# thunlp/OpenMatch

Hardware: AMD Instinct MI355X
Metric: passages/sec encode (bert-base DPR bi-encoder, 128 tok -> 768-d) [+ queries/sec exact top-1000 over 8.8M x 768 in `search`] (higher is better)
Workload: dtype f16; 1 GPU; bert-base DPR bi-encoder encode+search, MS MARCO 8.8M x 128-tok -> 768-d (BASELINE configs[1]); seq_len=128, global_batch=1024, index_rows=8841823, queries=6980, topk=1000, weights=random-init BertConfig() seed 0, parallelism=shard1

## Files before the change

### include/openmatch_hip.h

```cpp
#ifndef OPENMATCH_HIP_H
#define OPENMATCH_HIP_H

#include <stddef.h>
#include <stdint.h>

#ifdef __cplusplus
extern "C" {
#endif

#define OM_ABI_VERSION 6

#define OM_F32 0
#define OM_BF16 1
#define OM_F16 2

#define OM_ACT_NONE 0
#define OM_ACT_GELU_ERF 1
#define OM_ACT_RELU 2
#define OM_ACT_GELU_TANH 3
#define OM_ACT_SILU 5
#define OM_ACT_MUL_RESID 0x100
#define OM_ACT_PRE_GRAD 0x200

#define OM_ARCH_BERT 0
#define OM_ARCH_T5 1
#define OM_ARCH_MODERNBERT 2

#define OM_ARCH_CAUSAL 3

#define OM_ARCH_NOMICBERT 4

#define OM_POOL_NONE 0
#define OM_POOL_FIRST 1
#define OM_POOL_MEAN 2
#define OM_POOL_LAST 3

#define OM_SEARCH_F32 0
#define OM_SEARCH_F16_RESCORE 1
#define OM_SEARCH_F16_ONLY 2

const char* om_last_error(void);
int om_abi_version(void);

int om_device_count(void);

#define OM_TIMING_GEMM_BF16 0
#define OM_TIMING_GEMM_F32 1
#define OM_TIMING_SCAN 2
void om_debug_gemm_trace(unsigned long long* buf);
void om_debug_gemm_gen(int gen);
#define OM_GEMM_FAMILY_V1 1
#define OM_GEMM_FAMILY_V2 2
#define OM_GEMM_FAMILY_V6 6
#define OM_GEMM_FAMILY_G7 7
#define OM_GEMM_FAMILY_G7_ONE_TILE 70
#define OM_GEMM_FAMILY_G7C16 71
#define OM_GEMM_FAMILY_G7R16 72
#define OM_GEMM_FAMILY_SKINNY 9
int om_debug_gemm_last(void);
int om_debug_gemm_plan(int in_dtype, const void* A, int64_t lda, const void* B, int64_t ldb, int out_dtype, void* C, int64_t ldc,
                       int64_t M, int64_t N, int64_t K, const float* bias, const void* resid, int64_t ldr, int act);
typedef struct OmDebugGemmEpilogue {
  const float* bias; const void* resid; int64_t ldr; int act;
  void* pre_act; int64_t ldp; float drop_p; uint64_t seed; const int* drop_rows;
  const float* ln_stats; const float* ln_colsum; const float* rln_stats; const float* rln_g; const float* rln_b; float* stats_out;
  const void* resid_lo; void* out_lo;
  const float* resid32; float* out32;
  const float* a_ln32; const float* a_ln_g; const float* a_ln_b; float* a_ln_stats_out; const float* rln32; const float* rln32_stats;
  int lo8; float ln_inv_h, ln_eps; int ln_rms; int reverse;
  const int* rows_dev;
} OmDebugGemmEpilogue;
int om_debug_gemm_ex(int in_dtype, const void* A, int64_t lda, const void* B, int64_t ldb, int out_dtype, void* C, int64_t ldc,
                     int64_t M, int64_t N, int64_t K, const OmDebugGemmEpilogue* ep, void* stream);
int om_debug_gemm_plan_ex(int in_dtype, const void* A, int64_t lda, const void* B, int64_t ldb, int out_dtype, void* C, int64_t ldc,
                          int64_t M, int64_t N, int64_t K, const OmDebugGemmEpilogue* ep);
int om_debug_gemm_splitk(int in_dtype, const void* A, int64_t lda, const void* B, int64_t ldb, float* C, int64_t ldc, int64_t M,
                         int64_t N, int64_t K, void* stream);
#define OM_OPT_ENCODER_FUSED_LN 0
#define OM_OPT_ENCODER_DEBUG 1
#define OM_OPT_ATTENTION_FAST 2
#define OM_OPT_SCAN_GEN7 3
#define OM_OPT_SCAN_GROWTH 4
#define OM_OPT_WGRAD_DEBUG 5
#define OM_OPT_GEMM_GROUP_M 6
#define OM_OPT_SCAN_QGROUP 7
#define OM_OPT_TRAIN_WGRAD_STREAM 8
#define OM_OPT_ATTENTION_DEBUG 9
#define OM_OPT_ENCODER_PINGPONG 10
#define OM_OPT_ENCODER_TWO_PLANE 11
#define OM_OPT_GEMM_VARIANT 12
#define OM_OPT_SEARCH_DEBUG 13
#define OM_OPT_TRAIN_WGRAD_BATCH 14
#define OM_OPT_GEMM_MAX_GRID 15
#define OM_OPT_GEMM_CONT 16
#define OM_OPT_TRAIN_TAPE_GRAD 17
#define OM_OPT_TRAIN_RES32 18
#define OM_OPT_GEMM_SKINNY_M 19
#define OM_OPT_GEMM_SKINNY_CFG 20
#define OM_OPT_FEW_ROWS_LN_FUSE 21
#define OM_OPT_ENCODER_SKIP_PAD 22
#define OM_OPT_ENCODER_CLS_TAIL 23
#define OM_OPT_ENCODER_LANES 24
#define OM_OPT_COUNT 25
int om_debug_option(int opt, int value);
int om_debug_option_value(int opt);
int om_debug_attention(const void* qkv, void* ctx, const int64_t* mask, int64_t B, int L, int H, int heads, void* stream);
int om_debug_attention_ex(int dtype, const void* qkv, void* ctx, const int64_t* mask, const float* pos_bias, int64_t B, int L, int H,
                          int heads, float scale, float drop_p, uint64_t seed, void* stream, int reverse, const int* kmax,
                          const int* cu, int w);
int om_debug_rope(int dtype, void* qkv, int64_t M, int L, int H, float theta, void* stream);
int om_debug_rope_rows(int dtype, void* qkv, int64_t rows, int L, int H, float theta, const int* row_map, void* stream);
int om_debug_swiglu_rows(int dtype, const void* in, void* out, int64_t M, int F, void* stream);
int om_debug_embed(int dtype, const int64_t* ids, const int64_t* type_ids, const float* word, const float* pos, const float* type,
                   const float* g, const float* b, void* out, int64_t M, int L, int H, int vocab, int type_vocab, float eps, void* stream);
int om_debug_attention_causal(int dtype, const void* qkv, void* ctx, const int64_t* mask, int64_t B, int L, int n_heads, int n_kv_heads,
                              float scale, void* stream);
int om_debug_rope_gqa(int dtype, void* qkv, int64_t M, int L, int n_heads, int n_kv_heads, const float* inv_freq, float scaling, void* stream);
int om_debug_attention_causal_packed(int dtype, const void* qkv, void* ctx, const int64_t* mask, const int* cu, int64_t B, int L, int n_heads,
                                     int n_kv_heads, float scale, void* stream);
int om_debug_rope_gqa_rows(int dtype, void* qkv, int64_t rows, int L, int n_heads, int n_kv_heads, const float* inv_freq, float scaling,
                           const int* row_map, void* stream);
int om_debug_attention_causal_hd(int dtype, const void* qkv, void* ctx, const int64_t* mask, int64_t B, int L, int n_heads, int n_kv_heads,
                                 int head_dim, float scale, void* stream);
int om_debug_attention_causal_hd_packed(int dtype, const void* qkv, void* ctx, const int64_t* mask, const int* cu, int64_t B, int L,
                                        int n_heads, int n_kv_heads, int head_dim, float scale, void* stream);
int om_debug_qknorm_rope(int dtype, void* qkv, int64_t M, int L, int n_heads, int n_kv_heads, int head_dim, const float* q_norm_g,
                         const float* k_norm_g, float eps, const float* inv_freq, float scaling, void* stream);
int om_debug_qknorm_rope_rows(int dtype, void* qkv, int64_t rows, int L, int n_heads, int n_kv_heads, int head_dim, const float* q_norm_g,
                              const float* k_norm_g, float eps, const float* inv_freq, float scaling, const int* row_map, void* stream);
int om_debug_attention_gqa_d256(int dtype, const void* qkv, void* ctx, const int64_t* mask, int64_t B, int L, int n_heads, int n_kv_heads,
                                float scale, int w, void* stream);
int om_debug_qknorm_rope_d256(int dtype, void* qkv, int64_t M, int L, int n_heads, int n_kv_heads, const float* q_norm_g, const float* k_norm_g,
                              float eps, const float* inv_freq, float scaling, void* stream);
int om_debug_attention_gqa_d256_packed(int dtype, const void* qkv, void* ctx, const int64_t* mask, const int* cu, int64_t B, int L, int n_heads,
                                       int n_kv_heads, float scale, int w, void* stream);
int om_debug_qknorm_rope_d256_rows(int dtype, void* qkv, int64_t rows, int L, int n_heads, int n_kv_heads, const float* q_norm_g,
                                   const float* k_norm_g, float eps, const float* inv_freq, float scaling, const int* row_map, void* stream);
int om_debug_rmsnorm_add(int dtype, const void* h, int64_t ldh, float* x, int64_t ldx, const float* g, int64_t M, int H, float eps, void* stream);
int om_debug_mask_extent(const int64_t* mask, int64_t B, int L, int* kmax, void* stream);
int om_debug_pack_rows(const int* kmax, int64_t B, int L, int64_t rows, int* cu, int* cls_rows, int* row_map, void* stream);
#define OM_ATTN_FAMILY_GENERIC 1
#define OM_ATTN_FAMILY_FWD16 2
#define OM_ATTN_FAMILY_FWD16_KMAX4 3
#define OM_ATTN_FAMILY_FWD16C 4
#define OM_ATTN_FAMILY_LONG 5
#define OM_ATTN_FAMILY_D32 6
#define OM_ATTN_FAMILY_BAND16 7
#define OM_ATTN_FAMILY_BAND32 8
int om_debug_attention_last(void);
int om_debug_attention_plan(int dtype, int64_t B, int L, int H, int heads, int has_bias, float drop_p, int has_kmax, int has_cu, int w);
#define OM_ATTN_BWD_FAMILY_BWD16 1
#define OM_ATTN_BWD_FAMILY_GENERIC 2
#define OM_ATTN_BWD_FAMILY_LONG 3
#define OM_ATTN_BWD_FAMILY_D32 4
int om_debug_attention_bwd_last(void);
int om_debug_attention_bwd_plan(int dtype, int64_t B, int L, int H, int heads, int has_bias, int has_drel, int has_cu, int packed);
int om_debug_attention_bwd_ex(int dtype, const void* qkv, const void* ctx, const void* dctx, void* dqkv, const int64_t* mask,
                              const float* pos_bias, float* drel, float* stats, int64_t B, int L, int H, int heads, float scale,
                              float drop_p, uint64_t seed, const int* cu, int packed, void* stream);
size_t om_debug_attention_bwd_stats_bytes(int64_t B, int heads);
#define OM_ENC_PATH_BERT_FUSED 1
#define OM_ENC_PATH_BERT_PENDING_LN 2
#define OM_ENC_PATH_BERT_FEW32 3
#define OM_ENC_PATH_BERT_PLAIN 4
#define OM_ENC_PATH_MODERNBERT 5
#define OM_ENC_PATH_T5_FUSED 6
#define OM_ENC_PATH_T5_PLAIN 7
struct OmEncoderConfig;
int om_debug_encoder_plan(const struct OmEncoderConfig* cfg, int gated_ffn, int has_rel_bias, int64_t B, int64_t L, int64_t packed_rows,
                          int want_hidden);
int om_debug_encoder_skip_pad(const struct OmEncoderConfig* cfg, int gated_ffn, int has_rel_bias, int64_t B, int64_t L, int want_hidden);
int om_debug_encoder_cls_tail(const struct OmEncoderConfig* cfg, int gated_ffn, int has_rel_bias, int64_t B, int64_t L, int64_t packed_rows,
                              int want_hidden);
int om_debug_encoder_lanes(const struct OmEncoderConfig* cfg, int gated_ffn, int has_rel_bias, int64_t B, int64_t L, int64_t packed_rows,
                           int want_hidden, int64_t* B0);
#define OM_ENCODER_LANE_RANGES 15
int om_debug_encoder_lane_ranges(const struct OmEncoderConfig* cfg, int gated_ffn, int has_rel_bias, int64_t B, int64_t L, int lane,
                                 int64_t* out, int cap);
int64_t om_debug_encoder_lane_forks(void);
int om_debug_gather_rows(const void* src0, void* dst0, const void* src1, void* dst1, const void* src2, void* dst2, const float* stats_src,
                         float* stats_dst, const int* rows, int64_t B, int64_t L, int64_t Mc, int H, void* stream);
int om_debug_attn_drop_keep(uint64_t seed, int64_t b, int h, int heads, int Lm, int q, int key, float p);
int om_debug_wave_sum_check(const float* in, float* out_shuffle, float* out_dpp, int64_t groups, void* stream);
#define OM_ROW_FWD_GENERIC 1
#define OM_ROW_FWD_X8 2
#define OM_ROW_LN_BWD 3
int om_debug_row_kernel_last(void);
int om_debug_layernorm(int dtype, const void* x, int64_t ldx, void* y, int64_t ldy, const float* g, const float* b, int64_t M, int H,
                       float eps, int rms, const void* x_lo, int lo8, void* stream);
int om_debug_layernorm_f32out(int dtype, const void* x, int64_t ldx, float* y, int64_t ldy, const float* g, const float* b, int64_t M,
                              int H, float eps, int rms, const void* x_lo, const int* rows, int lo8, void* stream);
int om_debug_layernorm_from_f32(int dtype, const float* x, int64_t ldx, void* y, int64_t ldy, const float* g, const float* b, int64_t M,
                                int H, float eps, int rms, void* stream);
int om_debug_layernorm_dual(int dtype, const float* x, int64_t ldx, void* y, float* y32, int64_t ldy, const float* g, const float* b,
                            int64_t M, int H, float eps, void* stream);
int om_debug_norm_bwd(int dtype, const void* dy, const void* x, const float* g, void* dx, float* dg, float* db, int64_t M, int H,
                      float eps, int rms, const void* add, void* stream);
int om_debug_ln_bwd_drop(int dtype, const void* dy, const void* x, const float* g, void* dx, void* dx_drop, float drop_p,
                         uint64_t drop_seed, float* dg, float* db, int64_t M, int H, float eps, const float* dy32, const float* x32,
                         float* partial, int* partial_blocks , const int* drop_rows, void* stream);
typedef struct OmLnSite { const float* partial; float* dg; float* db; int blocks; } OmLnSite;
int om_debug_ln_param_reduce(const OmLnSite* sites , int n, int H, void* stream);
int om_debug_embed_bwd(int dtype, const void* dy, const int64_t* ids, const int64_t* type_ids, const float* word, const float* pos,
                       const float* type, const float* g, float* dword, float* dpos, float* dtype_, float* dg, float* db, int64_t M,
                       int L, int H, int vocab, int type_vocab, float eps, const int* cu, void* stream);
int om_debug_pool(int dtype, const void* x, const int64_t* mask, float* out, int64_t B, int L, int H, int mode, const int* cu,
                  void* stream);
int om_debug_pool_bwd(int dtype, const float* dp, const int64_t* mask, void* dh, int64_t B, int L, int H, int mode, const int* cu,
                      void* stream);
int om_debug_l2norm(const float* x, float* y, int64_t M, int D, void* stream);
int om_debug_l2norm_bwd(const float* x, const float* dy, float* dx, int64_t M, int D, void* stream);
int om_debug_colsum(int dtype, const void* x, int64_t ld, int64_t M, int N, float* out, void* stream);
int om_debug_dropout(int dtype, const void* x, void* y, int64_t n, float p, uint64_t seed, const int* rows, int H, void* stream);
int om_debug_ln_fold(int dtype, const void* W, const float* gamma, const float* beta, const float* b, void* Wf, float* colsum,
                     float* bf, int N, int K, void* stream);
int om_debug_ln_stats_reduce(const float* slots, int nslots, int64_t M, float* out, void* stream);
int om_debug_transpose(int dtype, const void* in, int64_t ldi, int64_t R, int C, void* out, int64_t ldo, int64_t Rp, int op, void* stream);
int om_debug_transpose_batch(int dtype, const void* const* in, void* const* out, const int* R, const int* C, int n, void* stream);
int om_debug_zero_rows_from(void* p, int64_t row_bytes, const int* first, int64_t M, void* stream);
int om_debug_t5_act_fwd(int dtype, const void* f, const void* f2, void* g, int64_t n, int kind, void* stream);
int om_debug_t5_act_bwd(int dtype, const void* dg, const void* f, const void* f2, void* df, void* df2, int64_t n, int kind, void* stream);
int om_debug_t5_embed_bwd(int dtype, const void* dy, const int64_t* ids, float* dword, int64_t M, int H, int vocab, const int* row_map,
                          void* stream);
int om_debug_t5_bias(const float* table, const int* lut, float* out, int L, int heads, void* stream);
int om_debug_t5_bias_bwd(const float* drel, const int* lut, float* dtable, int L, int heads, void* stream);
int om_kernel_timing_enable(int enable);
int om_kernel_timing_read(int kernel_class, double* total_ms, int64_t* launches, double* flops);

int om_gemm_nt(int in_dtype, const void* A, int64_t lda, const void* B, int64_t ldb,
               int out_dtype, void* C, int64_t ldc, int64_t M, int64_t N, int64_t K,
               const float* bias, const void* resid, int64_t ldr, int act, void* stream);

int om_gemm_tn_acc(int in_dtype, const void* A, int64_t lda, const void* B, int64_t ldb,
                   float* C, int64_t ldc, float* bias, int64_t M, int64_t N, int64_t K, void* stream);

typedef struct OmTnProblem {
  const void* A; const void* B; float* C; float* bias;
  int64_t lda, ldb, ldc, N, K;
} OmTnProblem;
int om_gemm_tn_acc_batch(int in_dtype, const OmTnProblem* problems, int n, int64_t M, void* stream);
int om_debug_gemm_tn_last(int64_t out[8]);
int om_debug_gemm_tn_plan(int dtype, int64_t M, int64_t N, int64_t K, int64_t lda, int64_t ldb, int batch, int64_t out[8]);

typedef struct OmLayerWeights {
  const void* qkv_w;
  const float* qkv_b;
  const void* o_w;
  const float* o_b;
  const float* ln1_g;
  const float* ln1_b;
  const void* ffn1_w;
  const float* ffn1_b;
  const void* ffn1g_w;
  const void* ffn2_w;
  const float* ffn2_b;
  const float* ln2_g;
  const float* ln2_b;
} OmLayerWeights;

typedef struct OmEncoderConfig {
  int arch;
  int dtype;
  int hidden;
  int n_layers;
  int n_heads;
  int head_dim;
  int ffn;
  int vocab;
  int max_pos;
  int type_vocab;
  int act;
  float ln_eps;
  int rel_buckets;
  int rel_max_dist;
  int pooling;
  int head_in;
  int head_out;
  int normalize;
  float rope_theta_global;
  float rope_theta_local;
  int half_window;
  uint64_t sliding_layers;
} OmEncoderConfig;

typedef struct OmEncoderWeights {
  const float* word_emb;
  const float* pos_emb;
  const float* type_emb;
  const float* emb_ln_g;
  const float* emb_ln_b;
  const OmLayerWeights* layers_host;
  const float* final_ln_g;
  const float* rel_bias;
  const float* head_w;
  const void* folded;
  const float* final_ln_b;
} OmEncoderWeights;

size_t om_encoder_fold_bytes(const OmEncoderConfig* cfg);
int om_encoder_fold_weights(const OmEncoderConfig* cfg, const OmEncoderWeights* w, void* folded, size_t bytes, void* stream);

size_t om_encoder_workspace_bytes(const OmEncoderConfig* cfg, int64_t B, int64_t L);

int om_t5_relative_bucket(int relative_position, int num_buckets, int max_distance);

int om_encoder_forward(const OmEncoderConfig* cfg, const OmEncoderWeights* w,
                       const int64_t* input_ids, const int64_t* attention_mask,
                       const int64_t* token_type_ids, int64_t B, int64_t L,
                       void* out_hidden, float* out_reps, void* workspace,
                       size_t workspace_bytes, void* stream);

int om_encoder_packed_supported(const OmEncoderConfig* cfg, int gated_ffn, int64_t B, int64_t L, int64_t packed_rows);
size_t om_encoder_workspace_bytes_packed(const OmEncoderConfig* cfg, int64_t B, int64_t L, int64_t packed_rows);
int om_encoder_forward_packed(const OmEncoderConfig* cfg, const OmEncoderWeights* w,
                              const int64_t* input_ids, const int64_t* attention_mask,
                              const int64_t* token_type_ids, int64_t B, int64_t L, int64_t packed_rows,
                              float* out_reps, void* workspace, size_t workspace_bytes, void* stream);

typedef struct OmCausalConfig {
  OmEncoderConfig base;
  int n_kv_heads;
  float rope_attention_scaling;
  float inv_freq[32];
} OmCausalConfig;
size_t om_causal_encoder_workspace_bytes(const OmCausalConfig* cfg, int64_t B, int64_t L);
int om_causal_encoder_forward(const OmCausalConfig* cfg, const OmEncoderWeights* w, const int64_t* input_ids,
                              const int64_t* attention_mask, int64_t B, int64_t L, void* out_hidden, float* out_reps,
                              void* workspace, size_t workspace_bytes, void* stream);
int om_causal_encoder_packed_supported(const OmCausalConfig* cfg, int64_t B, int64_t L, int64_t packed_rows);
size_t om_causal_encoder_workspace_bytes_packed(const OmCausalConfig* cfg, int64_t B, int64_t L, int64_t packed_rows);
int om_causal_encoder_forward_packed(const OmCausalConfig* cfg, const OmEncoderWeights* w, const int64_t* input_ids,
                                     const int64_t* attention_mask, int64_t B, int64_t L, int64_t packed_rows, float* out_reps,
                                     void* workspace, size_t workspace_bytes, void* stream);

typedef struct OmCausalConfig2 {
  OmCausalConfig base;
  int qk_norm;
  int reserved;
  float inv_freq[64];
} OmCausalConfig2;
typedef struct OmCausalQkNorm {
  const float* q_norm_g;
  const float* k_norm_g;
} OmCausalQkNorm;
size_t om_causal2_encoder_workspace_bytes(const OmCausalConfig2* cfg, int64_t B, int64_t L);
int om_causal2_encoder_forward(const OmCausalConfig2* cfg, const OmEncoderWeights* w, const OmCausalQkNorm* qk_norm_host,
                               const int64_t* input_ids, const int64_t* attention_mask, int64_t B, int64_t L, void* out_hidden,
                               float* out_reps, void* workspace, size_t workspace_bytes, void* stream);
int om_causal2_encoder_packed_supported(const OmCausalConfig2* cfg, int64_t B, int64_t L, int64_t packed_rows);
size_t om_causal2_encoder_workspace_bytes_packed(const OmCausalConfig2* cfg, int64_t B, int64_t L, int64_t packed_rows);
int om_causal2_encoder_forward_packed(const OmCausalConfig2* cfg, const OmEncoderWeights* w, const OmCausalQkNorm* qk_norm_host,
                                      const int64_t* input_ids, const int64_t* attention_mask, int64_t B, int64_t L, int64_t packed_rows,
                                      float* out_reps, void* workspace, size_t workspace_bytes, void* stream);

#define OM_ARCH_GEMMA3 5
typedef struct OmGemma3Config {
  OmCausalConfig base;
  float attn_scale;
  int half_window;
  uint64_t sliding_layers;
  float full_scaling;
  float sliding_scaling;
  float attn_logit_softcapping;
  int bidirectional;
  float full_inv_freq[128];
  float sliding_inv_freq[128];
} OmGemma3Config;
typedef struct OmGemma3Norms {
  const float* q_norm_g;
  const float* k_norm_g;
  const float* post_attention_norm_g;
  const float* post_feedforward_norm_g;
} OmGemma3Norms;
size_t om_gemma3_encoder_workspace_bytes(const OmGemma3Config* cfg, int64_t B, int64_t L);
int om_gemma3_encoder_forward(const OmGemma3Config* cfg, const OmEncoderWeights* w, const OmGemma3Norms* norms_host, const int64_t* input_ids,
                              const int64_t* attention_mask, int64_t B, int64_t L, void* out_hidden, float* out_reps, void* workspace,
                              size_t workspace_bytes, void* stream);
int om_gemma3_encoder_packed_supported(const OmGemma3Config* cfg, int64_t B, int64_t L, int64_t packed_rows);
size_t om_gemma3_encoder_workspace_bytes_packed(const OmGemma3Config* cfg, int64_t B, int64_t L, int64_t packed_rows);
int om_gemma3_encoder_forward_packed(const OmGemma3Config* cfg, const OmEncoderWeights* w, const OmGemma3Norms* norms_host,
                                     const int64_t* input_ids, const int64_t* attention_mask, int64_t B, int64_t L, int64_t packed_rows,
                                     float* out_reps, void* workspace, size_t workspace_bytes, void* stream);

typedef struct OmT5DecoderLayer {
  const void* sa_v_w;
  const void* sa_o_w;
  const float* sa_ln_g;
  const void* ca_q_w;
  const void* ca_kv_w;
  const void* ca_o_w;
  const float* ca_ln_g;
  const void* ffn1_w;
  const void* ffn1g_w;
  const void* ffn2_w;
  const float* ffn_ln_g;
} OmT5DecoderLayer;
typedef struct OmT5DecoderWeights {
  const float* start_emb;
  const float* final_ln_g;
  const OmT5DecoderLayer* layers_host;
  int n_layers;
} OmT5DecoderWeights;
size_t om_t5_decoder_workspace_bytes(const OmEncoderConfig* cfg, int64_t B, int64_t L);
int om_t5_decoder_step(const OmEncoderConfig* cfg, const OmT5DecoderWeights* w, const void* enc_hidden,
                       const int64_t* attention_mask, int64_t B, int64_t L, float* out_hidden,
                       void* workspace, size_t workspace_bytes, void* stream);

typedef struct OmT5DecoderLayerGrads {
  float* sa_v_w;  float* sa_o_w; float* sa_ln_g;
  float* ca_q_w;  float* ca_kv_w; float* ca_o_w; float* ca_ln_g;
  float* ffn1_w;  float* ffn1g_w; float* ffn2_w; float* ffn_ln_g;
} OmT5DecoderLayerGrads;
typedef struct OmT5DecoderGrads {
  float* start_emb;
  float* final_ln_g;
  const OmT5DecoderLayerGrads* layers_host;
} OmT5DecoderGrads;
size_t om_t5_decoder_tape_bytes(const OmEncoderConfig* cfg, int n_layers, int64_t B, int64_t L);
size_t om_t5_decoder_train_workspace_bytes(const OmEncoderConfig* cfg, int n_layers, int64_t B, int64_t L);
int om_t5_decoder_train_forward(const OmEncoderConfig* cfg, const OmT5DecoderWeights* w, const void* enc_hidden,
                                const int64_t* attention_mask, int64_t B, int64_t L, float dropout, uint64_t seed,
                                void* tape, size_t tape_bytes, float* out_hidden, void* workspace,
                                size_t workspace_bytes, void* stream);
int om_t5_decoder_train_backward(const OmEncoderConfig* cfg, const OmT5DecoderWeights* w, const void* enc_hidden,
                                 const int64_t* attention_mask, int64_t B, int64_t L, float dropout, uint64_t seed,
                                 const void* tape, const float* d_out, const OmT5DecoderGrads* grads,
                                 void* d_enc_hidden, void* workspace, size_t workspace_bytes, void* stream);

int om_linear_f32_backward(const float* dy, const float* x, const float* w, float* dw, float* dx, int B, int D, int K,
                           void* stream);

typedef struct OmLayerGrads {
  float* qkv_w;  float* qkv_b;  float* o_w;    float* o_b;   float* ln1_g; float* ln1_b;
  float* ffn1_w; float* ffn1_b; float* ffn2_w; float* ffn2_b; float* ln2_g; float* ln2_b;
  float* ffn1g_w;
} OmLayerGrads;

typedef struct OmEncoderGrads {
  float* word_emb; float* pos_emb; float* type_emb; float* emb_ln_g; float* emb_ln_b;
  const OmLayerGrads* layers_host;
  float* head_w;
  float* final_ln_g;
  float* rel_bias;
} OmEncoderGrads;

size_t om_encoder_tape_bytes(const OmEncoderConfig* cfg, int64_t B, int64_t L);
size_t om_encoder_train_workspace_bytes(const OmEncoderConfig* cfg, int64_t B, int64_t L);

int om_encoder_train_forward(const OmEncoderConfig* cfg, const OmEncoderWeights* w,
                             const int64_t* input_ids, const int64_t* attention_mask,
                             const int64_t* token_type_ids, int64_t B, int64_t L,
                             float hidden_dropout, float attn_dropout, uint64_t seed, void* tape,
                             size_t tape_bytes, float* out_reps, void* workspace,
                             size_t workspace_bytes, void* stream);

int om_encoder_train_backward(const OmEncoderConfig* cfg, const OmEncoderWeights* w,
                              const int64_t* input_ids, const int64_t* attention_mask,
                              const int64_t* token_type_ids, int64_t B, int64_t L,
                              float hidden_dropout, float attn_dropout, uint64_t seed,
                              const void* tape, const float* d_reps, const OmEncoderGrads* grads,
                              void* workspace, size_t workspace_bytes, void* stream);

int om_encoder_train_packed_supported(const OmEncoderConfig* cfg, int64_t B, int64_t L, int64_t packed_rows);
size_t om_encoder_tape_bytes_packed(const OmEncoderConfig* cfg, int64_t B, int64_t L, int64_t packed_rows);
size_t om_encoder_train_workspace_bytes_packed(const OmEncoderConfig* cfg, int64_t B, int64_t L, int64_t packed_rows);
int om_encoder_train_forward_packed(const OmEncoderConfig* cfg, const OmEncoderWeights* w,
                                    const int64_t* input_ids, const int64_t* attention_mask,
                                    const int64_t* token_type_ids, int64_t B, int64_t L, int64_t packed_rows,
                                    float hidden_dropout, float attn_dropout, uint64_t seed,
                                    void* tape, size_t tape_bytes, float* out_reps,
                                    void* workspace, size_t workspace_bytes, void* stream);
int om_encoder_train_backward_packed(const OmEncoderConfig* cfg, const OmEncoderWeights* w,
                                     const int64_t* input_ids, const int64_t* attention_mask,
                                     const int64_t* token_type_ids, int64_t B, int64_t L, int64_t packed_rows,
                                     float hidden_dropout, float attn_dropout, uint64_t seed,
                                     const void* tape, const float* d_reps, const OmEncoderGrads* grads,
// ... 107 lines not shown
```

### openmatch_amd/csrc/abi.cpp

```cpp
#include "common.h"

static thread_local std::string g_last_error;
void om_set_error(const std::string& msg) { g_last_error = msg; }

extern "C" const char* om_last_error(void) { return g_last_error.c_str(); }
extern "C" int om_abi_version(void) { return OM_ABI_VERSION; }
extern "C" int om_device_count(void) {
  int n = 0;
  hipError_t e = hipGetDeviceCount(&n);
  if (e != hipSuccess) {
    om_set_error(std::string("hipGetDeviceCount: ") + hipGetErrorString(e));
    return -1;
  }
  return n;
}

#include <mutex>
#include <vector>
namespace {
struct Span { hipEvent_t a, b; };
struct ClassStat { std::vector<Span> spans; double flops = 0; size_t used = 0; };
bool g_timing = false;
ClassStat g_stat[3];
std::mutex g_mu;
}
bool om_timing_on() { return g_timing; }
void om_timing_begin(int c, hipStream_t s) {
  std::lock_guard<std::mutex> lk(g_mu);
  ClassStat& st = g_stat[c];
  if (st.used == st.spans.size()) {
    Span sp;
    (void)hipEventCreate(&sp.a);
    (void)hipEventCreate(&sp.b);
    st.spans.push_back(sp);
  }
  (void)hipEventRecord(st.spans[st.used].a, s);
}
void om_timing_end(int c, hipStream_t s, double flops) {
  std::lock_guard<std::mutex> lk(g_mu);
  ClassStat& st = g_stat[c];
  (void)hipEventRecord(st.spans[st.used].b, s);
  st.used++;
  st.flops += flops;
}
extern "C" int om_kernel_timing_enable(int enable) { g_timing = enable != 0; return 0; }
extern "C" int om_kernel_timing_read(int c, double* total_ms, int64_t* launches, double* flops) {
  if (c < 0 || c > 2) { om_set_error("om_kernel_timing_read: bad class"); return 1; }
  std::lock_guard<std::mutex> lk(g_mu);
  ClassStat& st = g_stat[c];
  double ms = 0;
  for (size_t i = 0; i < st.used; ++i) {
    hipError_t e = hipEventSynchronize(st.spans[i].b);
    float t = 0;
    if (e == hipSuccess) e = hipEventElapsedTime(&t, st.spans[i].a, st.spans[i].b);
    if (e != hipSuccess) { om_set_error(std::string("om_kernel_timing_read: ") + hipGetErrorString(e)); return 1; }
    ms += t;
  }
  if (total_ms) *total_ms = ms;
  if (launches) *launches = (int64_t)st.used;
  if (flops) *flops = st.flops;
  st.used = 0; st.flops = 0;
  return 0;
}

#include <atomic>
#include <map>
#include <tuple>
namespace {
std::atomic<int> g_opt[OM_OPT_COUNT];
std::atomic<bool> g_opt_init{false};
std::mutex g_opt_mu;
void opt_init() {
  std::lock_guard<std::mutex> lk(g_opt_mu);
  if (g_opt_init.load()) return;
  const char* e = getenv("OM_ENCODER_FUSED_LN");
  g_opt[OM_OPT_ENCODER_FUSED_LN] = e ? atoi(e) : 1;
  g_opt[OM_OPT_ENCODER_DEBUG] = getenv("OM_ENCODER_DEBUG") ? 1 : 0;
  e = getenv("OM_ATTENTION_FAST");
  g_opt[OM_OPT_ATTENTION_FAST] = e ? atoi(e) : 1;
  e = getenv("OM_SCAN_GEN7");
  g_opt[OM_OPT_SCAN_GEN7] = e ? atoi(e) : 1;
  e = getenv("OM_SCAN_GROWTH");
  g_opt[OM_OPT_SCAN_GROWTH] = e ? atoi(e) : 60;
  g_opt[OM_OPT_WGRAD_DEBUG] = 0;
  g_opt[OM_OPT_ATTENTION_DEBUG] = 0;
  e = getenv("OM_ENCODER_PINGPONG");
  g_opt[OM_OPT_ENCODER_PINGPONG] = e ? atoi(e) : 1;
  e = getenv("OM_TRAIN_WGRAD_STREAM");
  g_opt[OM_OPT_TRAIN_WGRAD_STREAM] = e ? atoi(e) : 1;
  e = getenv("OM_SCAN_QGROUP");
  g_opt[OM_OPT_SCAN_QGROUP] = e ? atoi(e) : 8;
  e = getenv("OM_GEMM_GROUP_M");
  g_opt[OM_OPT_GEMM_GROUP_M] = e ? atoi(e) : 8;
  e = getenv("OM_ENCODER_TWO_PLANE");
  g_opt[OM_OPT_ENCODER_TWO_PLANE] = e ? atoi(e) : 3;
  e = getenv("OM_GEMM_VARIANT");
  g_opt[OM_OPT_GEMM_VARIANT] = e ? atoi(e) : 0;
  e = getenv("OM_SEARCH_DEBUG");
  g_opt[OM_OPT_SEARCH_DEBUG] = e ? (atoi(e) ? atoi(e) : 1) : 0;
  e = getenv("OM_TRAIN_WGRAD_BATCH");
  g_opt[OM_OPT_TRAIN_WGRAD_BATCH] = e ? atoi(e) : 4;
  e = getenv("OM_GEMM_MAX_GRID");
  g_opt[OM_OPT_GEMM_MAX_GRID] = e ? atoi(e) : 0;
  e = getenv("OM_TRAIN_TAPE_GRAD");
  g_opt[OM_OPT_TRAIN_TAPE_GRAD] = e ? atoi(e) : 1;
  e = getenv("OM_TRAIN_RES32");
  g_opt[OM_OPT_TRAIN_RES32] = e ? atoi(e) : 1;
  e = getenv("OM_GEMM_CONT");
  g_opt[OM_OPT_GEMM_CONT] = e ? atoi(e) : 495;
  e = getenv("OM_GEMM_SKINNY_M");
  g_opt[OM_OPT_GEMM_SKINNY_M] = e ? atoi(e) : 1024;
  e = getenv("OM_FEW_ROWS_LN_FUSE");
  g_opt[OM_OPT_FEW_ROWS_LN_FUSE] = e ? atoi(e) : 64;
  e = getenv("OM_ENCODER_SKIP_PAD");
  g_opt[OM_OPT_ENCODER_SKIP_PAD] = e ? atoi(e) : 1;
  e = getenv("OM_ENCODER_CLS_TAIL");
  g_opt[OM_OPT_ENCODER_CLS_TAIL] = e ? atoi(e) : 1;
  e = getenv("OM_ENCODER_LANES");
  g_opt[OM_OPT_ENCODER_LANES] = e ? atoi(e) : 65536;
  g_opt_init.store(true);
}
}
bool om_option_is_set(int opt) {
  if (opt == OM_OPT_SCAN_GROWTH) return getenv("OM_SCAN_GROWTH") != nullptr;
  return false;
}
int om_option(int opt) {
  if (!g_opt_init.load(std::memory_order_acquire)) opt_init();
  return g_opt[opt].load(std::memory_order_relaxed);
}
extern "C" int om_debug_option(int opt, int value) {
  if (opt < 0 || opt >= OM_OPT_COUNT) { om_set_error("om_debug_option: unknown option"); return 1; }
  if (!g_opt_init.load(std::memory_order_acquire)) opt_init();
  g_opt[opt].store(value);
  return 0;
}
extern "C" int om_debug_option_value(int opt) {
  if (opt < 0 || opt >= OM_OPT_COUNT) { om_set_error("om_debug_option_value: unknown option"); return -1; }
  return om_option(opt);
}

int om_t5_lut_device(int L, int buckets, int max_dist, const int** out) {
  static std::mutex mu;
  static std::map<std::tuple<int, int, int, int>, int*> cache;
  int dev = 0;
  OM_HIP(hipGetDevice(&dev));
  std::lock_guard<std::mutex> lk(mu);
  auto key = std::make_tuple(dev, L, buckets, max_dist);
  auto it = cache.find(key);
  if (it == cache.end()) {
    std::vector<int> lut(2 * L);
    for (int rel = -(L - 1); rel <= L - 1; ++rel) lut[rel + (L - 1)] = om_t5_relative_bucket(rel, buckets, max_dist);
    int* d = nullptr;
    OM_HIP(hipMalloc(&d, (size_t)(2 * L) * sizeof(int)));
    OM_HIP(hipMemcpy(d, lut.data(), (size_t)(2 * L - 1) * sizeof(int), hipMemcpyHostToDevice));
    it = cache.emplace(key, d).first;
  }
  *out = it->second;
  return 0;
}
```

### openmatch_amd/csrc/attention.hip

```cpp
#include <type_traits>

#include "attn_chunked.h"
#include "attn_plan.h"

static thread_local int g_attn_last = 0;
extern "C" int om_debug_attention_last(void) { return g_attn_last; }

template <typename T, int KT>
__global__ __launch_bounds__(64 * KT) void attention_kernel(
    const T* __restrict__ qkv, T* __restrict__ ctx, const int64_t* __restrict__ mask,
    const float* __restrict__ pos_bias, int L, int H, int heads, float scale, float drop_p,
    uint64_t seed) {
  typedef AttnGeom<T> G;
  typedef typename MmaOps<T>::frag_t frag_t;
  constexpr int LP = KT * 32 + 4;
  extern __shared__ __attribute__((aligned(16))) char smem[];
  char* sK = smem;
  T* sVt = (T*)(smem + KT * 32 * G::ROWB);
  float* sM = (float*)(smem + KT * 32 * G::ROWB + 64 * LP * (int)sizeof(T));

  const int h = blockIdx.x % heads;
  const int64_t b = blockIdx.x / heads;
  const int tid = threadIdx.x, nthr = blockDim.x;
  const int64_t ld = 3 * (int64_t)H;
  const T* base = qkv + b * L * ld + h * 64;

  for (int idx = tid; idx < KT * 32 * G::CPR; idx += nthr) {
    const int row = idx / G::CPR, c = idx % G::CPR;
    uint4 kv = make_uint4(0, 0, 0, 0), vv = make_uint4(0, 0, 0, 0);
    if (row < L) {
      kv = *(const uint4*)(base + (int64_t)row * ld + H + c * G::EPC);
      vv = *(const uint4*)(base + (int64_t)row * ld + 2 * H + c * G::EPC);
    }
    *(uint4*)(sK + row * G::ROWB + ((c ^ G::key(row)) << 4)) = kv;
    const T* ve = (const T*)&vv;
#pragma unroll
    for (int e = 0; e < G::EPC; ++e) sVt[(c * G::EPC + e) * LP + row] = ve[e];
  }
  for (int k = tid; k < KT * 32; k += nthr)
    sM[k] = k < L ? (mask[b * L + k] != 0 ? 0.f : kFinfoMin) : -INFINITY;
  __syncthreads();

  const int wave = tid >> 6, lane = tid & 63, half = lane >> 5, l31 = lane & 31;
  const int q0 = wave * 32;
  if (q0 >= L) return;
  const int qrow = (q0 + l31) < L ? (q0 + l31) : (L - 1);

  frag_t qf[G::NKK];
#pragma unroll
  for (int kk = 0; kk < G::NKK; ++kk)
    qf[kk] = *(const frag_t*)(base + (int64_t)qrow * ld + (kk * 2 + half) * G::EPC);

  f32x16_t s[KT];
#pragma unroll
  for (int t = 0; t < KT; ++t) {
#pragma unroll
    for (int r = 0; r < 16; ++r) s[t][r] = 0.f;
    const int row = t * 32 + l31;
    const char* krow = sK + row * G::ROWB;
    const int key = G::key(row);
#pragma unroll
    for (int kk = 0; kk < G::NKK; ++kk) {
      const frag_t a = *(const frag_t*)(krow + (((kk * 2 + half) ^ key) << 4));
      MmaOps<T>::mma(a, qf[kk], s[t]);
    }
  }

  float mx = -INFINITY;
#pragma unroll
  for (int t = 0; t < KT; ++t)
#pragma unroll
    for (int g = 0; g < 4; ++g) {
      const int k0 = t * 32 + 8 * g + 4 * half;
      const f32x4_t mb = *(const f32x4_t*)(sM + k0);
#pragma unroll
      for (int e = 0; e < 4; ++e) {
        float v = s[t][4 * g + e] * scale;
        if (pos_bias) {
          const int kc = (k0 + e) < L ? (k0 + e) : (L - 1);
          v += pos_bias[((int64_t)h * L + qrow) * L + kc];
        }
        v += mb[e];
        s[t][4 * g + e] = v;
        mx = fmaxf(mx, v);
      }
    }
  mx = fmaxf(mx, __shfl_xor(mx, 32, 64));
  float sum = 0.f;
#pragma unroll
  for (int t = 0; t < KT; ++t)
#pragma unroll
    for (int r = 0; r < 16; ++r) {
      const float e = G::exp_(s[t][r] - mx);
      s[t][r] = e;
      sum += e;
    }
  sum += __shfl_xor(sum, 32, 64);
  const float inv = 1.0f / sum;
#pragma unroll
  for (int t = 0; t < KT; ++t)
#pragma unroll
    for (int r = 0; r < 16; ++r) s[t][r] *= inv;
  if (drop_p > 0.f) {
    const AttnDrop dr(drop_p);
#pragma unroll
    for (int t = 0; t < KT; ++t)
#pragma unroll
      for (int g = 0; g < 4; ++g) {
        const uint64_t bits = attn_drop_bits(seed, b, h, heads, L, q0 + l31, (t * 32 + 8 * g + 4 * half) >> 2);
#pragma unroll
        for (int e = 0; e < 4; ++e) s[t][4 * g + e] = attn_drop_keep(bits, e, dr.thresh) ? s[t][4 * g + e] * dr.keep_scale : 0.f;
      }
  }

  f32x16_t o[2];
#pragma unroll
  for (int dt = 0; dt < 2; ++dt)
#pragma unroll
    for (int r = 0; r < 16; ++r) o[dt][r] = 0.f;
#pragma unroll
  for (int t = 0; t < KT; ++t) SlabMma<T>::run(s[t], sVt + l31 * LP + t * 32 + 4 * half, LP, o);

  __syncthreads();
  T* so = (T*)(sK + (size_t)q0 * G::ROWB);
#pragma unroll
  for (int dt = 0; dt < 2; ++dt)
#pragma unroll
    for (int r = 0; r < 16; ++r) {
      const int q = (r & 3) + 8 * (r >> 2) + 4 * half;
      ElemOps<T>::store(so + q * 64 + dt * 32 + l31, o[dt][r]);
    }
  T* out = ctx + (b * L + q0) * H + h * 64;
  constexpr int VPR = G::ROWB / 16;
#pragma unroll
  for (int it = 0; it < 32 * VPR / 64; ++it) {
    const int idx = it * 64 + lane, row = idx / VPR, c = idx % VPR;
    const uint4 v = *(const uint4*)((const char*)so + row * G::ROWB + c * 16);
    if (q0 + row < L) *(uint4*)((char*)(out + (int64_t)row * H) + c * 16) = v;
  }
}

template <typename T, int KT, bool BIAS, bool DROP, int DBG, int KTV>
__device__ __forceinline__ void attention_fwd16_body(
    const T* __restrict__ qkv, T* __restrict__ ctx, const int64_t* __restrict__ mask,
    const float* __restrict__ pos_bias, int L, int H, int heads, float scale, float drop_p, uint64_t seed, int rev,
    int64_t row0, int Lm) {
  typedef typename MmaOps<T>::frag_t frag_t;
  extern __shared__ __attribute__((aligned(16))) char smem[];
  char* const sK = smem;
  char* const sV = smem + KT * 32 * 128;
  float* const sM = (float*)(smem + 2 * KT * 32 * 128);
  const int h = blockIdx.x % heads;
  const int64_t b = rev ? (int64_t)(gridDim.x / heads) - 1 - blockIdx.x / heads : blockIdx.x / heads;
  const int tid = threadIdx.x, lane = tid & 63, half = lane >> 5, l31 = lane & 31;
  const int wave = __builtin_amdgcn_readfirstlane(tid >> 6);
  const int64_t ld2 = 6 * (int64_t)H;
  const char* const base = (const char*)(qkv + row0 * 3 * (int64_t)H + h * 64);
  if (!(DBG & 1))
#pragma unroll
  for (int i = 0; i < 4; ++i) {
    if (KTV < KT && i * KT + wave >= KTV * 4) continue;
    const int r = (i * KT + wave) * 8 + (lane >> 3);
    const int rr = r < L ? r : L - 1;
    const uint32_t off = (uint32_t)(rr * ld2) + (((lane & 7) ^ ((r >> 1) & 7)) << 4);
    const uint32_t offv = (uint32_t)(rr * ld2) + (((lane & 7) ^ (((r >> 1) & 1) << 2)) << 4);
    const uint32_t dst = (uint32_t)((i * KT + wave) * 1024);
    g7_dma(base + 2 * H, off, g7_lds_addr(sK) + dst);
    g7_dma(base + 4 * H, offv, g7_lds_addr(sV) + dst);
  }
  const float LOG2E = 1.4426950408889634f;
  for (int k = tid; k < KT * 32; k += 64 * KT)
    sM[k] = k < L ? (mask[b * Lm + k] != 0 ? 0.f : -1e30f) : -INFINITY;

  const int q0 = wave * 32;
  const int qrow = (q0 + l31) < L ? (q0 + l31) : (L - 1);
  frag_t qf[4];
#pragma unroll
  for (int kk = 0; kk < 4; ++kk) qf[kk] = *(const frag_t*)(base + (int64_t)qrow * ld2 + (kk * 2 + half) * 16);
  asm volatile("s_waitcnt vmcnt(0)" ::: "memory");
  __syncthreads();
  if (q0 >= L) return;

  constexpr int KTC = (DBG & 2) ? 0 : KTV;
  const int key = (l31 >> 1) & 7;
  f32x16_t s[KTV];
#pragma unroll
  for (int t = 0; t < KTC; ++t) {
#pragma unroll
    for (int r = 0; r < 16; ++r) s[t][r] = 0.f;
    const char* krow = sK + (t * 32 + l31) * 128;
#pragma unroll
    for (int kk = 0; kk < 4; ++kk) {
      const frag_t a = *(const frag_t*)(krow + (((kk * 2 + half) ^ key) << 4));
      MmaOps<T>::mma(a, qf[kk], s[t]);
    }
    __builtin_amdgcn_sched_barrier(0);
  }
  const float c2 = scale * LOG2E;
  float mx = -INFINITY;
#pragma unroll
  for (int t = 0; t < KTC; ++t)
#pragma unroll
    for (int g = 0; g < 4; ++g) {
      const int k0 = t * 32 + 8 * g + 4 * half;
      const f32x4_t mb = *(const f32x4_t*)(sM + k0);
      f32x4_t pb = {0.f, 0.f, 0.f, 0.f};
      if (BIAS) {
        const float* pr = pos_bias + ((int64_t)h * Lm + qrow) * Lm;
#pragma unroll
        for (int e = 0; e < 4; ++e) pb[e] = pr[(k0 + e) < Lm ? (k0 + e) : (Lm - 1)] * LOG2E;
      }
#pragma unroll
      for (int e = 0; e < 4; ++e) {
        const float v = fmaf(s[t][4 * g + e], c2, mb[e]) + pb[e];
        s[t][4 * g + e] = v;
        mx = fmaxf(mx, v);
      }
      __builtin_amdgcn_sched_barrier(0);
    }
  mx = fmaxf(mx, __shfl_xor(mx, 32, 64));
  float sum = 0.f;
#pragma unroll
  for (int t = 0; t < KTC; ++t)
#pragma unroll
    for (int r = 0; r < 16; ++r) {
      const float e = __builtin_amdgcn_exp2f(s[t][r] - mx);
      s[t][r] = e;
      sum += e;
    }
  sum += __shfl_xor(sum, 32, 64);
  float inv = 1.0f / sum;
  if (DROP) {
    const AttnDrop dr(drop_p);
#pragma unroll
    for (int t = 0; t < KTC; ++t)
  #pragma unroll
      for (int g = 0; g < 4; ++g) {
        const uint64_t bits = attn_drop_bits(seed, b, h, heads, Lm, q0 + l31, (t * 32 + 8 * g + 4 * half) >> 2);
#pragma unroll
        for (int e = 0; e < 4; ++e) s[t][4 * g + e] = attn_drop_keep(bits, e, dr.thresh) ? s[t][4 * g + e] : 0.f;
        __builtin_amdgcn_sched_barrier(0);
      }
    inv *= dr.keep_scale;
  }

  const int i16 = lane & 15;
  const char* const vt0 = sV + (4 * half + (i16 >> 2)) * 128 + 32 * ((lane >> 4) & 1) + 8 * (i16 & 3);
  const int vsw = (i16 >> 3) & 1;
  f32x16_t o[2];
#pragma unroll
  for (int dt = 0; dt < 2; ++dt)
#pragma unroll
    for (int r = 0; r < 16; ++r) o[dt][r] = 0.f;
#pragma unroll
  for (int t = 0; t < KTC; ++t) {
    uint4 pa[2];
#pragma unroll
    for (int u = 0; u < 2; ++u)
      pa[u] = make_uint4(Half16<T>::pack2(s[t][8 * u + 0], s[t][8 * u + 1]), Half16<T>::pack2(s[t][8 * u + 2], s[t][8 * u + 3]),
                         Half16<T>::pack2(s[t][8 * u + 4], s[t][8 * u + 5]), Half16<T>::pack2(s[t][8 * u + 6], s[t][8 * u + 7]));
#pragma unroll
    for (int u = 0; u < 2; ++u) {
#pragma unroll
      for (int dt = 0; dt < 2; ++dt) {
        const char* p = vt0 + (t * 32 + 16 * u) * 128 + ((dt ^ vsw) << 6);
        const frag_t vf = vfrag_of<frag_t>(vtrd(p), vtrd(p + 8 * 128));
        MmaOps<T>::mma(vf, __builtin_bit_cast(frag_t, pa[u]), o[dt]);
      }
    }
    __builtin_amdgcn_sched_barrier(0);
  }
  if (DBG & 2) {
#pragma unroll
    for (int kk = 0; kk < 4; ++kk) o[0][kk] = (float)qf[kk][0];
  }
  __syncthreads();
  char* const so = sK + q0 * 128;
#pragma unroll
  for (int dt = 0; dt < 2; ++dt)
#pragma unroll
    for (int gp = 0; gp < 2; ++gp) {
      uint32_t a0 = Half16<T>::pack2(o[dt][8 * gp + 0] * inv, o[dt][8 * gp + 1] * inv), a1 = Half16<T>::pack2(o[dt][8 * gp + 2] * inv, o[dt][8 * gp + 3] * inv);
      uint32_t b0 = Half16<T>::pack2(o[dt][8 * gp + 4] * inv, o[dt][8 * gp + 5] * inv), b1 = Half16<T>::pack2(o[dt][8 * gp + 6] * inv, o[dt][8 * gp + 7] * inv);
      auto r0 = __builtin_amdgcn_permlane32_swap(a0, b0, false, false);
      auto r1 = __builtin_amdgcn_permlane32_swap(a1, b1, false, false);
      *(uint4*)(so + l31 * 128 + (((4 * dt + 2 * gp + half) ^ (l31 & 7)) << 4)) = make_uint4(r0[0], r1[0], r0[1], r1[1]);
    }
  char* const out = (char*)(ctx + (row0 + q0) * (int64_t)H + h * 64);
#pragma unroll
  for (int it = 0; it < 4; ++it) {
    const int row = it * 8 + (lane >> 3), c = lane & 7;
    const uint4 v = *(const uint4*)(so + row * 128 + ((c ^ (row & 7)) << 4));
    if (!(DBG & 4) || v.x == 0x12345u) { if (q0 + row < L) *(uint4*)(out + (int64_t)row * H * 2 + c * 16) = v; }
  }
}

template <typename T, int KT, bool BIAS, bool DROP, int DBG = 0>
__global__ __launch_bounds__(64 * KT, KT <= 4 ? ((BIAS || DROP) ? 3 : 4) : 2) void attention_fwd16_kernel(
    const T* __restrict__ qkv, T* __restrict__ ctx, const int64_t* __restrict__ mask,
    const float* __restrict__ pos_bias, int L, int H, int heads, float scale, float drop_p, uint64_t seed, int rev,
    const int* __restrict__ kmax, const int* __restrict__ cu) {
#define OM_ATTN_BODY(V) attention_fwd16_body<T, KT, BIAS, DROP, DBG, V>(qkv, ctx, mask, pos_bias, Lb, H, heads, scale, drop_p, seed, rev, row0, L)
  const int64_t b = rev ? (int64_t)(gridDim.x / heads) - 1 - blockIdx.x / heads : blockIdx.x / heads;
  int64_t row0 = b * L;
  int Lb = L;
  if (cu) {
    const int c0 = __builtin_amdgcn_readfirstlane(cu[b]), c1 = __builtin_amdgcn_readfirstlane(cu[b + 1]);
    row0 = c0; Lb = c1 - c0;
    if (Lb <= 0) return;
  }
  if (KT == 4 && !BIAS && !DROP && (kmax || cu)) {
    const int kt = ((cu ? Lb : __builtin_amdgcn_readfirstlane(kmax[b])) + 31) >> 5;
    if (kt <= 1) { OM_ATTN_BODY(1); return; }
    if (kt == 2) { OM_ATTN_BODY(2); return; }
    if (kt == 3) { OM_ATTN_BODY(3); return; }
  }
  OM_ATTN_BODY(KT);
#undef OM_ATTN_BODY
}

template <typename T, int KT, bool BIAS, bool DROP>
static int launch_attn16(const void* qkv, void* ctx, const int64_t* mask, const float* pos_bias, int64_t B, int L, int H,
                         int heads, float scale, float drop_p, uint64_t seed, hipStream_t s, int rev, const int* kmax, const int* cu) {
  const int lds = 2 * KT * 32 * 128 + KT * 32 * 4;
  if (attn_lds_once<attention_fwd16_kernel<T, KT, BIAS, DROP>>(lds)) return 1;
#ifdef OM_PROBE_KERNELS
  const int dbg = (sizeof(T) == 2 && std::is_same<T, bf16_t>::value && KT == 4 && !BIAS && !DROP) ? om_option(OM_OPT_ATTENTION_DEBUG) : 0;
#else
  const int dbg = 0;
#endif
  if (dbg) {
#ifdef OM_PROBE_KERNELS
#define OM_ATTN_DBG(D)                                                                                                        \
  case D:                                                                                                                     \
    hipLaunchKernelGGL((attention_fwd16_kernel<bf16_t, 4, false, false, D>), dim3((unsigned)(heads * B)), dim3(256), lds, s,          \
                       (const bf16_t*)qkv, (bf16_t*)ctx, mask, pos_bias, L, H, heads, scale, drop_p, seed, rev, kmax, cu);    \
    break;
    switch (dbg) { OM_ATTN_DBG(1) OM_ATTN_DBG(2) OM_ATTN_DBG(3) OM_ATTN_DBG(4) OM_ATTN_DBG(5) OM_ATTN_DBG(6) OM_ATTN_DBG(7) default: break; }
#undef OM_ATTN_DBG
#endif
    OM_LAUNCH_CHECK();
    return 0;
  }
  hipLaunchKernelGGL((attention_fwd16_kernel<T, KT, BIAS, DROP>), dim3((unsigned)(heads * B)), dim3(64 * KT), lds, s, (const T*)qkv,
                     (T*)ctx, mask, pos_bias, L, H, heads, scale, drop_p, seed, rev, kmax, cu);
  OM_LAUNCH_CHECK();
  return 0;
}
template <typename T, bool BIAS, bool DROP>
__global__ __launch_bounds__(256, 2) void attention_fwd16c_kernel(
    const T* __restrict__ qkv, T* __restrict__ ctx, const int64_t* __restrict__ mask,
    const float* __restrict__ pos_bias, int Lm, int H, int heads, float scale, float drop_p, uint64_t seed, const int* __restrict__ cu) {
  const int h = blockIdx.x % heads;
  const int64_t b = blockIdx.x / heads;
  int64_t row0 = b * Lm;
  int L = Lm;
  if (cu) {
    const int c0 = __builtin_amdgcn_readfirstlane(cu[b]), c1 = __builtin_amdgcn_readfirstlane(cu[b + 1]);
    row0 = c0; L = c1 - c0;
  }
  const int qb = blockIdx.y * 128;
  if (qb >= L) return;
  attn_chunked16<T, AttnFull, BIAS, DROP>(attn_rows_fused(qkv, ctx, row0, H, h), AttnFull{}, mask + b * Lm, L, L, qb, scale, AttnFullArgs{pos_bias, drop_p, seed, b, h, heads, Lm});
}

template <typename T, bool BIAS, bool DROP>
static int launch_attn16c(const void* qkv, void* ctx, const int64_t* mask, const float* pos_bias, int64_t B, int L, int H,
                           int heads, float scale, float drop_p, uint64_t seed, hipStream_t s, const int* cu) {
  const int lds = 2 * 128 * 128 + 128 * 4;
  hipLaunchKernelGGL((attention_fwd16c_kernel<T, BIAS, DROP>), dim3((unsigned)(heads * B), (unsigned)((L + 127) / 128)), dim3(256), lds, s,
                     (const T*)qkv, (T*)ctx, mask, pos_bias, L, H, heads, scale, drop_p, seed, cu);
  OM_LAUNCH_CHECK();
  return 0;
}
template <typename T>
__global__ __launch_bounds__(256) void attention_long_kernel(
    const T* __restrict__ qkv, T* __restrict__ ctx, const int64_t* __restrict__ mask,
    const float* __restrict__ pos_bias, int Lm, int H, int heads, float scale, float drop_p, uint64_t seed, const int* __restrict__ cu) {
  const int h = blockIdx.x % heads;
  const int64_t b = blockIdx.x / heads;
  const int qb = blockIdx.y * 128;
  int64_t row0 = b * Lm;
  int L = Lm;
  if (cu) { row0 = cu[b]; L = cu[b + 1] - cu[b]; }
  if (qb >= L) return;
  attn_chunked_qreg<T, AttnFull>(attn_rows_fused(qkv, ctx, row0, H, h), AttnFull{}, mask + b * Lm, L, L, qb, scale, AttnFullArgs{pos_bias, drop_p, seed, b, h, heads, Lm});
}

template <typename T>
static int launch_attn_long(const void* qkv, void* ctx, const int64_t* mask, const float* pos_bias, int64_t B, int L, int H,
                            int heads, float scale, float drop_p, uint64_t seed, hipStream_t s, const int* cu) {
  const int lds = 128 * AttnGeom<T>::ROWB + 64 * 132 * (int)sizeof(T) + 128 * 4 + 128 * 4;
  if (attn_lds_once<attention_long_kernel<T>>(lds)) return 1;
  hipLaunchKernelGGL((attention_long_kernel<T>), dim3((unsigned)(heads * B), (unsigned)((L + 127) / 128)), dim3(256), lds, s,
                     (const T*)qkv, (T*)ctx, mask, pos_bias, L, H, heads, scale, drop_p, seed, cu);
  OM_LAUNCH_CHECK();
  return 0;
}

template <typename T, int KT>
static int launch_attn(const void* qkv, void* ctx, const int64_t* mask, const float* pos_bias,
                       int64_t B, int L, int H, int heads, float scale, float drop_p, uint64_t seed,
                       hipStream_t s) {
  constexpr int LP = KT * 32 + 4;
  const int lds = KT * 32 * AttnGeom<T>::ROWB + 64 * LP * (int)sizeof(T) + KT * 32 * 4;
  if (attn_lds_once<attention_kernel<T, KT>>(lds)) return 1;
  const int waves = (L + 31) / 32;
  hipLaunchKernelGGL((attention_kernel<T, KT>), dim3((unsigned)(heads * B)),
                     dim3(64 * waves), lds, s, (const T*)qkv, (T*)ctx, mask, pos_bias, L, H, heads,
                     scale, drop_p, seed);
  OM_LAUNCH_CHECK();
  return 0;
}

__global__ void mask_extent_kernel(const int64_t* __restrict__ mask, int64_t B, int L, int* __restrict__ kmax) {
  const int64_t b = (int64_t)blockIdx.x * (blockDim.x >> 6) + (threadIdx.x >> 6);
  if (b >= B) return;
  const int lane = threadIdx.x & 63;
  int last = 0;
  for (int k = lane; k < L; k += 64) if (mask[b * L + k] != 0) last = k + 1;
#pragma unroll
  for (int o = 32; o > 0; o >>= 1) last = max(last, __shfl_xor(last, o, 64));
  if (lane == 0) kmax[b] = last ? last : L;
}
__global__ __launch_bounds__(1024) void pack_rows_kernel(const int* __restrict__ kmax, int64_t B, int L, int64_t rows, int* __restrict__ cu,
                                                          int* __restrict__ cls_rows, int* __restrict__ row_map) {
  __shared__ int part[1024];
  const int tid = threadIdx.x;
  const int64_t per = (B + 1023) / 1024, lo = tid * per, hi = lo + per < B ? lo + per : B;
  int sum = 0;
  for (int64_t i = lo; i < hi; ++i) sum += kmax[i];
  part[tid] = sum;
  __syncthreads();
  for (int off = 1; off < 1024; off <<= 1) {
    const int v = tid >= off ? part[tid - off] : 0;
    __syncthreads();
    part[tid] += v;
    __syncthreads();
  }
  const int total = part[1023];
  const int cap = (int)rows;
  if (blockIdx.x == 0) {
    int run = part[tid] - sum;
    for (int64_t i = lo; i < hi; ++i) {
      cu[i] = run < cap ? run : cap;
      cls_rows[i] = run < cap ? run : cap - 1;
      run += kmax[i];
    }
    if (tid == 1023) { cu[B] = total < cap ? total : cap; cu[B + 1] = total; }
  }
  for (int64_t t = (int64_t)blockIdx.x * 1024 + tid; t < rows; t += (int64_t)gridDim.x * 1024) {
    int v = -1;
    if (t < total) {
      int a = 0, b = 1023;
      while (a < b) { const int m = (a + b) >> 1; if (part[m] > (int)t) b = m; else a = m + 1; }
      int64_t i = a * per;
      int run = a ? part[a - 1] : 0;
      for (int n = kmax[i]; run + n <= (int)t; n = kmax[++i]) run += n;
      v = (int)(i * L + ((int)t - run));
    }
    row_map[t] = v;
  }
}
int omk_pack_rows(const int* kmax, int64_t B, int L, int64_t rows, int* cu, int* cls_rows, int* row_map, hipStream_t s) {
  if (B <= 0) return 0;
  if (rows > 0x7fffffff || B * (int64_t)L > 0x7fffffff) OM_FAIL("packed rows: token counts below 2^31");
  const int64_t slices = (rows + 1023) / 1024;
  hipLaunchKernelGGL(pack_rows_kernel, dim3((unsigned)(slices < 1 ? 1 : slices > 1024 ? 1024 : slices)), dim3(1024), 0, s, kmax, B, L, rows, cu, cls_rows,
                     row_map);
  OM_LAUNCH_CHECK();
  return 0;
}

int omk_mask_extent(const int64_t* mask, int64_t B, int L, int* kmax, hipStream_t s) {
  if (B <= 0) return 0;
  hipLaunchKernelGGL(mask_extent_kernel, dim3((unsigned)((B + 3) / 4)), dim3(256), 0, s, mask, B, L, kmax);
  OM_LAUNCH_CHECK();
  return 0;
}

int omk_attention(int dtype, const void* qkv, void* ctx, const int64_t* mask, const float* pos_bias, int64_t B, int L, int H, int heads,
                  float scale, float drop_p, uint64_t seed, hipStream_t s, int reverse, const int* kmax, const int* cu, int w) {
  g_attn_last = 0;
  const AttnPlan p = attn_plan_fwd(dtype, B, L, H, heads, pos_bias != nullptr, drop_p, kmax != nullptr, cu != nullptr, w, attn_switches());
  if (p.error) OM_FAIL(p.error);
  g_attn_last = p.family | (p.kt << 8);
  switch (p.family) {
    case 0: return 0;
    case OM_ATTN_FAMILY_D32: return omk_attention_d32(p, dtype, qkv, ctx, mask, pos_bias, B, L, H, heads, scale, drop_p, seed, s, reverse, kmax, cu);
    case OM_ATTN_FAMILY_BAND16: case OM_ATTN_FAMILY_BAND32: return omk_attention_band(dtype, qkv, ctx, mask, B, L, H, heads, scale, w, kmax, s);
    case OM_ATTN_FAMILY_FWD16: case OM_ATTN_FAMILY_FWD16_KMAX4:
      return attn_with_type16(dtype, [&](auto t) {
        return attn_with_kt<1, 2, 4, 6, 8>(p.kt, [&](auto kt) {
          return attn_with_flags(p.bias, p.drop, [&](auto bias, auto drop) {
            return launch_attn16<decltype(t), kt(), bias(), drop()>(qkv, ctx, mask, pos_bias, B, L, H, heads, scale, drop_p, seed, s, reverse, kmax, cu);
          });
        });
      });
    case OM_ATTN_FAMILY_FWD16C:
      return attn_with_type16(dtype, [&](auto t) {
        return attn_with_flags(p.bias, p.drop, [&](auto bias, auto drop) {
          return launch_attn16c<decltype(t), bias(), drop()>(qkv, ctx, mask, pos_bias, B, L, H, heads, scale, drop_p, seed, s, cu);
        });
      });
    case OM_ATTN_FAMILY_LONG:
      return attn_with_type(dtype, [&](auto t) { return launch_attn_long<decltype(t)>(qkv, ctx, mask, pos_bias, B, L, H, heads, scale, drop_p, seed, s, cu); });
    default:
      if (dtype == OM_BF16)
        return attn_with_kt<1, 2, 4, 6, 8>(p.kt, [&](auto kt) { return launch_attn<bf16_t, kt()>(qkv, ctx, mask, pos_bias, B, L, H, heads, scale, drop_p, seed, s); });
      return attn_with_kt<1, 2, 4, 6, 8>(p.kt, [&](auto kt) { return launch_attn<float, kt()>(qkv, ctx, mask, pos_bias, B, L, H, heads, scale, drop_p, seed, s); });
  }
}

extern "C" int om_debug_attention_plan(int dtype, int64_t B, int L, int H, int heads, int has_bias, float drop_p, int has_kmax, int has_cu, int w) {
  const AttnPlan p = attn_plan_fwd(dtype, B, L, H, heads, has_bias != 0, drop_p, has_kmax != 0, has_cu != 0, w, attn_switches());
  if (p.error) { om_set_error(std::string(__func__) + ": " + p.error); return -1; }
  return p.family | (p.kt << 8);
}

extern "C" int om_debug_attention_ex(int dtype, const void* qkv, void* ctx, const int64_t* mask, const float* pos_bias, int64_t B, int L, int H,
                                     int heads, float scale, float drop_p, uint64_t seed, void* stream, int reverse, const int* kmax,
                                     const int* cu, int w) {
  g_attn_last = 0;
  if (!qkv || !ctx || !mask) OM_FAIL("null argument");
  if (dtype != OM_F32 && dtype != OM_BF16 && dtype != OM_F16) OM_FAIL("attention: dtype must be OM_F32, OM_BF16 or OM_F16");
  if (w > 0 && (pos_bias || drop_p > 0.f || cu || reverse)) OM_FAIL("banded attention: no position bias, dropout, packed rows or reverse walk");
  return omk_attention(dtype, qkv, ctx, mask, pos_bias, B, L, H, heads, scale, drop_p, seed, (hipStream_t)stream, reverse, kmax, cu, w);
}
extern "C" int om_debug_attention(const void* qkv, void* ctx, const int64_t* mask, int64_t B, int L, int H, int heads, void* stream) {
  return om_debug_attention_ex(OM_BF16, qkv, ctx, mask, nullptr, B, L, H, heads, 0.125f, 0.f, 0, stream, 0, nullptr, nullptr, 0);
}
extern "C" int om_debug_rope(int dtype, void* qkv, int64_t M, int L, int H, float theta, void* stream) {
  if (!qkv) OM_FAIL("null argument");
  if (dtype != OM_F32 && dtype != OM_BF16 && dtype != OM_F16) OM_FAIL("rotary positions: dtype must be OM_F32, OM_BF16 or OM_F16");
  return omk_rope(dtype, qkv, M, L, H, theta, (hipStream_t)stream);
}
extern "C" int om_debug_rope_rows(int dtype, void* qkv, int64_t rows, int L, int H, float theta, const int* row_map, void* stream) {
  if (!qkv || !row_map) OM_FAIL("null argument");
  if (dtype != OM_F32 && dtype != OM_BF16 && dtype != OM_F16) OM_FAIL("rotary positions: dtype must be OM_F32, OM_BF16 or OM_F16");
  return omk_rope(dtype, qkv, rows, L, H, theta, (hipStream_t)stream, row_map);
}
extern "C" int om_debug_mask_extent(const int64_t* mask, int64_t B, int L, int* kmax, void* stream) {
  if (!mask || !kmax) OM_FAIL("null argument");
  if (L < 1) OM_FAIL("mask extent: L must be at least 1");
  return omk_mask_extent(mask, B, L, kmax, (hipStream_t)stream);
}
extern "C" int om_debug_pack_rows(const int* kmax, int64_t B, int L, int64_t rows, int* cu, int* cls_rows, int* row_map, void* stream) {
  if (!kmax || !cu || !cls_rows || !row_map) OM_FAIL("null argument");
  if (rows < 1) OM_FAIL("packed rows: rows must be at least 1");
  return omk_pack_rows(kmax, B, L, rows, cu, cls_rows, row_map, (hipStream_t)stream);
}
extern "C" int om_debug_attn_drop_keep(uint64_t seed, int64_t b, int h, int heads, int Lm, int q, int key, float p) {
  return attn_drop_keep1(seed, b, h, heads, Lm, q, key, AttnDrop(p).thresh) ? 1 : 0;
}
```

### openmatch_amd/csrc/attn_plan.h

```cpp
#pragma once
#include "kernels.h"

struct AttnSwitches {
  int fast;
};

static AttnSwitches attn_switches() { return AttnSwitches{om_option(OM_OPT_ATTENTION_FAST)}; }

static int attn_kt(int L) { return L <= 32 ? 1 : L <= 64 ? 2 : L <= 128 ? 4 : L <= 192 ? 6 : 8; }

static bool attn_is16(int dtype) { return dtype == OM_BF16 || dtype == OM_F16; }

struct AttnPlan { int family; int kt; bool bias, drop; const char* error; };

static AttnPlan attn_plan_fwd(int dtype, int64_t B, int L, int H, int heads, bool has_bias, float drop_p, bool has_kmax, bool has_cu, int w,
                              const AttnSwitches sw) {
  AttnPlan p = {0, 0, has_bias, drop_p > 0.f, nullptr};
  auto run = [&](int family, int kt) { p.family = family; p.kt = kt; return p; };
  auto refuse = [&](const char* why) { p.error = why; return p; };
  const bool d32 = H == heads * 32;
  if (dtype != OM_F32 && !attn_is16(dtype)) return refuse("attention: dtype must be OM_F32, OM_BF16 or OM_F16");
  if (B <= 0) return p;
  const bool band = w > 0 && w < L - 1;
  if (band && H != heads * 64) return refuse("banded attention: head_dim must be 64");
  if (band && (has_bias || p.drop || has_cu)) return refuse("banded attention: no position bias, dropout, packed rows or reverse walk");
  if (!band && !d32 && H != heads * 64) return refuse("head_dim must be 32 or 64");
  if (has_cu && !(dtype == OM_F16 || (dtype == OM_BF16 && (d32 || sw.fast)))) return refuse("packed rows: the 16-bit attention kernels");
  if (L < 1 || L > 1024) return refuse("sequence length must be in [1,1024]");
  if (L > 256 && p.drop && (L > 512 || dtype == OM_F32)) return refuse("attention with dropout: up to 512 tokens in the 16-bit formats (float32: 256)");
  if (B * heads > 0x7fffffffLL) return refuse("batch too large for one launch");
  if (d32) return run(OM_ATTN_FAMILY_D32, attn_kt(L));
  if (band) return run(dtype == OM_F32 ? OM_ATTN_FAMILY_BAND32 : OM_ATTN_FAMILY_BAND16, 4);
  const bool fast16 = dtype == OM_F16 || (dtype == OM_BF16 && sw.fast);
  if (L > 256 || ((sw.fast & 2) && dtype != OM_F32)) return run(fast16 && !(sw.fast & 4) ? OM_ATTN_FAMILY_FWD16C : OM_ATTN_FAMILY_LONG, 4);
  if (fast16) return run(attn_kt(L) == 4 && !has_bias && !p.drop && (has_kmax || has_cu) ? OM_ATTN_FAMILY_FWD16_KMAX4 : OM_ATTN_FAMILY_FWD16, attn_kt(L));
  return run(OM_ATTN_FAMILY_GENERIC, attn_kt(L));
}

static AttnPlan attn_plan_bwd(int dtype, int64_t B, int L, int H, int heads, bool has_bias, bool has_drel, bool has_cu, bool packed,
                              const AttnSwitches sw) {
  AttnPlan p = {0, 0, has_bias, false, nullptr};
  auto run = [&](int family, int kt) { p.family = family; p.kt = kt; return p; };
  auto refuse = [&](const char* why) { p.error = why; return p; };
  const bool b16 = attn_is16(dtype);
  if (B <= 0) return p;
  if (H != heads * 32 && H != heads * 64) return refuse("head_dim must be 32 or 64");
  if (H == heads * 32) {
    if (L < 1 || L > 256) return refuse("training with head_dim 32 supports sequence lengths up to 256");
    if (has_cu && !b16) return refuse("packed rows: attention backward for 16-bit formats");
    if (B * heads > 0x7fffffffLL) return refuse("batch too large for one launch");
    if (has_bias != has_drel) return refuse("attention backward: a position bias needs its gradient buffer (and the reverse)");
    if (!b16 && dtype != OM_F32) return refuse("attention backward: dtype must be OM_F32, OM_BF16 or OM_F16");
    return run(OM_ATTN_BWD_FAMILY_D32, attn_kt(L));
  }
  if (L > 256 || (!packed && dtype != OM_F32 && ((sw.fast & 2) || ((sw.fast & 1) && L > 192)))) {
    if (L < 1 || L > 512) return refuse("attention backward (tile-at-a-time form): up to 512 tokens");
    if (!b16) return refuse("attention backward beyond 256 tokens: 16-bit formats");
    if (has_cu) return refuse("attention backward (tile-at-a-time form): no packed rows");
    return run(OM_ATTN_BWD_FAMILY_LONG, 4);
  }
  if (has_cu && !b16) return refuse("packed rows: attention backward for 16-bit formats");
  if (b16 && L >= 1 && L <= 128 && sw.fast && has_bias == has_drel) return run(OM_ATTN_BWD_FAMILY_BWD16, attn_kt(L));
  if (L < 1 || L > 256)
    return refuse(has_cu && !has_bias && !has_drel ? "packed rows: attention backward up to 256 tokens, head_dim 64" : "training supports sequence lengths up to 256");
  if (dtype == OM_F32 && L > 192) return refuse("float32 training supports sequence lengths up to 192 (16-bit formats: 256)");
  return run(OM_ATTN_BWD_FAMILY_GENERIC, attn_kt(L));
}
```

### openmatch_amd/csrc/encoder.hip

```cpp
#include <math.h>

#include <stdlib.h>

#include <algorithm>
#include <atomic>
#include <map>
#include <mutex>
#include <utility>
#include <vector>

#include "encoder_plan.h"

namespace {
struct FoldSlot { size_t w, cs, bf; };
struct FoldLayout { size_t per_layer, total; FoldSlot qkv, ffn1; };
FoldLayout fold_layout(const OmEncoderConfig* c) {
  const size_t H = c->hidden, F = enc_ffn1_cols(c);
  size_t off = 0;
  auto take = [&](size_t bytes) { size_t o = off; off = align_up(off + bytes, 256); return o; };
  FoldLayout L;
  L.qkv.w = take(3 * H * H * 2); L.qkv.cs = take(3 * H * 4); L.qkv.bf = take(3 * H * 4);
  L.ffn1.w = take(F * H * 2); L.ffn1.cs = take(F * 4); L.ffn1.bf = take(F * 4);
  L.per_layer = off;
  L.total = off * (size_t)c->n_layers;
  return L;
}
bool fold_applies(const OmEncoderConfig* c) {
  return c->arch != OM_ARCH_MODERNBERT && (c->dtype == OM_BF16 || c->dtype == OM_F16) && c->n_layers > 0 && c->hidden % 256 == 0 && c->ffn % 256 == 0;
}
}

extern "C" size_t om_encoder_fold_bytes(const OmEncoderConfig* cfg) {
  if (!cfg || !fold_applies(cfg)) return 0;
  return fold_layout(cfg).total;
}

extern "C" int om_encoder_fold_weights(const OmEncoderConfig* c, const OmEncoderWeights* w, void* blob, size_t bytes, void* stream) {
  if (!c || !w || !blob) OM_FAIL("null argument");
  if (!fold_applies(c)) OM_FAIL("nothing to fold for this configuration (om_encoder_fold_bytes is 0)");
  const FoldLayout L = fold_layout(c);
  if (bytes < L.total || ((uintptr_t)blob & 255)) OM_FAIL("fold buffer too small or not 256-byte aligned");
  const OmLayerWeights* Ls = w->layers_host;
  if (!Ls) OM_FAIL("layers_host is null");
  hipStream_t s = (hipStream_t)stream;
  const int H = c->hidden, F = enc_ffn1_cols(c);
  const bool bert = enc_bert_family(c);
  for (int l = 0; l < c->n_layers; ++l) {
    char* base = (char*)blob + (size_t)l * L.per_layer;
    const OmLayerWeights& lw = Ls[l];
    if (l > 0) {
      const float* g = bert ? Ls[l - 1].ln2_g : lw.ln1_g;
      const float* beta = bert ? Ls[l - 1].ln2_b : nullptr;
      if (omk_ln_fold(c->dtype, lw.qkv_w, g, beta, bert ? lw.qkv_b : nullptr, base + L.qkv.w, (float*)(base + L.qkv.cs),
                      (float*)(base + L.qkv.bf), 3 * H, H, s)) return 1;
    }
    if (!lw.ffn1g_w) {
      const float* g = bert ? lw.ln1_g : lw.ln2_g;
      const float* beta = bert ? lw.ln1_b : nullptr;
      if (omk_ln_fold(c->dtype, lw.ffn1_w, g, beta, bert ? lw.ffn1_b : nullptr, base + L.ffn1.w, (float*)(base + L.ffn1.cs),
                      (float*)(base + L.ffn1.bf), F, H, s)) return 1;
    }
  }
  return 0;
}

static int folded_weights(const OmEncoderConfig* c, const OmEncoderWeights* w, int layer, bool ffn1, const void* W, const float* g,
                          const float* beta, const float* b, int N, int K, void* scratch_w, float* scratch_cs, float* scratch_bf,
                          hipStream_t s, const void** Wf, const float** cs, const float** bf) {
  if (w->folded) {
    const FoldLayout L = fold_layout(c);
    const char* base = (const char*)w->folded + (size_t)layer * L.per_layer;
    const FoldSlot& sl = ffn1 ? L.ffn1 : L.qkv;
    *Wf = base + sl.w; *cs = (const float*)(base + sl.cs); *bf = (const float*)(base + sl.bf);
    return 0;
  }
  if (omk_ln_fold(c->dtype, W, g, beta, b, scratch_w, scratch_cs, scratch_bf, N, K, s)) return 1;
  *Wf = scratch_w; *cs = scratch_cs; *bf = scratch_bf;
  return 0;
}

struct EncWs {
  char *x, *y, *x1, *qkv, *ctx, *ff, *ff2;
  float *pooled, *headout, *posbias;
  float* final32;
  int* lut;
  int* kmax;
  int *cu, *cls_rows, *row_map;
  char* wfold;
  float *colsum, *bfold, *stats1, *stats2, *slots;
  char *y_lo, *x1_lo;
  float *r32a, *r32b, *y32;
  size_t total;
};

static EncWs carve(const OmEncoderConfig* c, const EncPlan& p, int64_t B, int64_t L, int64_t packed_rows, char* base) {
  const bool half = c->dtype == OM_BF16 || c->dtype == OM_F16;
  const size_t es = half ? 2 : 4;
  const size_t Mreal = (size_t)p.M, M = (size_t)p.Mp, H = c->hidden, F = c->ffn, F1 = enc_ffn1_cols(c);
  const bool bertf = enc_bert_family(c);
  size_t off = 0;
  auto take = [&](size_t bytes) { size_t o = off; off = align_up(off + bytes, 256); return base + o; };
  EncWs w;
  w.x = take(M * H * es);
  w.y = take(M * H * es);
  w.x1 = take(M * H * es);
  w.qkv = take(M * 3 * H * es);
  w.ctx = take(M * H * es);
  w.ff = take(M * F1 * es);
  w.ff2 = take(c->arch == OM_ARCH_T5 || c->arch == OM_ARCH_MODERNBERT || c->arch == OM_ARCH_NOMICBERT ? M * F * es : 0);
  w.pooled = (float*)take((size_t)B * H * 4);
  w.headout = (float*)take((size_t)B * (c->head_out > 0 ? c->head_out : 1) * 4);
  const bool rel = c->arch == OM_ARCH_T5 || (c->arch == OM_ARCH_BERT && c->rel_buckets > 0);
  w.posbias = (float*)take(rel ? (size_t)c->n_heads * L * L * 4 : 0);
  w.lut = (int*)take(rel ? (size_t)(2 * L) * 4 : 0);
  w.kmax = (int*)take((size_t)B * 4);
  w.cu = (int*)take(packed_rows > 0 ? (size_t)(B + 2) * 4 : 0);
  w.cls_rows = (int*)take(packed_rows > 0 ? (size_t)B * 4 : 0);
  w.row_map = (int*)take(packed_rows > 0 ? (size_t)packed_rows * 4 : 0);
  w.final32 = (float*)take(half && c->pooling != OM_POOL_NONE ? (c->pooling == OM_POOL_FIRST ? (size_t)B : Mreal) * H * 4 : 0);
  const bool fuse = half && c->arch != OM_ARCH_MODERNBERT;
  const size_t wide = std::max((size_t)3 * H, F1);
  w.wfold = take(fuse ? wide * H * es : 0);
  w.colsum = (float*)take(fuse ? wide * 4 : 0);
  w.bfold = (float*)take(fuse ? wide * 4 : 0);
  w.stats1 = (float*)take(fuse ? (size_t)2 * c->n_layers * M * 8 : 0);
  w.stats2 = w.stats1 ? w.stats1 + (size_t)c->n_layers * M * 2 : nullptr;
  w.slots = (float*)take(fuse ? (size_t)2 * ((H + 255) / 256) * M * 8 : 0);
  const bool two = fuse && bertf;
  w.y_lo = take(two ? M * H * es : 0);
  w.x1_lo = take(two ? M * H * es : 0);
  w.r32a = (float*)take(p.alloc_few32 ? Mreal * H * 4 : 0);
  w.r32b = (float*)take(p.alloc_few32 ? Mreal * H * 4 : 0);
  w.y32 = (float*)take(p.alloc_few32 ? Mreal * H * 4 : 0);
  w.total = off;
  return w;
}

static size_t workspace_bytes(const OmEncoderConfig* c, int64_t B, int64_t L, int64_t packed_rows) {
  const EncPlan p = encoder_plan_checked(EncPlanIn{c, B, L, packed_rows, false, false, false, false}, encoder_switches());
  return carve(c, p, B, L, packed_rows, nullptr).total;
}

extern "C" size_t om_encoder_workspace_bytes(const OmEncoderConfig* cfg, int64_t B, int64_t L) {
  if (!cfg || B <= 0 || L <= 0) return 0;
  return workspace_bytes(cfg, B, L, 0);
}

extern "C" size_t om_encoder_workspace_bytes_packed(const OmEncoderConfig* cfg, int64_t B, int64_t L, int64_t packed_rows) {
  if (!cfg || B <= 0 || L <= 0 || packed_rows <= 0) return 0;
  return workspace_bytes(cfg, B, L, packed_rows);
}

extern "C" int om_encoder_packed_supported(const OmEncoderConfig* c, int gated_ffn, int64_t B, int64_t L, int64_t packed_rows) {
  return encoder_packed_ok(c, gated_ffn != 0, B, L, packed_rows, encoder_switches()) ? 1 : 0;
}

extern "C" int om_debug_encoder_plan(const OmEncoderConfig* c, int gated_ffn, int has_rel_bias, int64_t B, int64_t L, int64_t packed_rows,
                                     int want_hidden) {
  if (!c) {
    om_set_error("om_debug_encoder_plan: null argument");
    return -1;
  }
  const EncPlan p = encoder_plan(EncPlanIn{c, B, L, packed_rows, want_hidden != 0, gated_ffn != 0, has_rel_bias != 0, c->type_vocab > 0},
                                 encoder_switches());
  if (p.error) {
    om_set_error(std::string("om_debug_encoder_plan: ") + p.error);
    return -1;
  }
  return p.path | (int)p.few_rows << 8 | (int)p.two << 9 | p.lo8 << 10;
}

extern "C" int om_debug_encoder_skip_pad(const OmEncoderConfig* c, int gated_ffn, int has_rel_bias, int64_t B, int64_t L, int want_hidden) {
  if (!c) {
    om_set_error("om_debug_encoder_skip_pad: null argument");
    return -1;
  }
  const EncPlanIn in = {c, B, L, 0, want_hidden != 0, gated_ffn != 0, has_rel_bias != 0, c->type_vocab > 0};
  const EncSwitches sw = encoder_switches();
  return encoder_skip_pad(in, encoder_plan(in, sw), sw) ? 1 : 0;
}

extern "C" int om_debug_encoder_cls_tail(const OmEncoderConfig* c, int gated_ffn, int has_rel_bias, int64_t B, int64_t L, int64_t packed_rows,
                                         int want_hidden) {
  if (!c) {
    om_set_error("om_debug_encoder_cls_tail: null argument");
    return -1;
  }
  const EncPlanIn in = {c, B, L, packed_rows, want_hidden != 0, gated_ffn != 0, has_rel_bias != 0, c->type_vocab > 0};
  const EncSwitches sw = encoder_switches();
  return encoder_cls_tail(in, encoder_plan(in, sw), sw) ? 1 : 0;
}

extern "C" int om_t5_relative_bucket(int relative_position, int num_buckets, int max_distance) {
  int nb = num_buckets / 2;
  int bucket = relative_position > 0 ? nb : 0;
  const int n = relative_position < 0 ? -relative_position : relative_position;
  const int max_exact = nb / 2;
  if (n < max_exact) return bucket + n;
  const double v = log((double)n / max_exact) / log((double)max_distance / max_exact) * (nb - max_exact);
  int large = max_exact + (int)v;
  if (large > nb - 1) large = nb - 1;
  return bucket + large;
}

static int check_cfg(const OmEncoderConfig* c) {
  if (const char* why = encoder_cfg_error(c)) OM_FAIL(why);
  return 0;
}

struct EncCall {
  const OmEncoderConfig* c;
  const OmEncoderWeights* w;
  const int64_t* mask;
  int64_t B, L;
  const EncPlan& p;
  const EncWs& ws;
  const float* posbias;
  const int* cu;
  const int* row_map;
  void* out_hidden;
  hipStream_t s;
  const int* rows_dev;
  int64_t cls_mc;
  std::vector<int>* families;
  int64_t whole_mg, whole_mc;
};

struct EncStream {
  const void* x;
  const void* x_lo;
  int lo8;
  const float *g, *b;
  int rms;
  void* spare;
  char* hidden;
  const float* rows32;
  bool cls_compact;
};

#define GEMM(A_, lda_, W_, ldw_, C_, ldc_, N_, K_, bias_, res_, ldr_, act_)                        \
  do {                                                                                             \
    if (om_gemm_nt(dt, A_, lda_, W_, ldw_, dt, C_, ldc_, Mg, N_, K_, bias_, res_, ldr_, act_, s)) \
      return 1;                                                                                    \
  } while (0)
#define RUN(expr) do { if (expr) return 1; } while (0)
#define ENC_LOCALS                                                                                                   \
  const OmEncoderConfig* c = k.c; const EncWs& ws = k.ws; const OmLayerWeights* Ls = k.w->layers_host; hipStream_t s = k.s;     \
  const int dt = c->dtype, H = c->hidden, F = c->ffn, nh = c->n_heads;                                              \
  const int64_t B = k.B, L = k.L, M = k.p.M, Mg = k.p.Mg
#define NOMIC_LOCALS                                                                                                 \
  const bool nomic = c->arch == OM_ARCH_NOMICBERT;                                                                   \
  const int F1 = enc_ffn1_cols(c), act1 = nomic ? OM_ACT_NONE : c->act;                                             \
  const void* const ffa = nomic ? ws.ff2 : ws.ff
#define NOMIC_ROPE() do { if (nomic) RUN(omk_rope(dt, ws.qkv, M, (int)L, H, c->rope_theta_global, s, k.row_map)); } while (0)
#define NOMIC_SWIGLU(rows_) do { if (nomic) RUN(omk_swiglu_rows(dt, ws.ff, ws.ff2, rows_, F, s)); } while (0)

static int bert_fused(const EncCall& k, EncStream* out) {
  ENC_LOCALS;
  NOMIC_LOCALS;
  const float scale = 1.0f / sqrtf((float)c->head_dim);
  const float inv_h = 1.0f / (float)H;
  const bool two = k.p.two;
  const int lo8 = k.p.lo8;
  const int nslots = 2 * (H / 256);
  const bool pingpong = k.p.pingpong;
  int walk = 1;
  const bool probe = k.families != nullptr;
  auto gemm = [&](const void* A, int64_t lda, const void* W, int64_t ldw, void* C, int64_t ldc, int64_t rows, int64_t N, int64_t K,
                  const GemmEpilogue& ep) {
    const int64_t as = rows == Mg ? k.whole_mg : k.whole_mc;
    if (!probe) return omk_gemm(dt, A, lda, W, ldw, dt, C, ldc, rows, N, K, ep, s, as);
    k.families->push_back(omk_gemm_family(dt, A, lda, W, ldw, dt, C, ldc, rows, N, K, ep, as));
    return 0;
  };
#define LAUNCH(expr) do { if (!probe) RUN(expr); } while (0)
  const int64_t Mc = k.cls_mc;
  const size_t cplane = (size_t)Mc * H * 2;
  char* const cbase = ws.qkv;
  float* const cst2p = (float*)(cbase + 7 * cplane);
  float* const cst1 = cst2p + 2 * Mc;
  if (Mc > 0 && ((char*)(cst1 + 2 * Mc) > ws.qkv + (size_t)Mg * 3 * H * 2 || Mc > Mg || c->n_layers < 2 || lo8))
    OM_FAIL("[CLS] tail: the compact buffers do not fit the qkv area");
#define OM_WALK() (pingpong ? (walk ^= 1, walk ^ 1) : 0)
  for (int l = 0; l < c->n_layers; ++l) {
    const OmLayerWeights& lw = Ls[l];
    const bool last = l == c->n_layers - 1, tail = last && Mc > 0;
    float* st1 = tail ? cst1 : ws.stats1 + (size_t)l * Mg * 2;
    float* st2 = ws.stats2 + (size_t)l * Mg * 2;
    const float* st2p = l ? ws.stats2 + (size_t)(l - 1) * Mg * 2 : nullptr;
    const int64_t Mr = tail ? Mc : Mg;
    const int* const rdev = tail ? nullptr : k.rows_dev;
    const char *ctx = ws.ctx, *xin = ws.x1, *xin_lo = ws.x1_lo;
    char *y = ws.y, *y_lo = ws.y_lo, *xout = ws.x1, *xout_lo = ws.x1_lo;
    GemmEpilogue e = {};
    if (l == 0) {
      e.bias = lw.qkv_b; e.reverse = OM_WALK(); e.rows_dev = k.rows_dev;
      RUN(gemm(ws.x, H, lw.qkv_w, H, ws.qkv, 3 * H, Mg, 3 * H, H, e));
    } else {
      const OmLayerWeights& pw = Ls[l - 1];
      const void* wf; const float *cs, *bfp;
      RUN(folded_weights(c, k.w, l, false, lw.qkv_w, pw.ln2_g, pw.ln2_b, lw.qkv_b, 3 * H, H, ws.wfold, ws.colsum, ws.bfold, s, &wf, &cs, &bfp));
      e.bias = bfp; e.ln_stats = st2p; e.ln_colsum = cs; e.ln_inv_h = inv_h; e.ln_eps = c->ln_eps; e.reverse = OM_WALK(); e.rows_dev = k.rows_dev;
      RUN(gemm(ws.x1, H, wf, H, ws.qkv, 3 * H, Mg, 3 * H, H, e));
    }
    if (!probe) NOMIC_ROPE();
    const int attn_walk = OM_WALK();
    LAUNCH(omk_attention(dt, ws.qkv, ws.ctx, k.mask, k.posbias, B, (int)L, H, nh, scale, 0.f, 0, s, attn_walk, ws.kmax, k.cu));
    if (tail) {
      const GatherPlane planes[3] = {{ws.ctx, cbase}, {ws.x1, cbase + cplane}, {two ? ws.x1_lo : nullptr, cbase + 2 * cplane}};
      LAUNCH(omk_gather_rows(planes, st2p, cst2p, k.cu ? ws.cls_rows : nullptr, B, L, Mc, H, s));
      ctx = cbase; xin = cbase + cplane; xin_lo = cbase + 2 * cplane; st2p = cst2p;
      y = cbase + 3 * cplane; y_lo = cbase + 4 * cplane; xout = cbase + 5 * cplane; xout_lo = cbase + 6 * cplane;
    }
    e = GemmEpilogue{};
    e.bias = lw.o_b; e.ldr = H; e.stats_out = ws.slots; e.ln_inv_h = inv_h; e.ln_eps = c->ln_eps;
    if (two) { e.out_lo = y_lo; e.lo8 = lo8; }
    if (l == 0) {
      e.resid = ws.x;
    } else {
      const OmLayerWeights& pw = Ls[l - 1];
      e.resid = xin; e.rln_stats = st2p; e.rln_g = pw.ln2_g; e.rln_b = pw.ln2_b;
      if (two) e.resid_lo = xin_lo;
    }
    e.reverse = OM_WALK(); e.rows_dev = rdev;
    RUN(gemm(ctx, H, lw.o_w, H, y, H, Mr, H, H, e));
    LAUNCH(omk_ln_stats_reduce(ws.slots, nslots, Mr, st1, s));
    const void* wf1; const float *cs1, *bf1;
    RUN(folded_weights(c, k.w, l, true, lw.ffn1_w, lw.ln1_g, lw.ln1_b, lw.ffn1_b, F1, H, ws.wfold, ws.colsum, ws.bfold, s, &wf1, &cs1, &bf1));
    e = GemmEpilogue{};
    e.bias = bf1; e.act = act1; e.ln_stats = st1; e.ln_colsum = cs1; e.ln_inv_h = inv_h; e.ln_eps = c->ln_eps;
    e.reverse = OM_WALK(); e.rows_dev = rdev;
    RUN(gemm(y, H, wf1, H, ws.ff, F1, Mr, F1, H, e));
    if (!probe) NOMIC_SWIGLU(Mr);
    e = GemmEpilogue{};
    e.bias = lw.ffn2_b; e.resid = y; e.ldr = H; e.rln_stats = st1; e.rln_g = lw.ln1_g; e.rln_b = lw.ln1_b;
    e.stats_out = ws.slots; e.ln_inv_h = inv_h; e.ln_eps = c->ln_eps;
    if (two) { e.resid_lo = y_lo; e.out_lo = xout_lo; e.lo8 = lo8; }
    e.reverse = OM_WALK(); e.rows_dev = rdev;
    RUN(gemm(ffa, F, lw.ffn2_w, F, xout, H, Mr, H, F, e));
    if (!last) LAUNCH(omk_ln_stats_reduce(ws.slots, nslots, Mg, st2, s));
  }
#undef LAUNCH
#undef OM_WALK
  const OmLayerWeights& lastw = Ls[c->n_layers - 1];
  *out = EncStream{ws.x1, two ? ws.x1_lo : nullptr, lo8, lastw.ln2_g, lastw.ln2_b, 0, ws.x};
  if (Mc > 0) { out->x = cbase + 5 * cplane; out->x_lo = two ? cbase + 6 * cplane : nullptr; out->cls_compact = true; }
  return 0;
}

static int bert_pending_ln(const EncCall& k, EncStream* out) {
  ENC_LOCALS;
  NOMIC_LOCALS;
  const float scale = 1.0f / sqrtf((float)c->head_dim);
  float* const y_a = ws.y32;
  float* const y_b = ws.r32b;
  for (int l = 0; l < c->n_layers; ++l) {
    const OmLayerWeights& lw = Ls[l];
    float* const st1 = ws.stats1 + (size_t)l * M * 2;
    float* const st2p = l ? ws.stats2 + (size_t)(l - 1) * M * 2 : nullptr;
    GemmEpilogue e = {};
    e.bias = lw.qkv_b; e.ln_eps = c->ln_eps;
    if (l) { e.a_ln32 = y_b; e.a_ln_g = Ls[l - 1].ln2_g; e.a_ln_b = Ls[l - 1].ln2_b; e.a_ln_stats_out = st2p; }
    RUN(omk_gemm(dt, ws.x, H, lw.qkv_w, H, dt, ws.qkv, 3 * H, Mg, 3 * H, H, e, s));
    NOMIC_ROPE();
    RUN(omk_attention(dt, ws.qkv, ws.ctx, k.mask, k.posbias, B, (int)L, H, nh, scale, 0.f, 0, s, 0, ws.kmax));
    e = GemmEpilogue{};
    e.bias = lw.o_b; e.ldr = H; e.out32 = y_a; e.ln_eps = c->ln_eps;
    if (l) { e.rln32 = y_b; e.rln32_stats = st2p; e.rln_g = Ls[l - 1].ln2_g; e.rln_b = Ls[l - 1].ln2_b; }
    else e.resid32 = ws.r32a;
    RUN(omk_gemm(dt, ws.ctx, H, lw.o_w, H, dt, ws.y, H, Mg, H, H, e, s));
    e = GemmEpilogue{};
    e.bias = lw.ffn1_b; e.act = act1; e.ln_eps = c->ln_eps;
    e.a_ln32 = y_a; e.a_ln_g = lw.ln1_g; e.a_ln_b = lw.ln1_b; e.a_ln_stats_out = st1;
    RUN(omk_gemm(dt, ws.x1, H, lw.ffn1_w, H, dt, ws.ff, F1, Mg, F1, H, e, s));
    NOMIC_SWIGLU(Mg);
    e = GemmEpilogue{};
    e.bias = lw.ffn2_b; e.ldr = H; e.out32 = y_b; e.ln_eps = c->ln_eps;
    e.rln32 = y_a; e.rln32_stats = st1; e.rln_g = lw.ln1_g; e.rln_b = lw.ln1_b;
    RUN(omk_gemm(dt, ffa, F, lw.ffn2_w, F, dt, ws.y, H, Mg, H, F, e, s));
  }
  const OmLayerWeights& last = Ls[c->n_layers - 1];
  void* dst = k.out_hidden ? k.out_hidden : (void*)ws.x;
  RUN(omk_layernorm_dual(dt, y_b, H, dst, ws.r32a, H, last.ln2_g, last.ln2_b, M, H, c->ln_eps, s));
  *out = EncStream{};
  out->hidden = (char*)dst; out->rows32 = ws.r32a;
  return 0;
}

static int bert_few32(const EncCall& k, EncStream* out) {
  ENC_LOCALS;
  NOMIC_LOCALS;
  const float scale = 1.0f / sqrtf((float)c->head_dim);
  void* dst = ws.x;
  for (int l = 0; l < c->n_layers; ++l) {
    const OmLayerWeights& lw = Ls[l];
    GEMM(ws.x, H, lw.qkv_w, H, ws.qkv, 3 * H, 3 * H, H, lw.qkv_b, nullptr, 0, OM_ACT_NONE);
    NOMIC_ROPE();
    RUN(omk_attention(dt, ws.qkv, ws.ctx, k.mask, k.posbias, B, (int)L, H, nh, scale, 0.f, 0, s, 0, ws.kmax));
    GemmEpilogue e = {};
    e.bias = lw.o_b; e.resid32 = ws.r32a; e.ldr = H; e.out32 = ws.y32;
    RUN(omk_gemm(dt, ws.ctx, H, lw.o_w, H, dt, ws.y, H, Mg, H, H, e, s));
    RUN(omk_layernorm_dual(dt, ws.y32, H, ws.x1, ws.r32b, H, lw.ln1_g, lw.ln1_b, M, H, c->ln_eps, s));
    GEMM(ws.x1, H, lw.ffn1_w, H, ws.ff, F1, F1, H, lw.ffn1_b, nullptr, 0, act1);
    NOMIC_SWIGLU(Mg);
    e = GemmEpilogue{};
    e.bias = lw.ffn2_b; e.resid32 = ws.r32b; e.ldr = H; e.out32 = ws.y32;
    RUN(omk_gemm(dt, ffa, F, lw.ffn2_w, F, dt, ws.y, H, Mg, H, F, e, s));
    if (l == c->n_layers - 1 && k.out_hidden) dst = k.out_hidden;
    RUN(omk_layernorm_dual(dt, ws.y32, H, dst, ws.r32a, H, lw.ln2_g, lw.ln2_b, M, H, c->ln_eps, s));
  }
  *out = EncStream{};
  out->hidden = (char*)dst; out->rows32 = ws.r32a;
  return 0;
}

static int bert_plain(const EncCall& k, EncStream* out) {
  ENC_LOCALS;
  NOMIC_LOCALS;
  const float scale = 1.0f / sqrtf((float)c->head_dim);
  for (int l = 0; l < c->n_layers; ++l) {
    const OmLayerWeights& lw = Ls[l];
    if (l) RUN(omk_layernorm(dt, ws.y, H, ws.x, H, Ls[l - 1].ln2_g, Ls[l - 1].ln2_b, M, H, c->ln_eps, 0, s));
    GEMM(ws.x, H, lw.qkv_w, H, ws.qkv, 3 * H, 3 * H, H, lw.qkv_b, nullptr, 0, OM_ACT_NONE);
    NOMIC_ROPE();
    RUN(omk_attention(dt, ws.qkv, ws.ctx, k.mask, k.posbias, B, (int)L, H, nh, scale, 0.f, 0, s, 0, ws.kmax));
    GEMM(ws.ctx, H, lw.o_w, H, ws.y, H, H, H, lw.o_b, ws.x, H, OM_ACT_NONE);
    RUN(omk_layernorm(dt, ws.y, H, ws.x1, H, lw.ln1_g, lw.ln1_b, M, H, c->ln_eps, 0, s));
    GEMM(ws.x1, H, lw.ffn1_w, H, ws.ff, F1, F1, H, lw.ffn1_b, nullptr, 0, act1);
    NOMIC_SWIGLU(Mg);
    GEMM(ffa, F, lw.ffn2_w, F, ws.y, H, H, F, lw.ffn2_b, ws.x1, H, OM_ACT_NONE);
  }
  *out = EncStream{};
  if (c->n_layers > 0) *out = EncStream{ws.y, nullptr, 0, Ls[c->n_layers - 1].ln2_g, Ls[c->n_layers - 1].ln2_b, 0, ws.x};
  else out->hidden = ws.x;
  return 0;
}

static int modernbert(const EncCall& k, EncStream* out) {
  ENC_LOCALS;
  const float scale = 1.0f / sqrtf((float)c->head_dim);
  for (int l = 0; l < c->n_layers; ++l) {
    const OmLayerWeights& lw = Ls[l];
    if (!lw.ffn1g_w) OM_FAIL("ModernBERT layers need the gate half of Wi (ffn1g_w)");
    const void* a_in = ws.x;
    if (lw.ln1_g) {
      RUN(omk_layernorm(dt, ws.x, H, ws.y, H, lw.ln1_g, lw.ln1_b, M, H, c->ln_eps, 0, s));
      a_in = ws.y;
    }
    GEMM(a_in, H, lw.qkv_w, H, ws.qkv, 3 * H, 3 * H, H, lw.qkv_b, nullptr, 0, OM_ACT_NONE);
    const bool sliding = ((c->sliding_layers >> l) & 1) != 0;
    RUN(omk_rope(dt, ws.qkv, M, (int)L, H, sliding ? c->rope_theta_local : c->rope_theta_global, s));
    RUN(omk_attention(dt, ws.qkv, ws.ctx, k.mask, nullptr, B, (int)L, H, nh, scale, 0.f, 0, s, 0, ws.kmax, nullptr, sliding ? c->half_window : 0));
    GEMM(ws.ctx, H, lw.o_w, H, ws.x, H, H, H, lw.o_b, ws.x, H, OM_ACT_NONE);
    RUN(omk_layernorm(dt, ws.x, H, ws.y, H, lw.ln2_g, lw.ln2_b, M, H, c->ln_eps, 0, s));
    GEMM(ws.y, H, lw.ffn1g_w, H, ws.ff2, F, F, H, nullptr, nullptr, 0, OM_ACT_NONE);
    GEMM(ws.y, H, lw.ffn1_w, H, ws.ff, F, F, H, lw.ffn1_b, ws.ff2, F, c->act | OM_ACT_MUL_RESID);
    GEMM(ws.ff, F, lw.ffn2_w, F, ws.x, H, H, F, lw.ffn2_b, ws.x, H, OM_ACT_NONE);
  }
  *out = EncStream{ws.x, nullptr, 0, k.w->final_ln_g, k.w->final_ln_b, 0, ws.y};
  return 0;
}

static int t5_fused(const EncCall& k, EncStream* out) {
  ENC_LOCALS;
  const float inv_h = 1.0f / (float)H;
  const int nslots = 2 * (H / 256);
  auto folded = [&](int layer_, bool ffn1_, const void* A_, const void* W_, const float* g_, const float* stats_, void* C_, int N_, int act_,
                    const void* res_, int64_t ldr_) -> int {
    const void* wf; const float *cs, *bfp;
    if (folded_weights(c, k.w, layer_, ffn1_, W_, g_, nullptr, nullptr, N_, H, ws.wfold, ws.colsum, ws.bfold, s, &wf, &cs, &bfp)) return 1;
    (void)cs; (void)bfp;
    GemmEpilogue e = {};
    e.act = act_; e.resid = res_; e.ldr = ldr_;
    e.ln_stats = stats_; e.ln_rms = 1; e.ln_inv_h = inv_h; e.ln_eps = c->ln_eps; e.rows_dev = k.rows_dev;
    return omk_gemm(dt, A_, H, wf, H, dt, C_, N_, Mg, N_, H, e, s);
  };
  for (int l = 0; l < c->n_layers; ++l) {
    const OmLayerWeights& lw = Ls[l];
    float* st1 = ws.stats1 + (size_t)l * Mg * 2;
    float* st2 = ws.stats2 + (size_t)l * Mg * 2;
    if (l == 0) {
      RUN(omk_layernorm(dt, ws.x, H, ws.y, H, lw.ln1_g, nullptr, M, H, c->ln_eps, 1, s));
      GemmEpilogue e0 = {};
      e0.rows_dev = k.rows_dev;
      RUN(omk_gemm(dt, ws.y, H, lw.qkv_w, H, dt, ws.qkv, 3 * H, Mg, 3 * H, H, e0, s));
    } else {
      RUN(folded(l, false, ws.x, lw.qkv_w, lw.ln1_g, ws.stats2 + (size_t)(l - 1) * Mg * 2, ws.qkv, 3 * H, OM_ACT_NONE, nullptr, 0));
    }
    RUN(omk_attention(dt, ws.qkv, ws.ctx, k.mask, k.posbias, B, (int)L, H, nh, 1.0f, 0.f, 0, s, 0, ws.kmax, k.cu));
    GemmEpilogue e = {};
    e.resid = ws.x; e.ldr = H; e.stats_out = ws.slots; e.ln_inv_h = inv_h; e.ln_eps = c->ln_eps; e.rows_dev = k.rows_dev;
    RUN(omk_gemm(dt, ws.ctx, H, lw.o_w, H, dt, ws.x, H, Mg, H, H, e, s));
    RUN(omk_ln_stats_reduce(ws.slots, nslots, Mg, st1, s));
    RUN(folded(l, true, ws.x, lw.ffn1_w, lw.ln2_g, st1, ws.ff, F, c->act, nullptr, 0));
    e = GemmEpilogue{};
    e.resid = ws.x; e.ldr = H; e.stats_out = ws.slots; e.ln_inv_h = inv_h; e.ln_eps = c->ln_eps; e.rows_dev = k.rows_dev;
    RUN(omk_gemm(dt, ws.ff, F, lw.ffn2_w, F, dt, ws.x, H, Mg, H, F, e, s));
    RUN(omk_ln_stats_reduce(ws.slots, nslots, Mg, st2, s));
  }
  *out = EncStream{ws.x, nullptr, 0, k.w->final_ln_g, nullptr, 1, ws.y};
  return 0;
}

static int t5_plain(const EncCall& k, EncStream* out) {
  ENC_LOCALS;
  for (int l = 0; l < c->n_layers; ++l) {
    const OmLayerWeights& lw = Ls[l];
    RUN(omk_layernorm(dt, ws.x, H, ws.y, H, lw.ln1_g, nullptr, M, H, c->ln_eps, 1, s));
    GEMM(ws.y, H, lw.qkv_w, H, ws.qkv, 3 * H, 3 * H, H, nullptr, nullptr, 0, OM_ACT_NONE);
    RUN(omk_attention(dt, ws.qkv, ws.ctx, k.mask, k.posbias, B, (int)L, H, nh, 1.0f, 0.f, 0, s, 0, ws.kmax));
    GEMM(ws.ctx, H, lw.o_w, H, ws.x, H, H, H, nullptr, ws.x, H, OM_ACT_NONE);
    RUN(omk_layernorm(dt, ws.x, H, ws.y, H, lw.ln2_g, nullptr, M, H, c->ln_eps, 1, s));
    if (lw.ffn1g_w) {
      GEMM(ws.y, H, lw.ffn1g_w, H, ws.ff2, F, F, H, nullptr, nullptr, 0, OM_ACT_NONE);
      GEMM(ws.y, H, lw.ffn1_w, H, ws.ff, F, F, H, nullptr, ws.ff2, F, c->act | OM_ACT_MUL_RESID);
    } else {
      GEMM(ws.y, H, lw.ffn1_w, H, ws.ff, F, F, H, nullptr, nullptr, 0, c->act);
    }
    GEMM(ws.ff, F, lw.ffn2_w, F, ws.x, H, H, F, nullptr, ws.x, H, OM_ACT_NONE);
  }
  *out = EncStream{ws.x, nullptr, 0, k.w->final_ln_g, nullptr, 1, ws.y};
  return 0;
}

static int final_norm(const EncCall& k, const EncStream& n, char** hidden, const float** rows32, int64_t* n32) {
  const OmEncoderConfig* c = k.c; const EncWs& ws = k.ws; hipStream_t s = k.s;
  const int dt = c->dtype, H = c->hidden;
  const int64_t B = k.B, L = k.L, M = k.p.M;
  const bool pooled32 = dt != OM_F32 && c->pooling != OM_POOL_NONE;
  *hidden = n.hidden; *rows32 = ws.final32; *n32 = 0;
  if (!n.x) {
    if (n.rows32 && c->pooling != OM_POOL_NONE) { *rows32 = n.rows32; *n32 = M; }
    return 0;
  }
  if (k.out_hidden || !pooled32) {
    void* dst = k.out_hidden ? k.out_hidden : n.spare;
    RUN(omk_layernorm(dt, n.x, H, dst, H, n.g, n.b, M, H, c->ln_eps, n.rms, s, n.x_lo, n.lo8));
    *hidden = (char*)dst;
  }
  if (pooled32 && c->pooling == OM_POOL_FIRST) {
    const int* rows = k.cu && !n.cls_compact ? ws.cls_rows : nullptr;
    RUN(omk_layernorm_f32out(dt, n.x, rows || n.cls_compact ? H : L * H, ws.final32, H, n.g, n.b, B, H, c->ln_eps, n.rms, s, n.x_lo, rows, n.lo8));
    *n32 = B;
  } else if (pooled32) {
    RUN(omk_layernorm_f32out(dt, n.x, H, ws.final32, H, n.g, n.b, M, H, c->ln_eps, n.rms, s, n.x_lo, nullptr, n.lo8));
    *n32 = M;
  }
  return 0;
}

int omk_pooled_tail(const OmEncoderConfig* c, const OmEncoderWeights* w, const float* pooled, float* out_reps, int64_t B, const int* cu,
                    int64_t packed_rows, hipStream_t s) {
  int D = c->hidden;
  if (c->head_in > 0 && w->head_w) {
    D = c->head_out;
    RUN(om_gemm_nt(OM_F32, pooled, c->hidden, w->head_w, c->head_in, OM_F32, out_reps, D, B, D, c->head_in, nullptr, nullptr, 0, OM_ACT_NONE, s));
  }
  if (c->normalize) RUN(omk_l2norm(out_reps, out_reps, B, D, s));
  if (cu) RUN(omk_pack_overflow_poison(cu, B, packed_rows, out_reps, B * (int64_t)D, s));
  return 0;
}

static int skip_pad_buffer(hipStream_t s, size_t ints, int** out) {
  struct Buf { int* p = nullptr; size_t n = 0; bool captured = false; };
  static std::mutex mu;
  static std::map<std::pair<int, hipStream_t>, Buf> bufs;
  *out = nullptr;
  int dev = 0;
  OM_HIP(hipGetDevice(&dev));
  hipStreamCaptureStatus st = hipStreamCaptureStatusNone;
  if (hipStreamIsCapturing(s, &st) != hipSuccess) {
    (void)hipGetLastError();
    return 0;
  }
  const bool capturing = st != hipStreamCaptureStatusNone;
  std::lock_guard<std::mutex> lk(mu);
  Buf& b = bufs[std::make_pair(dev, s)];
  if (b.n < ints) {
    if (capturing) return 0;
    if (b.p && !b.captured) { OM_HIP(hipDeviceSynchronize()); OM_HIP(hipFree(b.p)); }
    b = Buf{};
    OM_HIP(hipMalloc(&b.p, ints * sizeof(int)));
    b.n = ints;
  }
  b.captured |= capturing;
  *out = b.p;
  return 0;
}

struct EncChain {
  const OmEncoderConfig* c;
  const OmEncoderWeights* w;
  const int64_t *input_ids, *attention_mask, *token_type_ids;
  void* out_hidden;
  float* out_reps;
  EncPlanIn in;
  EncPlan plan;
  EncSwitches sw;
  EncWs ws;
  hipStream_t s;
  int* side;
  int64_t whole_mg, whole_mc;
};

static EncWs lane_view(const OmEncoderConfig* c, const EncWs& w, const EncPlan& lane, int h, int64_t B0, int64_t L) {
  const size_t H = c->hidden, F = c->ffn, F1 = enc_ffn1_cols(c), es = 2;
  const size_t row0 = h ? (size_t)(B0 * L) : 0, seq0 = h ? (size_t)B0 : 0;
  EncWs v = {};
  v.x = w.x + row0 * H * es; v.y = w.y + row0 * H * es; v.x1 = w.x1 + row0 * H * es;
  v.qkv = w.qkv + row0 * 3 * H * es;
  v.ctx = w.ctx + row0 * H * es;
  v.ff = w.ff + row0 * F1 * es;
  v.ff2 = c->arch == OM_ARCH_NOMICBERT ? w.ff2 + row0 * F * es : w.ff2;
  v.y_lo = w.y_lo + row0 * H * es; v.x1_lo = w.x1_lo + row0 * H * es;
  v.pooled = w.pooled + seq0 * H;
  v.headout = w.headout + seq0 * (size_t)(c->head_out > 0 ? c->head_out : 1);
  v.kmax = w.kmax + seq0;
  v.final32 = w.final32 + (c->pooling == OM_POOL_FIRST ? seq0 : row0) * H;
  v.stats1 = w.stats1 + 4 * (size_t)c->n_layers * row0;
  v.stats2 = v.stats1 + (size_t)c->n_layers * (size_t)lane.Mg * 2;
  v.slots = w.slots + 4 * ((H + 255) / 256) * row0;
  v.total = w.total;
  return v;
}

static void lane_ranges(const OmEncoderConfig* c, const EncWs& v, const EncPlan& lane, int64_t Bh, const char* base, int64_t* out) {
  const size_t H = c->hidden, F = c->ffn, F1 = enc_ffn1_cols(c), es = 2, M = (size_t)lane.Mp, B = (size_t)Bh;
  const bool nomic = c->arch == OM_ARCH_NOMICBERT;
  const std::pair<const void*, size_t> f[OM_ENCODER_LANE_RANGES] = {
      {v.x, M * H * es}, {v.y, M * H * es}, {v.x1, M * H * es}, {v.qkv, M * 3 * H * es}, {v.ctx, M * H * es}, {v.ff, M * F1 * es},
      {v.ff2, nomic ? M * F * es : 0}, {v.pooled, B * H * 4}, {v.headout, B * (size_t)(c->head_out > 0 ? c->head_out : 1) * 4}, {v.kmax, B * 4},
      {v.final32, (c->pooling == OM_POOL_FIRST ? B : (size_t)lane.M) * H * 4}, {v.stats1, (size_t)2 * c->n_layers * M * 8},
      {v.slots, (size_t)2 * ((H + 255) / 256) * M * 8}, {v.y_lo, M * H * es}, {v.x1_lo, M * H * es}};
  for (int i = 0; i < OM_ENCODER_LANE_RANGES; ++i) {
    out[2 * i] = (int64_t)((const char*)f[i].first - base);
    out[2 * i + 1] = (int64_t)f[i].second;
  }
}

extern "C" int om_debug_encoder_lanes(const OmEncoderConfig* c, int gated_ffn, int has_rel_bias, int64_t B, int64_t L, int64_t packed_rows,
                                      int want_hidden, int64_t* B0) {
  if (!c) {
    om_set_error("om_debug_encoder_lanes: null argument");
    return -1;
  }
  const EncPlanIn in = {c, B, L, packed_rows, want_hidden != 0, gated_ffn != 0, has_rel_bias != 0, c->type_vocab > 0};
  const EncSwitches sw = encoder_switches();
  return encoder_lanes(in, encoder_plan(in, sw), sw, B0) ? 1 : 0;
}

extern "C" int om_debug_encoder_lane_ranges(const OmEncoderConfig* c, int gated_ffn, int has_rel_bias, int64_t B, int64_t L, int lane,
                                            int64_t* out, int cap) {
  if (!c || !out || cap < 2 * OM_ENCODER_LANE_RANGES || (lane != 0 && lane != 1)) {
    om_set_error("om_debug_encoder_lane_ranges: null argument, a lane other than 0 | 1, or room for fewer than 15 pairs");
    return -1;
  }
  EncPlanIn in = {c, B, L, 0, false, gated_ffn != 0, has_rel_bias != 0, c->type_vocab > 0};
  const EncSwitches sw = encoder_switches();
  const EncPlan whole = encoder_plan(in, sw);
  int64_t B0 = 0;
  if (!encoder_lanes(in, whole, sw, &B0)) {
    om_set_error("om_debug_encoder_lane_ranges: this call does not fork (om_debug_encoder_lanes)");
    return -1;
  }
  static char origin[1];
  const EncWs ws = carve(c, whole, B, L, 0, origin);
  in.B = lane ? B - B0 : B0;
  const EncPlan lp = encoder_plan_checked(in, sw);
  lane_ranges(c, lane_view(c, ws, lp, lane, B0, L), lp, in.B, origin, out);
  return OM_ENCODER_LANE_RANGES;
}

static std::atomic<int64_t> g_lane_forks{0};
extern "C" int64_t om_debug_encoder_lane_forks(void) { return g_lane_forks.load(); }

struct LaneStream { hipStream_t side = nullptr; hipEvent_t fork = nullptr, join = nullptr; };
static int lane_stream(hipStream_t s, LaneStream* out) {
  static std::mutex mu;
  static std::map<std::pair<int, hipStream_t>, LaneStream> lanes;
  int dev = 0;
  OM_HIP(hipGetDevice(&dev));
  std::lock_guard<std::mutex> lk(mu);
  LaneStream& l = lanes[std::make_pair(dev, s)];
  if (!l.side) {
    LaneStream n;
    OM_HIP(hipStreamCreateWithFlags(&n.side, hipStreamNonBlocking));
    OM_HIP(hipEventCreateWithFlags(&n.fork, hipEventDisableTiming));
    OM_HIP(hipEventCreateWithFlags(&n.join, hipEventDisableTiming));
    l = n;
  }
  *out = l;
  return 0;
}

static int encoder_chain(const EncChain& q, std::vector<int>* families);

static int encoder_fork(const EncChain& whole, int* forked) {
  *forked = 0;
  const OmEncoderConfig* c = whole.c;
  const int64_t B = whole.in.B, L = whole.in.L;
  int64_t B0 = 0;
  if (!whole.w->folded || om_timing_on() || !encoder_lanes(whole.in, whole.plan, whole.sw, &B0)) return 0;
  hipStreamCaptureStatus st = hipStreamCaptureStatusNone;
  if (hipStreamIsCapturing(whole.s, &st) != hipSuccess) {
    (void)hipGetLastError();
    return 0;
  }
  if (st != hipStreamCaptureStatusNone) return 0;
  LaneStream ls;
  RUN(lane_stream(whole.s, &ls));
  const bool skip = encoder_skip_pad(whole.in, whole.plan, whole.sw);
  int64_t whole_mc = 0;
  if (!encoder_cls_tail(whole.in, whole.plan, whole.sw, &whole_mc)) whole_mc = 0;
  const int64_t D =c->head_in > 0 && whole.w->head_w ? c->head_out : c->hidden;
  EncChain lane[2] = {whole, whole};
  for (int h = 0; h < 2; ++h) {
    EncChain& q = lane[h];
    const int64_t seq0 = h ? B0 : 0;
    q.in.B = h ? B - B0 : B0;
    q.plan = encoder_plan_checked(q.in, q.sw);
    q.ws = lane_view(c, whole.ws, q.plan, h, B0, L);
    q.input_ids += seq0 * L; q.attention_mask += seq0 * L;
    if (q.token_type_ids) q.token_type_ids += seq0 * L;
    q.out_reps += seq0 * D;
    if (h) q.s = ls.side;
    q.whole_mg = whole.plan.Mg; q.whole_mc = whole_mc;
    q.side = nullptr;
    if (skip) {
      RUN(skip_pad_buffer(q.s, (size_t)(q.plan.Mp + 2 * q.in.B + 2), &q.side));
      if (!q.side) return 0;
    }
  }
  if (lane[0].plan.Mp != B0 * L || lane[0].plan.Mp + lane[1].plan.Mp != whole.plan.Mp) return 0;
  EncChain ask = whole;
  ask.side = lane[0].side;
  std::vector<int> fam_whole, fam_lane[2];
  if (encoder_chain(ask, &fam_whole) || encoder_chain(lane[0], &fam_lane[0]) || encoder_chain(lane[1], &fam_lane[1])) return 0;
  if (fam_lane[0] != fam_whole || fam_lane[1] != fam_whole || std::find_if(fam_whole.begin(), fam_whole.end(), [](int f) { return f <= 0; }) != fam_whole.end())
    return 0;

  OM_HIP(hipEventRecord(ls.fork, whole.s));
  OM_HIP(hipStreamWaitEvent(ls.side, ls.fork, 0));
  *forked = 1;
  g_lane_forks.fetch_add(1);
  int rc = encoder_chain(lane[0], nullptr);
  if (!rc) rc = encoder_chain(lane[1], nullptr);
  hipError_t e = hipEventRecord(ls.join, ls.side);
  if (e == hipSuccess) e = hipStreamWaitEvent(whole.s, ls.join, 0);
  if (e != hipSuccess) {
    (void)hipStreamSynchronize(ls.side);
    if (!rc) OM_FAIL(std::string("encoder lanes: join failed: ") + hipGetErrorString(e));
  }
  return rc;
}

static int encoder_forward_impl(const OmEncoderConfig* c, const OmEncoderWeights* w,
                                const int64_t* input_ids, const int64_t* attention_mask,
                                const int64_t* token_type_ids, int64_t B, int64_t L,
                                void* out_hidden, float* out_reps, void* workspace,
                                size_t workspace_bytes, void* stream, int64_t packed_rows) {
  if (!c || !w || !input_ids || !attention_mask) OM_FAIL("null argument");
  if (check_cfg(c)) return 1;
  if (B <= 0) return 0;
  const OmLayerWeights* Ls = w->layers_host;
  if (!Ls) OM_FAIL("layers_host is null");
  const EncPlanIn plan_in = {c, B, L, packed_rows, out_hidden != nullptr, c->n_layers > 0 && Ls[0].ffn1g_w != nullptr, w->rel_bias != nullptr,
                             w->type_emb != nullptr};
  const EncSwitches sw = encoder_switches();
  const EncPlan plan = encoder_plan_checked(plan_in, sw);
  if (om_option(OM_OPT_ENCODER_DEBUG) && plan.path && enc_bert_family(c))
    fprintf(stderr, "om_encoder_forward: M=%ld fused_ln=%d packed=%d few_rows=%d pending_ln=%d L=%ld head_dim=%d rel_bias=%d\n", (long)plan.M,
            (int)(plan.path == OM_ENC_PATH_BERT_FUSED), (int)(packed_rows > 0), (int)plan.few_rows, (int)(plan.path == OM_ENC_PATH_BERT_PENDING_LN), (long)L,
            c->head_dim, (int)plan.rel_bias);
  if (om_option(OM_OPT_ENCODER_DEBUG) && plan.path && c->arch == OM_ARCH_T5)
    fprintf(stderr, "om_encoder_forward (t5): M=%ld fused_norm=%d packed=%d\n", (long)plan.M, (int)(plan.path == OM_ENC_PATH_T5_FUSED), (int)(packed_rows > 0));
  if (plan.error) OM_FAIL(plan.error);
  if (c->arch == OM_ARCH_T5 && !w->final_ln_g) OM_FAIL("T5 needs rel_bias and final_ln_g");
  if (c->arch == OM_ARCH_MODERNBERT && (!w->emb_ln_g || !w->final_ln_g)) OM_FAIL("ModernBERT needs emb_ln_g and final_ln_g");
  if (c->arch == OM_ARCH_NOMICBERT && (!w->type_emb || w->pos_emb || w->rel_bias)) OM_FAIL("NomicBERT needs type_emb and takes no pos_emb or rel_bias");
  if (!workspace || ((uintptr_t)workspace & 255)) OM_FAIL("workspace must be 256-byte aligned");
  EncChain whole = {c, w, input_ids, attention_mask, token_type_ids, out_hidden, out_reps, plan_in, plan, sw,
                    carve(c, plan, B, L, packed_rows, (char*)workspace), (hipStream_t)stream, nullptr, 0, 0};
  if (whole.ws.total > workspace_bytes) OM_FAIL("workspace too small");
  if (c->pooling != OM_POOL_NONE && !out_reps) OM_FAIL("out_reps required when pooling is set");
  int forked = 0;
  RUN(encoder_fork(whole, &forked));
  if (forked) return 0;
  if (encoder_skip_pad(plan_in, plan, sw)) RUN(skip_pad_buffer(whole.s, (size_t)(plan.Mp + 2 * B + 2), &whole.side));
  return encoder_chain(whole, nullptr);
}

static int encoder_chain(const EncChain& q, std::vector<int>* families) {
  const OmEncoderConfig* c = q.c; const OmEncoderWeights* w = q.w;
  const int64_t *input_ids = q.input_ids, *attention_mask = q.attention_mask, *token_type_ids = q.token_type_ids;
  void* const out_hidden = q.out_hidden; float* const out_reps = q.out_reps;
  const EncPlanIn& plan_in = q.in; const EncPlan& plan = q.plan; const EncSwitches sw = q.sw;
  const int64_t B = q.in.B, L = q.in.L, packed_rows = q.in.packed_rows;
  const bool bert = enc_bert_family(c);
  EncWs ws = q.ws;
  hipStream_t s = q.s;
  const int dt = c->dtype, H = c->hidden;
  const int64_t M = plan.M;
  int64_t pack_bound = packed_rows;
  const bool skip = q.side != nullptr;
  if (skip) {
    pack_bound = plan.Mp;
    ws.cu = q.side; ws.cls_rows = q.side + (B + 2); ws.row_map = ws.cls_rows + B;
  }
  const bool packed = pack_bound > 0;
  int64_t cls_mc = 0;
  if (!encoder_cls_tail(plan_in, plan, sw, &cls_mc)) cls_mc = 0;
  const int* const row_map = packed ? ws.row_map : nullptr;
  if (families) {
    if (plan.path != OM_ENC_PATH_BERT_FUSED) OM_FAIL("encoder lanes: the fused BERT path only");
    const EncCall k = {c, w, attention_mask, B, L, plan, ws, nullptr, packed ? ws.cu : nullptr, row_map, out_hidden, s, skip ? ws.cu + B : nullptr,
                       cls_mc, families, q.whole_mg, q.whole_mc};
    EncStream unused = {};
    RUN(bert_fused(k, &unused));
    if (c->head_in > 0 && w->head_w)
      families->push_back(omk_gemm_family(OM_F32, ws.pooled, c->hidden, w->head_w, c->head_in, OM_F32, out_reps, c->head_out, B, c->head_out,
                                          c->head_in, GemmEpilogue{}));
    return 0;
  }

  RUN(omk_mask_extent(attention_mask, B, (int)L, ws.kmax, s));
  if (packed) RUN(omk_pack_rows(ws.kmax, B, (int)L, pack_bound, ws.cu, ws.cls_rows, ws.row_map, s));
  if (plan.rel_bias) {
    const int* lut = nullptr;
    RUN(om_t5_lut_device((int)L, c->rel_buckets, c->rel_max_dist, &lut));
    RUN(omk_t5_bias(w->rel_bias, lut, ws.posbias, (int)L, c->n_heads, s));
  }
  const bool few32 = plan.path == OM_ENC_PATH_BERT_FEW32 || plan.path == OM_ENC_PATH_BERT_PENDING_LN;
  if (bert)
    RUN(omk_embed(dt, input_ids, token_type_ids, w->word_emb, w->pos_emb, w->type_emb, w->emb_ln_g, w->emb_ln_b, ws.x, M, (int)L, H,
                  c->vocab, c->type_vocab, c->ln_eps, 1, s, row_map, few32 ? ws.r32a : nullptr));
  else if (c->arch == OM_ARCH_MODERNBERT)
    RUN(omk_embed(dt, input_ids, nullptr, w->word_emb, nullptr, nullptr, w->emb_ln_g, w->emb_ln_b, ws.x, M, (int)L, H, c->vocab, 1, c->ln_eps, 1, s));
  else
    RUN(omk_embed(dt, input_ids, nullptr, w->word_emb, nullptr, nullptr, nullptr, nullptr, ws.x, M, (int)L, H, c->vocab, 1, c->ln_eps, 0, s, row_map));

  const EncCall k = {c, w, attention_mask, B, L, plan, ws, plan.rel_bias ? ws.posbias : nullptr, packed ? ws.cu : nullptr, row_map, out_hidden, s,
                     skip ? ws.cu + B : nullptr, cls_mc, nullptr, q.whole_mg, q.whole_mc};
  EncStream stream_out = {};
  switch (plan.path) {
    case OM_ENC_PATH_BERT_FUSED: RUN(bert_fused(k, &stream_out)); break;
    case OM_ENC_PATH_BERT_PENDING_LN: RUN(bert_pending_ln(k, &stream_out)); break;
    case OM_ENC_PATH_BERT_FEW32: RUN(bert_few32(k, &stream_out)); break;
    case OM_ENC_PATH_BERT_PLAIN: RUN(bert_plain(k, &stream_out)); break;
    case OM_ENC_PATH_MODERNBERT: RUN(modernbert(k, &stream_out)); break;
    case OM_ENC_PATH_T5_FUSED: RUN(t5_fused(k, &stream_out)); break;
    case OM_ENC_PATH_T5_PLAIN: RUN(t5_plain(k, &stream_out)); break;
    default: OM_FAIL("no path planned");
  }
  char* final_hidden;
  const float* f32_rows;
  int64_t final32_rows;
  RUN(final_norm(k, stream_out, &final_hidden, &f32_rows, &final32_rows));

  if (c->pooling != OM_POOL_NONE) {
    float* pooled = c->head_in > 0 && w->head_w ? ws.pooled : out_reps;
    if (final32_rows == B && c->pooling == OM_POOL_FIRST && (f32_rows == ws.final32 || L == 1))
      OM_HIP(hipMemcpyAsync(pooled, f32_rows, (size_t)B * H * 4, hipMemcpyDeviceToDevice, s));
    else if (final32_rows == M)
      RUN(omk_pool(OM_F32, f32_rows, attention_mask, pooled, B, (int)L, H, c->pooling, s, k.cu));
    else
      RUN(omk_pool(dt, final_hidden, attention_mask, pooled, B, (int)L, H, c->pooling, s));
    RUN(omk_pooled_tail(c, w, pooled, out_reps, B, k.cu, pack_bound, s));
  }
  return 0;
}
#undef NOMIC_SWIGLU
#undef NOMIC_ROPE
#undef NOMIC_LOCALS
#undef ENC_LOCALS
#undef GEMM
#undef RUN

extern "C" int om_encoder_forward(const OmEncoderConfig* c, const OmEncoderWeights* w,
                                  const int64_t* input_ids, const int64_t* attention_mask,
                                  const int64_t* token_type_ids, int64_t B, int64_t L,
                                  void* out_hidden, float* out_reps, void* workspace,
                                  size_t workspace_bytes, void* stream) {
  return encoder_forward_impl(c, w, input_ids, attention_mask, token_type_ids, B, L, out_hidden, out_reps, workspace, workspace_bytes, stream, 0);
}

extern "C" int om_encoder_forward_packed(const OmEncoderConfig* c, const OmEncoderWeights* w,
                                         const int64_t* input_ids, const int64_t* attention_mask,
                                         const int64_t* token_type_ids, int64_t B, int64_t L, int64_t packed_rows,
                                         float* out_reps, void* workspace, size_t workspace_bytes, void* stream) {
  if (packed_rows <= 0) OM_FAIL("packed_rows must be positive");
  return encoder_forward_impl(c, w, input_ids, attention_mask, token_type_ids, B, L, nullptr, out_reps, workspace, workspace_bytes, stream, packed_rows);
}
```

### openmatch_amd/csrc/encoder_plan.h

```cpp
#pragma once
#include <algorithm>

#include "kernels.h"

bool omk_gemm_skinny_ok(int in_dtype, int out_dtype, int64_t M, int64_t N, int64_t K, const GemmEpilogue& ep, int max_m);

struct EncSwitches {
  int fused_ln;
  int two_plane;
  int pingpong;
  int skinny_m;
  int few_ln_fuse;
  int attention_fast;
  int skip_pad;
  int cls_tail;
  int lanes;
};

static EncSwitches encoder_switches() {
  return EncSwitches{om_option(OM_OPT_ENCODER_FUSED_LN), om_option(OM_OPT_ENCODER_TWO_PLANE), om_option(OM_OPT_ENCODER_PINGPONG),
                     om_option(OM_OPT_GEMM_SKINNY_M), om_option(OM_OPT_FEW_ROWS_LN_FUSE), om_option(OM_OPT_ATTENTION_FAST),
                     om_option(OM_OPT_ENCODER_SKIP_PAD), om_option(OM_OPT_ENCODER_CLS_TAIL), om_option(OM_OPT_ENCODER_LANES)};
}

struct EncPlanIn {
  const OmEncoderConfig* c;
  int64_t B, L, packed_rows;
  bool want_hidden;
  bool gated_ffn, has_rel_bias, has_type_emb;
};

struct EncPlan {
  int path;
  const char* error;
  int64_t M;
  int64_t Mp;
  int64_t Mg;
  bool few_rows;
  bool two;
  int lo8;
  bool pingpong;
  bool rel_bias;
  bool alloc_few32;
};

static const char* encoder_cfg_error(const OmEncoderConfig* c) {
  if (c->dtype != OM_F32 && c->dtype != OM_BF16 && c->dtype != OM_F16) return "dtype must be OM_F32, OM_BF16 or OM_F16";
  if (c->dtype == OM_F16 && c->arch == OM_ARCH_BERT && c->act != OM_ACT_GELU_ERF) return "float16 mode: erf-GELU BERT-family encoders only";
  if (c->dtype == OM_F16 && c->arch == OM_ARCH_T5 && c->act != OM_ACT_RELU && c->act != OM_ACT_GELU_TANH)
    return "float16 mode: T5 feed-forwards with ReLU or tanh-GELU only";
  if (c->arch != OM_ARCH_BERT && c->arch != OM_ARCH_T5 && c->arch != OM_ARCH_MODERNBERT && c->arch != OM_ARCH_NOMICBERT) return "unknown arch";
  if (c->arch == OM_ARCH_NOMICBERT) {
    if (c->head_dim != 64 || c->n_heads * 64 != c->hidden) return "NomicBERT: only head_dim 64 with n_heads*64 == hidden is supported";
    if (c->act != OM_ACT_SILU) return "NomicBERT: hidden_act must be \"silu\"";
    if (!(c->rope_theta_global > 0.f)) return "NomicBERT: a positive rope theta";
    if (c->rel_buckets != 0) return "NomicBERT: no relative position bias (rel_buckets must be 0)";
    if (c->hidden % 64 || c->ffn % 64 || c->ffn < 64) return "NomicBERT: hidden and ffn must be multiples of 64";
  }
  if (c->arch == OM_ARCH_MODERNBERT) {
    if (c->head_dim != 64 || c->n_heads * 64 != c->hidden) return "ModernBERT: only head_dim 64 with n_heads*64 == hidden is supported";
    if (c->act != OM_ACT_GELU_ERF) return "ModernBERT: hidden_activation must be \"gelu\" (erf)";
    if (c->n_layers > 64) return "ModernBERT: at most 64 layers";
    if (!(c->rope_theta_global > 0.f) || !(c->rope_theta_local > 0.f) || c->half_window < 0)
      return "ModernBERT: positive rope thetas and a non-negative half window";
  }
  if (c->arch == OM_ARCH_T5 && (c->head_dim != 64 || c->n_heads * 64 != c->hidden))
    return "T5 encoders: only d_kv 64 with n_heads*64 == d_model is supported";
  if ((c->head_dim != 32 && c->head_dim != 64) || c->n_heads * c->head_dim != c->hidden)
    return "head_dim must be 32 or 64 with n_heads*head_dim == hidden";
  if (c->arch == OM_ARCH_BERT && c->rel_buckets != 0 && (c->rel_buckets < 4 || c->rel_buckets % 2 || c->rel_max_dist <= c->rel_buckets / 4))
    return "relative position bias: an even number of buckets >= 4 and a maximum distance beyond the exact buckets";
  const int es = c->dtype == OM_F32 ? 4 : 2;
  if ((c->hidden * es) % 128 || (c->ffn * es) % 128) return "hidden/ffn rows must be multiples of 128 bytes";
  if (c->head_in > 0 && ((c->head_in * 4) % 128 || c->head_in != c->hidden)) return "head_in must equal hidden";
  return nullptr;
}

static inline bool enc_bert_family(const OmEncoderConfig* c) { return c->arch == OM_ARCH_BERT || c->arch == OM_ARCH_NOMICBERT; }
static inline int enc_ffn1_cols(const OmEncoderConfig* c) { return c->arch == OM_ARCH_NOMICBERT ? 2 * c->ffn : c->ffn; }

static bool enc_ln_fusable(int dt, int64_t rows, int H, int F, int F1) {
  return omk_gemm_ln_fusable(dt, rows, H, H) && omk_gemm_ln_fusable(dt, rows, F1, H) && omk_gemm_ln_fusable(dt, rows, 3 * H, H) &&
         omk_gemm_ln_fusable(dt, rows, H, F);
}

static bool enc_pending_ln_ok(int dt, int64_t M, int H, int F, int F1, int act, int max_m) {
  static const float one = 1.f;
  GemmEpilogue a = {}, r = {};
  a.a_ln32 = &one; a.a_ln_g = &one; a.a_ln_b = &one;
  r.rln32 = &one; r.rln32_stats = &one; r.rln_g = &one; r.rln_b = &one; r.out32 = const_cast<float*>(&one);
  GemmEpilogue f = a;
  f.act = act;
  return omk_gemm_skinny_ok(dt, dt, M, 3 * (int64_t)H, H, a, max_m) && omk_gemm_skinny_ok(dt, dt, M, F1, H, f, max_m) &&
         omk_gemm_skinny_ok(dt, dt, M, H, H, r, max_m) && omk_gemm_skinny_ok(dt, dt, M, H, F, r, max_m);
}

static EncPlan encoder_plan_checked(const EncPlanIn& in, const EncSwitches sw) {
  const OmEncoderConfig* c = in.c;
  EncPlan p = {};
  auto run = [&](int path) { p.path = path; return p; };
  auto refuse = [&](const char* why) { p.error = why; return p; };
  const int dt = c->dtype, H = c->hidden, F = c->ffn, F1 = enc_ffn1_cols(c);
  const bool half = dt == OM_BF16 || dt == OM_F16, packed = in.packed_rows > 0, bert = enc_bert_family(c), nomic = c->arch == OM_ARCH_NOMICBERT;
  p.M = packed ? in.packed_rows : in.B * in.L;
  p.Mp = half && p.M >= 512 ? (p.M + 255) / 256 * 256 : p.M;
  p.alloc_few32 = half && bert && !packed && p.M <= (int64_t)std::max(0, sw.skinny_m);
  if (in.B <= 0) return p;
  if (in.L < 1 || in.L > 1024) return refuse("sequence length must be in [1,1024]");
  if (packed) {
    if (dt == OM_F32 || in.want_hidden || c->pooling == OM_POOL_NONE || c->n_layers < 1)
      return refuse("packed rows: 16-bit inference that returns representations only");
    if (in.packed_rows % 256 || in.packed_rows < 512 || in.packed_rows > in.B * in.L + 255)
      return refuse("packed_rows: a multiple of 256 in [512, B * L + 255]");
  }
  p.few_rows = !packed && half && p.M <= (int64_t)sw.skinny_m && !(dt == OM_BF16 && bert && p.M >= 512 && (sw.two_plane & 1) != 0);
  p.Mg = p.few_rows ? p.M : p.Mp;
  const bool fusable = sw.fused_ln != 0 && !p.few_rows && c->n_layers > 0 && H % 8 == 0 && enc_ln_fusable(dt, p.Mg, H, F, F1);
  if (c->arch == OM_ARCH_MODERNBERT) {
    if (packed) return refuse("packed rows: not for ModernBERT (om_encoder_packed_supported is 0)");
    return run(OM_ENC_PATH_MODERNBERT);
  }
  if (!bert) {
    if (!in.has_rel_bias) return refuse("T5 needs rel_bias and final_ln_g");
    p.rel_bias = true;
    p.path = fusable && !in.gated_ffn ? OM_ENC_PATH_T5_FUSED : OM_ENC_PATH_T5_PLAIN;
    if (packed && p.path != OM_ENC_PATH_T5_FUSED) return refuse("packed rows need the fused 16-bit path (T5: widths of 256, no gated feed-forward)");
    return p;
  }
  if (in.L > c->max_pos) return refuse(nomic ? "NomicBERT: sequence longer than max_pos (max_position_embeddings)" : "sequence longer than the position table");
  if (in.has_rel_bias != (c->rel_buckets > 0)) return refuse("relative position bias: rel_bias and rel_buckets must be set together");
  if (in.has_type_emb && c->type_vocab <= 0) return refuse("token types: a type_emb table needs type_vocab > 0");
  p.rel_bias = in.has_rel_bias;
  const bool plane = (sw.two_plane & (dt == OM_BF16 ? 1 : 2)) != 0;
  if (fusable && (c->act == OM_ACT_GELU_ERF || nomic)) {
    p.two = plane;
    p.lo8 = plane && dt == OM_F16 && (sw.two_plane & 4) ? 1 : 0;
    p.pingpong = sw.pingpong != 0;
    return run(OM_ENC_PATH_BERT_FUSED);
  }
  const bool few32 = p.few_rows && c->n_layers > 0 && plane;
  p.path = !few32 ? OM_ENC_PATH_BERT_PLAIN
           : p.M <= (int64_t)sw.few_ln_fuse && enc_pending_ln_ok(dt, p.Mg, H, F, F1, nomic ? OM_ACT_NONE : c->act, sw.skinny_m) ? OM_ENC_PATH_BERT_PENDING_LN
                                                                                                       : OM_ENC_PATH_BERT_FEW32;
  if (packed) return refuse("packed rows need the fused 16-bit path (hidden, ffn multiples of 256; erf-GELU)");
  return p;
}

static EncPlan encoder_plan(const EncPlanIn& in, const EncSwitches sw) {
  if (const char* why = encoder_cfg_error(in.c)) {
    EncPlan p = {};
    p.error = why;
    return p;
  }
  return encoder_plan_checked(in, sw);
}

static bool encoder_packed_ok(const OmEncoderConfig* c, bool gated_ffn, int64_t B, int64_t L, int64_t packed_rows, const EncSwitches sw) {
  if (!c || B <= 0 || packed_rows <= 0) return false;
  if ((c->dtype != OM_BF16 && c->dtype != OM_F16) || (!enc_bert_family(c) && c->arch != OM_ARCH_T5)) return false;
  if (B * L <= (int64_t)sw.skinny_m) return false;
  if (c->dtype == OM_BF16 && !sw.attention_fast) return false;
  if (c->arch == OM_ARCH_T5 && c->dtype == OM_F16 && c->act != OM_ACT_RELU) return false;
  OmEncoderConfig q = *c;
  q.pooling = OM_POOL_FIRST;
  q.max_pos = 1024;
  const bool rel = c->arch == OM_ARCH_T5 || c->rel_buckets > 0;
  const EncPlan p = encoder_plan_checked(EncPlanIn{&q, B, L, packed_rows, false, gated_ffn, rel, false}, sw);
  return p.path && !p.error;
}

static bool encoder_skip_pad(const EncPlanIn& in, const EncPlan& p, const EncSwitches sw) {
  if (!sw.skip_pad || in.packed_rows != 0 || in.want_hidden || in.c->pooling == OM_POOL_NONE) return false;
  if (p.error || (p.path != OM_ENC_PATH_BERT_FUSED && p.path != OM_ENC_PATH_T5_FUSED)) return false;
  return encoder_packed_ok(in.c, in.gated_ffn, in.B, in.L, p.Mp, sw);
}

static bool encoder_cls_tail(const EncPlanIn& in, const EncPlan& p, const EncSwitches sw, int64_t* Mc = nullptr) {
  if (!sw.cls_tail || p.error || p.path != OM_ENC_PATH_BERT_FUSED || p.lo8) return false;
  if (in.c->pooling != OM_POOL_FIRST || in.want_hidden || in.c->n_layers < 2 || in.B < 512) return false;
  const int64_t mc = (in.B + 255) / 256 * 256;
  if (4 * mc > p.Mp) return false;
  if (Mc) *Mc = mc;
  return true;
}

static const int64_t ENC_LANE_ROWS_END = 131072;
static bool encoder_lanes(const EncPlanIn& in, const EncPlan& p, const EncSwitches sw, int64_t* B0 = nullptr) {
  if (sw.lanes <= 0 || in.packed_rows != 0 || in.want_hidden || in.has_rel_bias || in.c->pooling == OM_POOL_NONE) return false;
  if (p.error || p.path != OM_ENC_PATH_BERT_FUSED || p.rel_bias || in.B < 2 || in.L < 1) return false;
  int64_t step = 256;
  for (int64_t l = in.L; step > 1 && l % 2 == 0; l /= 2) step /= 2;
  const int64_t b0 = in.B / 2 / step * step;
  if (b0 <= 0 || b0 * in.L < (int64_t)sw.lanes || (in.B - b0) * in.L < (int64_t)sw.lanes) return false;
  if ((in.B - b0) * in.L >= ENC_LANE_ROWS_END) return false;
  const bool skip = encoder_skip_pad(in, p, sw), tail = encoder_cls_tail(in, p, sw);
  for (const int64_t bh : {b0, in.B - b0}) {
    EncPlanIn li = in;
    li.B = bh;
    const EncPlan lp = encoder_plan_checked(li, sw);
    if (lp.error || lp.path != p.path || lp.two != p.two || lp.lo8 != p.lo8 || lp.pingpong != p.pingpong) return false;
    if (encoder_skip_pad(li, lp, sw) != skip || encoder_cls_tail(li, lp, sw) != tail) return false;
  }
  if (B0) *B0 = b0;
  return true;
}
```

### openmatch_amd/csrc/kernels.h

```cpp
#pragma once
#include "common.h"

int omk_ln_fold(int dtype , const void* W, const float* gamma, const float* beta, const float* b, void* Wf,
                float* colsum, float* bf, int N, int K, hipStream_t s);
int omk_layernorm(int dtype, const void* x, int64_t ldx, void* y, int64_t ldy, const float* g,
                  const float* b, int64_t M, int H, float eps, int rms, hipStream_t s,
                  const void* x_lo = nullptr ,
                  int lo8 = 0 );
int omk_layernorm_dual(int dtype, const float* x, int64_t ldx, void* y, float* y32, int64_t ldy, const float* g, const float* b,
                       int64_t M, int H, float eps, hipStream_t s);
int omk_layernorm_f32out(int dtype, const void* x, int64_t ldx, float* y, int64_t ldy, const float* g, const float* b,
                         int64_t M, int H, float eps, int rms, hipStream_t s, const void* x_lo = nullptr,
                         const int* rows = nullptr ,
                         int lo8 = 0 );
int omk_layernorm_from_f32(int dtype, const float* x, int64_t ldx, void* y, int64_t ldy, const float* g, const float* b, int64_t M, int H,
                           float eps, int rms, hipStream_t s);
int omk_embed(int dtype, const int64_t* ids, const int64_t* type_ids, const float* word,
              const float* pos, const float* type, const float* g, const float* b, void* out,
              int64_t M, int L, int H, int vocab, int type_vocab, float eps, int bert,
              hipStream_t s, const int* row_map = nullptr ,
              float* out32 = nullptr );
int omk_pool(int dtype, const void* x, const int64_t* mask, float* out, int64_t B, int L, int H,
             int mode, hipStream_t s, const int* cu = nullptr );
int omk_l2norm(const float* x, float* y, int64_t M, int D, hipStream_t s);
int omk_swiglu_rows(int dtype, const void* in, void* out, int64_t M, int F, hipStream_t s);
void omk_row_note(int word);
int omk_t5_bias(const float* table, const int* lut, float* out, int L, int heads, hipStream_t s);

int omk_attention(int dtype, const void* qkv, void* ctx, const int64_t* mask,
                  const float* pos_bias, int64_t B, int L, int H, int heads, float scale,
                  float drop_p, uint64_t seed, hipStream_t s, int reverse = 0 ,
                  const int* kmax = nullptr ,
                  const int* cu = nullptr ,
                  int w = 0 );
struct AttnPlan;
int omk_attention_d32(const AttnPlan& p, int dtype, const void* qkv, void* ctx, const int64_t* mask, const float* pos_bias, int64_t B, int L,
                      int H, int heads, float scale, float drop_p, uint64_t seed, hipStream_t s, int reverse, const int* kmax, const int* cu);
int omk_rope(int dtype, void* qkv, int64_t M, int L, int H, float theta, hipStream_t s,
             const int* row_map = nullptr );
int omk_attention_band(int dtype, const void* qkv, void* ctx, const int64_t* mask, int64_t B, int L, int H, int heads, float scale,
                       int w, const int* kmax, hipStream_t s);
int omk_rope_gqa(int dtype, void* qkv, int64_t M, int L, int heads, int kv_heads, const float* inv_freq_host, float scaling, hipStream_t s,
                 const int* row_map = nullptr );
int omk_attention_causal(int dtype, const void* qkv, void* ctx, const int64_t* mask, int64_t B, int L, int heads, int kv_heads, float scale,
                         const int* kmax, hipStream_t s);
int omk_attention_causal_packed(int dtype, const void* qkv, void* ctx, const int64_t* mask, int64_t B, int L, int heads, int kv_heads, float scale,
                                const int* cu, hipStream_t s);
int omk_attention_causal_d128(int dtype, const void* qkv, void* ctx, const int64_t* mask, int64_t B, int L, int heads, int kv_heads, float scale,
                              const int* kmax, hipStream_t s);
int omk_attention_causal_d128_packed(int dtype, const void* qkv, void* ctx, const int64_t* mask, int64_t B, int L, int heads, int kv_heads,
                                     float scale, const int* cu, hipStream_t s);
int omk_qknorm_rope(int dtype, void* qkv, int64_t M, int L, int heads, int kv_heads, int head_dim, const float* q_norm_g, const float* k_norm_g,
                    float eps, const float* inv_freq_host, float scaling, hipStream_t s, const int* row_map = nullptr,
                    int gemma = 0 );
int omk_attention_gqa_d256(int dtype, const void* qkv, void* ctx, const int64_t* mask, int64_t B, int L, int heads, int kv_heads, float scale, int w,
                           const int* kmax, hipStream_t s);
int omk_attention_gqa_d256_packed(int dtype, const void* qkv, void* ctx, const int64_t* mask, int64_t B, int L, int heads, int kv_heads, float scale,
                                  int w, const int* cu, hipStream_t s);
int omk_rmsnorm_add(int dtype, const void* h, int64_t ldh, float* x, int64_t ldx, const float* g, int64_t M, int H, float eps, hipStream_t s);
int omk_rope_table(const float* inv_freq, int n, float scaling, const float2** out);
int omk_causal_debug_kmax(int64_t B, int** out);
int omk_pack_rows(const int* kmax, int64_t B, int L, int64_t rows, int* cu, int* cls_rows, int* row_map, hipStream_t s);
int omk_pack_overflow_poison(const int* cu, int64_t B, int64_t rows, float* out, int64_t n, hipStream_t s);
int omk_mask_extent(const int64_t* mask, int64_t B, int L, int* kmax, hipStream_t s);
int omk_pooled_tail(const OmEncoderConfig* c, const OmEncoderWeights* w, const float* pooled, float* out_reps, int64_t B, const int* cu,
                    int64_t packed_rows, hipStream_t s);

#define OM_ACT_GELU_ERF_GRAD 4
struct GemmEpilogue {
  const float* bias;
  const void* resid;
  int64_t ldr;
  int act;
  void* pre_act;
  int64_t ldp;
  float drop_p;
  uint64_t seed;
  const int* drop_rows;
  unsigned long long* trace;
  const float* ln_stats;
  const float* ln_colsum;
  const float* rln_stats;
  const float* rln_g;
  const float* rln_b;
  float* stats_out;
  const void* resid_lo;
  void* out_lo;
  const float* resid32;
  float* out32;
  const float* a_ln32;
  const float* a_ln_g;
  const float* a_ln_b;
  float* a_ln_stats_out;
  const float* rln32;
  const float* rln32_stats;
  int lo8;
  float ln_inv_h, ln_eps;
  int ln_rms;
  int reverse;
  const int* rows_dev;
};
__host__ __device__ inline size_t omk_lo8_offset(int64_t m, int64_t n, int64_t N) {
  const int64_t tile = (m >> 8) * (N >> 8) + (n >> 8);
  const int wave = (int)(((m >> 7) & 1) * 2 + ((n >> 7) & 1));
  const int r = (int)(m & 127), c = (int)(n & 127);
  const int P = 2 * (r >> 5) + (c >> 6);
  const int G = 2 * ((r >> 4) & 1) + ((c >> 5) & 1);
  const int lane = ((c >> 2) & 3) * 16 + (r & 15);
  return ((size_t)((tile * 4 + wave) * 8 + P)) * 2048 + (size_t)((G >> 1) * 1024 + lane * 16 + (G & 1) * 8 + ((c >> 4) & 1) * 4 + (c & 3));
}
int omk_ln_stats_reduce(const float* slots, int nslots, int64_t M, float* out, hipStream_t s);
struct GatherPlane { const void* src; void* dst; };
int omk_gather_rows(const GatherPlane (&planes)[3], const float* stats_src, float* stats_dst, const int* rows, int64_t B, int64_t L, int64_t Mc,
                    int H, hipStream_t s);
struct GemmPlan { int family; const char* error; int act ; bool resid, train ; int lnf ; };
inline int gemm_lnf(const GemmEpilogue& ep, bool f16) {
  return ep.ln_stats ? 1 : ((ep.rln_stats || ep.stats_out) ? (ep.out_lo ? (ep.lo8 && f16 ? 4 : 3) : 2) : 0);
}
inline bool gemm_whole_tiles(int64_t M, int64_t N, int64_t K) { return M % 256 == 0 && N % 256 == 0 && (K * 2) % 128 == 0; }
bool omk_gemm_ln_fusable(int dtype, int64_t M, int64_t N, int64_t K);
unsigned long long* omk_debug_trace();
bool omk_gemm_tn_ok(int dtype, int64_t M, int64_t N, int64_t K, int64_t lda, int64_t ldb);
int omk_gemm_tn(int dtype, const void* A, int64_t lda, const void* B, int64_t ldb, float* C, int64_t ldc, float* bias,
                int64_t M, int64_t N, int64_t K, hipStream_t s);
bool omk_gemm_tn_batch_ok(int dtype, int64_t M, int64_t N, int64_t K, int64_t lda, int64_t ldb);
int omk_gemm_tn_batch(int dtype, const OmTnProblem* probs, int n, int64_t M, hipStream_t s);
bool omk_gemm_wide6_b16_has(int in_dtype, int out_dtype, int act, bool train, bool resid);
int omk_gemm_wide6_b16(int in_dtype, const void* A, int64_t lda, const void* B, int64_t ldb, int out_dtype,
                       void* C, int64_t ldc, int64_t M, int64_t N, int64_t K, const GemmEpilogue& ep, hipStream_t s);
bool omk_gemm_wide6_f32_has(int in_dtype, int out_dtype, int act, bool train, bool resid);
int omk_gemm_wide6_f32(int in_dtype, const void* A, int64_t lda, const void* B, int64_t ldb, int out_dtype,
                       void* C, int64_t ldc, int64_t M, int64_t N, int64_t K, const GemmEpilogue& ep, hipStream_t s);
int omk_gemm(int in_dtype, const void* A, int64_t lda, const void* B, int64_t ldb, int out_dtype,
             void* C, int64_t ldc, int64_t M, int64_t N, int64_t K, const GemmEpilogue& ep,
             hipStream_t s, int64_t plan_m = 0);
int omk_gemm_family(int in_dtype, const void* A, int64_t lda, const void* B, int64_t ldb, int out_dtype, const void* C, int64_t ldc, int64_t M,
                    int64_t N, int64_t K, const GemmEpilogue& ep, int64_t plan_m = 0);
void omk_gemm_note(int family);

int omk_gemm_splitk(int in_dtype, const void* A, int64_t lda, const void* B, int64_t ldb, float* C,
                    int64_t ldc, int64_t M, int64_t N, int64_t K, hipStream_t s);

__host__ __device__ inline uint64_t om_hash64(uint64_t seed, uint64_t idx) {
  uint64_t x = idx * 0x9E3779B97F4A7C15ull + seed;
  x ^= x >> 32; x *= 0xD6E8FEB86659FD93ull;
  x ^= x >> 32; x *= 0xD6E8FEB86659FD93ull;
  x ^= x >> 32;
  return x;
}
struct DropCfg {
  uint32_t thresh;
  float keep_scale;
  __host__ __device__ explicit DropCfg(float p) {
    thresh = p > 0.f ? (uint32_t)(p * 65536.0f + 0.5f) : 0u;
    if (thresh > 65535u) thresh = 65535u;
    keep_scale = 65536.0f / (float)(65536u - thresh);
  }
};
__host__ __device__ inline uint64_t dropout_bits(uint64_t seed, uint64_t group) { return om_hash64(seed, group); }
__host__ __device__ inline bool dropout_field(uint64_t bits, int e, uint32_t thresh) {
  return ((uint32_t)(bits >> (16 * e)) & 0xffffu) >= thresh;
}
__host__ __device__ inline bool dropout_keep(uint64_t seed, uint64_t idx, uint32_t thresh) {
  return dropout_field(dropout_bits(seed, idx >> 2), (int)(idx & 3), thresh);
}
```

### openmatch_amd/native.py

```python
import ctypes as C
import os

import torch

_HERE = os.path.dirname(os.path.abspath(__file__))
LIB_PATH = os.path.join(_HERE, "csrc", "libopenmatch_hip.so")

OM_F32, OM_BF16, OM_F16 = 0, 1, 2
ACT_NONE, ACT_GELU_ERF, ACT_RELU, ACT_GELU_TANH = 0, 1, 2, 3
ACT_SILU = 5
ACT_MUL_RESID = 0x100
ACT_GELU_ERF_GRAD, ACT_PRE_GRAD = 4, 0x200
ARCH_BERT, ARCH_T5, ARCH_MODERNBERT, ARCH_CAUSAL, ARCH_NOMICBERT, ARCH_GEMMA3 = 0, 1, 2, 3, 4, 5
POOL_NONE, POOL_FIRST, POOL_MEAN, POOL_LAST = 0, 1, 2, 3
OPT_TRAIN_WGRAD_BATCH, OPT_GEMM_MAX_GRID, OPT_GEMM_CONT = 14, 15, 16
OPT_WGRAD_DEBUG = 5
OPT_GEMM_GROUP_M, OPT_GEMM_VARIANT, OPT_GEMM_SKINNY_M = 6, 12, 19
GEMM_FAMILY = {"v1": 1, "v2": 2, "v6": 6, "g7": 7, "g7_one_tile": 70, "7c16": 71, "7r16": 72, "skinny": 9}
ATTN_FAMILY = {"generic": 1, "fwd16": 2, "fwd16_kmax4": 3, "fwd16c": 4, "long": 5, "d32": 6, "band16": 7, "band32": 8}
ATTN_BWD_FAMILY = {"bwd16": 1, "generic": 2, "long": 3, "d32": 4}
ENC_PATH = {"bert_fused": 1, "bert_pending_ln": 2, "bert_few32": 3, "bert_plain": 4, "modernbert": 5, "t5_fused": 6, "t5_plain": 7}
SCAN_FAMILY = {"dense": 0, "generic": 1, "wide": 2, "stream32": 3, "stream16": 4}
SCAN_FAMILY_NAME = {v: k for k, v in SCAN_FAMILY.items()}
SCAN_KERNEL = {"dense": 0, "tile2": 1, "tile6": 2, "wide7": 3, "wide7c": 4, "stream": 5}
SCAN_KERNEL_NAME = {v: k for k, v in SCAN_KERNEL.items()}
OPT_SCAN_GEN7 = 3
OPT_ATTENTION_FAST = 2
SEARCH_F32, SEARCH_F16_RESCORE, SEARCH_F16_ONLY = 0, 1, 2
ABI_VERSION = 6

c_void_p, c_int, c_int64, c_float, c_size_t = C.c_void_p, C.c_int, C.c_int64, C.c_float, C.c_size_t


class OmLayerWeights(C.Structure):
    _fields_ = [(n, c_void_p) for n in (
        "qkv_w", "qkv_b", "o_w", "o_b", "ln1_g", "ln1_b", "ffn1_w", "ffn1_b", "ffn1g_w",
        "ffn2_w", "ffn2_b", "ln2_g", "ln2_b")]


class OmEncoderConfig(C.Structure):
    _fields_ = [("arch", c_int), ("dtype", c_int), ("hidden", c_int), ("n_layers", c_int),
                ("n_heads", c_int), ("head_dim", c_int), ("ffn", c_int), ("vocab", c_int),
                ("max_pos", c_int), ("type_vocab", c_int), ("act", c_int), ("ln_eps", c_float),
                ("rel_buckets", c_int), ("rel_max_dist", c_int), ("pooling", c_int),
                ("head_in", c_int), ("head_out", c_int), ("normalize", c_int),
                ("rope_theta_global", c_float), ("rope_theta_local", c_float), ("half_window", c_int),
                ("sliding_layers", C.c_uint64)]


class OmCausalConfig(C.Structure):
    _fields_ = [("base", OmEncoderConfig), ("n_kv_heads", c_int), ("rope_attention_scaling", c_float), ("inv_freq", c_float * 32)]


class OmCausalConfig2(C.Structure):
    _fields_ = [("base", OmCausalConfig), ("qk_norm", c_int), ("reserved", c_int), ("inv_freq", c_float * 64)]


class OmCausalQkNorm(C.Structure):
    _fields_ = [("q_norm_g", c_void_p), ("k_norm_g", c_void_p)]


class OmGemma3Config(C.Structure):
    _fields_ = [("base", OmCausalConfig), ("attn_scale", c_float), ("half_window", c_int), ("sliding_layers", C.c_uint64),
                ("full_scaling", c_float), ("sliding_scaling", c_float), ("attn_logit_softcapping", c_float), ("bidirectional", c_int),
                ("full_inv_freq", c_float * 128), ("sliding_inv_freq", c_float * 128)]


class OmGemma3Norms(C.Structure):
    _fields_ = [(n, c_void_p) for n in ("q_norm_g", "k_norm_g", "post_attention_norm_g", "post_feedforward_norm_g")]


class OmEncoderWeights(C.Structure):
    _fields_ = [("word_emb", c_void_p), ("pos_emb", c_void_p), ("type_emb", c_void_p),
                ("emb_ln_g", c_void_p), ("emb_ln_b", c_void_p),
                ("layers_host", C.POINTER(OmLayerWeights)), ("final_ln_g", c_void_p),
                ("rel_bias", c_void_p), ("head_w", c_void_p), ("folded", c_void_p), ("final_ln_b", c_void_p)]


class OmTnProblem(C.Structure):
    _fields_ = [("A", c_void_p), ("B", c_void_p), ("C", c_void_p), ("bias", c_void_p),
                ("lda", c_int64), ("ldb", c_int64), ("ldc", c_int64), ("N", c_int64), ("K", c_int64)]


class OmT5DecoderLayer(C.Structure):
    _fields_ = [(n, c_void_p) for n in (
        "sa_v_w", "sa_o_w", "sa_ln_g", "ca_q_w", "ca_kv_w", "ca_o_w", "ca_ln_g", "ffn1_w", "ffn1g_w", "ffn2_w", "ffn_ln_g")]


class OmT5DecoderWeights(C.Structure):
    _fields_ = [("start_emb", c_void_p), ("final_ln_g", c_void_p),
                ("layers_host", C.POINTER(OmT5DecoderLayer)), ("n_layers", c_int)]


class OmT5DecoderLayerGrads(C.Structure):
    _fields_ = [(n, c_void_p) for n in (
        "sa_v_w", "sa_o_w", "sa_ln_g", "ca_q_w", "ca_kv_w", "ca_o_w", "ca_ln_g", "ffn1_w", "ffn1g_w", "ffn2_w", "ffn_ln_g")]


class OmT5DecoderGrads(C.Structure):
    _fields_ = [("start_emb", c_void_p), ("final_ln_g", c_void_p), ("layers_host", C.POINTER(OmT5DecoderLayerGrads))]


class OmAdamTensor(C.Structure):
    _fields_ = [("p", c_void_p), ("g", c_void_p), ("m", c_void_p), ("v", c_void_p), ("shadow0", c_void_p), ("shadow1", c_void_p),
                ("n", c_int64), ("weight_decay", c_float), ("shadow0_dtype", c_int), ("shadow1_dtype", c_int), ("reserved", c_int)]


class OmDebugGemmEpilogue(C.Structure):
    _fields_ = [("bias", c_void_p), ("resid", c_void_p), ("ldr", c_int64), ("act", c_int),
                ("pre_act", c_void_p), ("ldp", c_int64), ("drop_p", c_float), ("seed", C.c_uint64), ("drop_rows", c_void_p),
                ("ln_stats", c_void_p), ("ln_colsum", c_void_p), ("rln_stats", c_void_p), ("rln_g", c_void_p), ("rln_b", c_void_p),
                ("stats_out", c_void_p), ("resid_lo", c_void_p), ("out_lo", c_void_p), ("resid32", c_void_p), ("out32", c_void_p),
                ("a_ln32", c_void_p), ("a_ln_g", c_void_p), ("a_ln_b", c_void_p), ("a_ln_stats_out", c_void_p), ("rln32", c_void_p),
                ("rln32_stats", c_void_p), ("lo8", c_int), ("ln_inv_h", c_float), ("ln_eps", c_float), ("ln_rms", c_int),
                ("reverse", c_int), ("rows_dev", c_void_p)]


class OmLnSite(C.Structure):
    _fields_ = [("partial", c_void_p), ("dg", c_void_p), ("db", c_void_p), ("blocks", c_int)]


ROW_KERNEL = {"fwd_generic": 1, "fwd_x8": 2, "ln_bwd": 3}
OPT_TRAIN_WGRAD_STREAM = 8
ADAM_CHUNK = 16384


class OmLayerGrads(C.Structure):
    _fields_ = [(n, c_void_p) for n in (
        "qkv_w", "qkv_b", "o_w", "o_b", "ln1_g", "ln1_b", "ffn1_w", "ffn1_b", "ffn2_w", "ffn2_b",
        "ln2_g", "ln2_b", "ffn1g_w")]


class OmEncoderGrads(C.Structure):
    _fields_ = [("word_emb", c_void_p), ("pos_emb", c_void_p), ("type_emb", c_void_p),
                ("emb_ln_g", c_void_p), ("emb_ln_b", c_void_p),
                ("layers_host", C.POINTER(OmLayerGrads)), ("head_w", c_void_p),
                ("final_ln_g", c_void_p), ("rel_bias", c_void_p)]


_SIGNATURES = {
    "om_last_error": (C.c_char_p, []),
    "om_abi_version": (c_int, []),
    "om_device_count": (c_int, []),
    "om_debug_gemm_trace": (None, [c_void_p]),
    "om_debug_gemm_gen": (None, [c_int]),
    "om_debug_option": (c_int, [c_int, c_int]),
    "om_debug_option_value": (c_int, [c_int]),
    "om_debug_gemm_last": (c_int, []),
    "om_debug_gemm_plan": (c_int, [c_int, c_void_p, c_int64, c_void_p, c_int64, c_int, c_void_p, c_int64,
                                   c_int64, c_int64, c_int64, c_void_p, c_void_p, c_int64, c_int]),
    "om_debug_gemm_ex": (c_int, [c_int, c_void_p, c_int64, c_void_p, c_int64, c_int, c_void_p, c_int64,
                                 c_int64, c_int64, c_int64, C.POINTER(OmDebugGemmEpilogue), c_void_p]),
    "om_debug_gemm_plan_ex": (c_int, [c_int, c_void_p, c_int64, c_void_p, c_int64, c_int, c_void_p, c_int64,
                                      c_int64, c_int64, c_int64, C.POINTER(OmDebugGemmEpilogue)]),
    "om_debug_gemm_splitk": (c_int, [c_int, c_void_p, c_int64, c_void_p, c_int64, c_void_p, c_int64, c_int64, c_int64, c_int64, c_void_p]),
    "om_debug_attention": (c_int, [c_void_p, c_void_p, c_void_p, c_int64, c_int, c_int, c_int, c_void_p]),
    "om_debug_attention_ex": (c_int, [c_int, c_void_p, c_void_p, c_void_p, c_void_p, c_int64, c_int, c_int, c_int, c_float, c_float,
                                      C.c_uint64, c_void_p, c_int, c_void_p, c_void_p, c_int]),
    "om_debug_rope": (c_int, [c_int, c_void_p, c_int64, c_int, c_int, c_float, c_void_p]),
    "om_debug_rope_rows": (c_int, [c_int, c_void_p, c_int64, c_int, c_int, c_float, c_void_p, c_void_p]),
    "om_debug_swiglu_rows": (c_int, [c_int, c_void_p, c_void_p, c_int64, c_int, c_void_p]),
    "om_debug_embed": (c_int, [c_int, c_void_p, c_void_p, c_void_p, c_void_p, c_void_p, c_void_p, c_void_p, c_void_p, c_int64, c_int, c_int,
                               c_int, c_int, c_float, c_void_p]),
    "om_debug_attention_causal": (c_int, [c_int, c_void_p, c_void_p, c_void_p, c_int64, c_int, c_int, c_int, c_float, c_void_p]),
    "om_debug_rope_gqa": (c_int, [c_int, c_void_p, c_int64, c_int, c_int, c_int, C.POINTER(c_float), c_float, c_void_p]),
    "om_debug_attention_causal_packed": (c_int, [c_int, c_void_p, c_void_p, c_void_p, c_void_p, c_int64, c_int, c_int, c_int, c_float, c_void_p]),
    "om_debug_rope_gqa_rows": (c_int, [c_int, c_void_p, c_int64, c_int, c_int, c_int, C.POINTER(c_float), c_float, c_void_p, c_void_p]),
    "om_debug_attention_causal_hd": (c_int, [c_int, c_void_p, c_void_p, c_void_p, c_int64, c_int, c_int, c_int, c_int, c_float, c_void_p]),
    "om_debug_attention_causal_hd_packed": (c_int, [c_int, c_void_p, c_void_p, c_void_p, c_void_p, c_int64, c_int, c_int, c_int, c_int, c_float,
                                                    c_void_p]),
    "om_debug_qknorm_rope": (c_int, [c_int, c_void_p, c_int64, c_int, c_int, c_int, c_int, c_void_p, c_void_p, c_float, C.POINTER(c_float),
                                     c_float, c_void_p]),
    "om_debug_qknorm_rope_rows": (c_int, [c_int, c_void_p, c_int64, c_int, c_int, c_int, c_int, c_void_p, c_void_p, c_float, C.POINTER(c_float),
                                          c_float, c_void_p, c_void_p]),
    "om_debug_attention_gqa_d256": (c_int, [c_int, c_void_p, c_void_p, c_void_p, c_int64, c_int, c_int, c_int, c_float, c_int, c_void_p]),
    "om_debug_qknorm_rope_d256": (c_int, [c_int, c_void_p, c_int64, c_int, c_int, c_int, c_void_p, c_void_p, c_float, C.POINTER(c_float), c_float,
                                          c_void_p]),
    "om_debug_attention_gqa_d256_packed": (c_int, [c_int, c_void_p, c_void_p, c_void_p, c_void_p, c_int64, c_int, c_int, c_int, c_float, c_int,
                                                   c_void_p]),
    "om_debug_qknorm_rope_d256_rows": (c_int, [c_int, c_void_p, c_int64, c_int, c_int, c_int, c_void_p, c_void_p, c_float, C.POINTER(c_float),
                                               c_float, c_void_p, c_void_p]),
    "om_debug_rmsnorm_add": (c_int, [c_int, c_void_p, c_int64, c_void_p, c_int64, c_void_p, c_int64, c_int, c_float, c_void_p]),
    "om_debug_mask_extent": (c_int, [c_void_p, c_int64, c_int, c_void_p, c_void_p]),
    "om_debug_pack_rows": (c_int, [c_void_p, c_int64, c_int, c_int64, c_void_p, c_void_p, c_void_p, c_void_p]),
    "om_debug_attention_last": (c_int, []),
    "om_debug_attention_plan": (c_int, [c_int, c_int64, c_int, c_int, c_int, c_int, c_float, c_int, c_int, c_int]),
    "om_debug_attention_bwd_last": (c_int, []),
    "om_debug_attention_bwd_plan": (c_int, [c_int, c_int64, c_int, c_int, c_int, c_int, c_int, c_int, c_int]),
    "om_debug_attention_bwd_ex": (c_int, [c_int, c_void_p, c_void_p, c_void_p, c_void_p, c_void_p, c_void_p, c_void_p, c_void_p, c_int64, c_int,
                                          c_int, c_int, c_float, c_float, C.c_uint64, c_void_p, c_int, c_void_p]),
    "om_debug_attention_bwd_stats_bytes": (c_size_t, [c_int64, c_int]),
    "om_debug_encoder_plan": (c_int, [C.POINTER(OmEncoderConfig), c_int, c_int, c_int64, c_int64, c_int64, c_int]),
    "om_debug_encoder_skip_pad": (c_int, [C.POINTER(OmEncoderConfig), c_int, c_int, c_int64, c_int64, c_int]),
    "om_debug_encoder_cls_tail": (c_int, [C.POINTER(OmEncoderConfig), c_int, c_int, c_int64, c_int64, c_int64, c_int]),
    "om_debug_encoder_lanes": (c_int, [C.POINTER(OmEncoderConfig), c_int, c_int, c_int64, c_int64, c_int64, c_int, C.POINTER(c_int64)]),
    "om_debug_encoder_lane_ranges": (c_int, [C.POINTER(OmEncoderConfig), c_int, c_int, c_int64, c_int64, c_int, C.POINTER(c_int64), c_int]),
    "om_debug_encoder_lane_forks": (c_int64, []),
    "om_debug_gather_rows": (c_int, [c_void_p, c_void_p, c_void_p, c_void_p, c_void_p, c_void_p, c_void_p, c_void_p, c_void_p, c_int64, c_int64,
                                     c_int64, c_int, c_void_p]),
    "om_debug_attn_drop_keep": (c_int, [C.c_uint64, c_int64, c_int, c_int, c_int, c_int, c_int, c_float]),
    "om_debug_wave_sum_check": (c_int, [c_void_p, c_void_p, c_void_p, c_int64, c_void_p]),
    "om_debug_row_kernel_last": (c_int, []),
    "om_debug_layernorm": (c_int, [c_int, c_void_p, c_int64, c_void_p, c_int64, c_void_p, c_void_p, c_int64, c_int, c_float, c_int, c_void_p,
                                   c_int, c_void_p]),
    "om_debug_layernorm_f32out": (c_int, [c_int, c_void_p, c_int64, c_void_p, c_int64, c_void_p, c_void_p, c_int64, c_int, c_float, c_int,
                                          c_void_p, c_void_p, c_int, c_void_p]),
    "om_debug_layernorm_from_f32": (c_int, [c_int, c_void_p, c_int64, c_void_p, c_int64, c_void_p, c_void_p, c_int64, c_int, c_float, c_int,
                                            c_void_p]),
    "om_debug_layernorm_dual": (c_int, [c_int, c_void_p, c_int64, c_void_p, c_void_p, c_int64, c_void_p, c_void_p, c_int64, c_int, c_float,
                                        c_void_p]),
    "om_debug_norm_bwd": (c_int, [c_int, c_void_p, c_void_p, c_void_p, c_void_p, c_void_p, c_void_p, c_int64, c_int, c_float, c_int, c_void_p,
                                  c_void_p]),
    "om_debug_ln_bwd_drop": (c_int, [c_int, c_void_p, c_void_p, c_void_p, c_void_p, c_void_p, c_float, C.c_uint64, c_void_p, c_void_p, c_int64,
                                     c_int, c_float, c_void_p, c_void_p, c_void_p, C.POINTER(c_int), c_void_p, c_void_p]),
    "om_debug_ln_param_reduce": (c_int, [C.POINTER(OmLnSite), c_int, c_int, c_void_p]),
    "om_debug_embed_bwd": (c_int, [c_int, c_void_p, c_void_p, c_void_p, c_void_p, c_void_p, c_void_p, c_void_p, c_void_p, c_void_p, c_void_p,
                                   c_void_p, c_void_p, c_int64, c_int, c_int, c_int, c_int, c_float, c_void_p, c_void_p]),
    "om_debug_pool": (c_int, [c_int, c_void_p, c_void_p, c_void_p, c_int64, c_int, c_int, c_int, c_void_p, c_void_p]),
    "om_debug_pool_bwd": (c_int, [c_int, c_void_p, c_void_p, c_void_p, c_int64, c_int, c_int, c_int, c_void_p, c_void_p]),
    "om_debug_l2norm": (c_int, [c_void_p, c_void_p, c_int64, c_int, c_void_p]),
    "om_debug_l2norm_bwd": (c_int, [c_void_p, c_void_p, c_void_p, c_int64, c_int, c_void_p]),
    "om_debug_colsum": (c_int, [c_int, c_void_p, c_int64, c_int64, c_int, c_void_p, c_void_p]),
    "om_debug_dropout": (c_int, [c_int, c_void_p, c_void_p, c_int64, c_float, C.c_uint64, c_void_p, c_int, c_void_p]),
    "om_debug_ln_fold": (c_int, [c_int, c_void_p, c_void_p, c_void_p, c_void_p, c_void_p, c_void_p, c_void_p, c_int, c_int, c_void_p]),
    "om_debug_ln_stats_reduce": (c_int, [c_void_p, c_int, c_int64, c_void_p, c_void_p]),
    "om_encoder_fold_bytes": (c_size_t, [C.POINTER(OmEncoderConfig)]),
    "om_encoder_fold_weights": (c_int, [C.POINTER(OmEncoderConfig), C.POINTER(OmEncoderWeights), c_void_p, c_size_t, c_void_p]),
    "om_kernel_timing_enable": (c_int, [c_int]),
    "om_kernel_timing_read": (c_int, [c_int, C.POINTER(C.c_double), C.POINTER(c_int64), C.POINTER(C.c_double)]),
    "om_gemm_nt": (c_int, [c_int, c_void_p, c_int64, c_void_p, c_int64, c_int, c_void_p, c_int64,
                           c_int64, c_int64, c_int64, c_void_p, c_void_p, c_int64, c_int, c_void_p]),
    "om_gemm_tn_acc": (c_int, [c_int, c_void_p, c_int64, c_void_p, c_int64, c_void_p, c_int64, c_void_p,
                               c_int64, c_int64, c_int64, c_void_p]),
    "om_gemm_tn_acc_batch": (c_int, [c_int, C.POINTER(OmTnProblem), c_int, c_int64, c_void_p]),
    "om_debug_gemm_tn_last": (c_int, [C.POINTER(c_int64)]),
    "om_debug_gemm_tn_plan": (c_int, [c_int, c_int64, c_int64, c_int64, c_int64, c_int64, c_int, C.POINTER(c_int64)]),
    "om_debug_transpose": (c_int, [c_int, c_void_p, c_int64, c_int64, c_int, c_void_p, c_int64, c_int64, c_int, c_void_p]),
    "om_debug_transpose_batch": (c_int, [c_int, C.POINTER(c_void_p), C.POINTER(c_void_p), C.POINTER(c_int), C.POINTER(c_int), c_int, c_void_p]),
    "om_debug_zero_rows_from": (c_int, [c_void_p, c_int64, c_void_p, c_int64, c_void_p]),
    "om_debug_t5_act_fwd": (c_int, [c_int, c_void_p, c_void_p, c_void_p, c_int64, c_int, c_void_p]),
    "om_debug_t5_act_bwd": (c_int, [c_int, c_void_p, c_void_p, c_void_p, c_void_p, c_void_p, c_int64, c_int, c_void_p]),
    "om_debug_t5_embed_bwd": (c_int, [c_int, c_void_p, c_void_p, c_void_p, c_int64, c_int, c_int, c_void_p, c_void_p]),
    "om_debug_t5_bias": (c_int, [c_void_p, c_void_p, c_void_p, c_int, c_int, c_void_p]),
    "om_debug_t5_bias_bwd": (c_int, [c_void_p, c_void_p, c_void_p, c_int, c_int, c_void_p]),
    "om_encoder_workspace_bytes": (c_size_t, [C.POINTER(OmEncoderConfig), c_int64, c_int64]),
    "om_t5_decoder_workspace_bytes": (c_size_t, [C.POINTER(OmEncoderConfig), c_int64, c_int64]),
    "om_t5_decoder_step": (c_int, [C.POINTER(OmEncoderConfig), C.POINTER(OmT5DecoderWeights), c_void_p, c_void_p,
                                   c_int64, c_int64, c_void_p, c_void_p, c_size_t, c_void_p]),
    "om_t5_relative_bucket": (c_int, [c_int, c_int, c_int]),
    "om_encoder_forward": (c_int, [C.POINTER(OmEncoderConfig), C.POINTER(OmEncoderWeights), c_void_p,
                                   c_void_p, c_void_p, c_int64, c_int64, c_void_p, c_void_p,
                                   c_void_p, c_size_t, c_void_p]),
    "om_causal_encoder_workspace_bytes": (c_size_t, [C.POINTER(OmCausalConfig), c_int64, c_int64]),
    "om_causal_encoder_forward": (c_int, [C.POINTER(OmCausalConfig), C.POINTER(OmEncoderWeights), c_void_p, c_void_p, c_int64, c_int64,
                                          c_void_p, c_void_p, c_void_p, c_size_t, c_void_p]),
    "om_causal_encoder_packed_supported": (c_int, [C.POINTER(OmCausalConfig), c_int64, c_int64, c_int64]),
    "om_causal_encoder_workspace_bytes_packed": (c_size_t, [C.POINTER(OmCausalConfig), c_int64, c_int64, c_int64]),
    "om_causal_encoder_forward_packed": (c_int, [C.POINTER(OmCausalConfig), C.POINTER(OmEncoderWeights), c_void_p, c_void_p, c_int64, c_int64,
                                                 c_int64, c_void_p, c_void_p, c_size_t, c_void_p]),
    "om_causal2_encoder_workspace_bytes": (c_size_t, [C.POINTER(OmCausalConfig2), c_int64, c_int64]),
    "om_causal2_encoder_forward": (c_int, [C.POINTER(OmCausalConfig2), C.POINTER(OmEncoderWeights), C.POINTER(OmCausalQkNorm), c_void_p, c_void_p,
                                           c_int64, c_int64, c_void_p, c_void_p, c_void_p, c_size_t, c_void_p]),
    "om_causal2_encoder_packed_supported": (c_int, [C.POINTER(OmCausalConfig2), c_int64, c_int64, c_int64]),
    "om_causal2_encoder_workspace_bytes_packed": (c_size_t, [C.POINTER(OmCausalConfig2), c_int64, c_int64, c_int64]),
    "om_causal2_encoder_forward_packed": (c_int, [C.POINTER(OmCausalConfig2), C.POINTER(OmEncoderWeights), C.POINTER(OmCausalQkNorm), c_void_p,
                                                  c_void_p, c_int64, c_int64, c_int64, c_void_p, c_void_p, c_size_t, c_void_p]),
    "om_gemma3_encoder_workspace_bytes": (c_size_t, [C.POINTER(OmGemma3Config), c_int64, c_int64]),
    "om_gemma3_encoder_forward": (c_int, [C.POINTER(OmGemma3Config), C.POINTER(OmEncoderWeights), C.POINTER(OmGemma3Norms), c_void_p, c_void_p,
                                          c_int64, c_int64, c_void_p, c_void_p, c_void_p, c_size_t, c_void_p]),
    "om_gemma3_encoder_packed_supported": (c_int, [C.POINTER(OmGemma3Config), c_int64, c_int64, c_int64]),
    "om_gemma3_encoder_workspace_bytes_packed": (c_size_t, [C.POINTER(OmGemma3Config), c_int64, c_int64, c_int64]),
    "om_gemma3_encoder_forward_packed": (c_int, [C.POINTER(OmGemma3Config), C.POINTER(OmEncoderWeights), C.POINTER(OmGemma3Norms), c_void_p,
                                                 c_void_p, c_int64, c_int64, c_int64, c_void_p, c_void_p, c_size_t, c_void_p]),
    "om_encoder_packed_supported": (c_int, [C.POINTER(OmEncoderConfig), c_int, c_int64, c_int64, c_int64]),
    "om_encoder_workspace_bytes_packed": (c_size_t, [C.POINTER(OmEncoderConfig), c_int64, c_int64, c_int64]),
    "om_encoder_forward_packed": (c_int, [C.POINTER(OmEncoderConfig), C.POINTER(OmEncoderWeights), c_void_p,
                                          c_void_p, c_void_p, c_int64, c_int64, c_int64, c_void_p,
                                          c_void_p, c_size_t, c_void_p]),
    "om_encoder_tape_bytes": (c_size_t, [C.POINTER(OmEncoderConfig), c_int64, c_int64]),
    "om_encoder_train_workspace_bytes": (c_size_t, [C.POINTER(OmEncoderConfig), c_int64, c_int64]),
    "om_encoder_train_forward": (c_int, [C.POINTER(OmEncoderConfig), C.POINTER(OmEncoderWeights), c_void_p,
                                         c_void_p, c_void_p, c_int64, c_int64, c_float, c_float, C.c_uint64,
                                         c_void_p, c_size_t, c_void_p, c_void_p, c_size_t, c_void_p]),
    "om_encoder_train_backward": (c_int, [C.POINTER(OmEncoderConfig), C.POINTER(OmEncoderWeights), c_void_p,
                                          c_void_p, c_void_p, c_int64, c_int64, c_float, c_float, C.c_uint64,
                                          c_void_p, c_void_p, C.POINTER(OmEncoderGrads), c_void_p, c_size_t,
                                          c_void_p]),
    "om_encoder_train_packed_supported": (c_int, [C.POINTER(OmEncoderConfig), c_int64, c_int64, c_int64]),
    "om_encoder_tape_bytes_packed": (c_size_t, [C.POINTER(OmEncoderConfig), c_int64, c_int64, c_int64]),
    "om_encoder_train_workspace_bytes_packed": (c_size_t, [C.POINTER(OmEncoderConfig), c_int64, c_int64, c_int64]),
    "om_encoder_train_forward_packed": (c_int, [C.POINTER(OmEncoderConfig), C.POINTER(OmEncoderWeights), c_void_p,
                                                c_void_p, c_void_p, c_int64, c_int64, c_int64, c_float, c_float, C.c_uint64,
                                                c_void_p, c_size_t, c_void_p, c_void_p, c_size_t, c_void_p]),
    "om_encoder_train_backward_packed": (c_int, [C.POINTER(OmEncoderConfig), C.POINTER(OmEncoderWeights), c_void_p,
                                                 c_void_p, c_void_p, c_int64, c_int64, c_int64, c_float, c_float, C.c_uint64,
                                                 c_void_p, c_void_p, C.POINTER(OmEncoderGrads), c_void_p, c_size_t,
                                                 c_void_p]),
    "om_encoder_train_forward_hidden": (c_int, [C.POINTER(OmEncoderConfig), C.POINTER(OmEncoderWeights), c_void_p,
                                                c_void_p, c_void_p, c_int64, c_int64, c_float, c_float, C.c_uint64,
                                                c_void_p, c_size_t, c_void_p, c_void_p, c_size_t, c_void_p]),
    "om_encoder_train_backward_hidden": (c_int, [C.POINTER(OmEncoderConfig), C.POINTER(OmEncoderWeights), c_void_p,
                                                 c_void_p, c_void_p, c_int64, c_int64, c_float, c_float, C.c_uint64,
                                                 c_void_p, c_void_p, C.POINTER(OmEncoderGrads), c_void_p, c_size_t,
                                                 c_void_p]),
    "om_t5_decoder_tape_bytes": (c_size_t, [C.POINTER(OmEncoderConfig), c_int, c_int64, c_int64]),
    "om_t5_decoder_train_workspace_bytes": (c_size_t, [C.POINTER(OmEncoderConfig), c_int, c_int64, c_int64]),
    "om_t5_decoder_train_forward": (c_int, [C.POINTER(OmEncoderConfig), C.POINTER(OmT5DecoderWeights), c_void_p, c_void_p,
                                            c_int64, c_int64, c_float, C.c_uint64, c_void_p, c_size_t, c_void_p,
                                            c_void_p, c_size_t, c_void_p]),
    "om_t5_decoder_train_backward": (c_int, [C.POINTER(OmEncoderConfig), C.POINTER(OmT5DecoderWeights), c_void_p, c_void_p,
                                             c_int64, c_int64, c_float, C.c_uint64, c_void_p, c_void_p,
                                             C.POINTER(OmT5DecoderGrads), c_void_p, c_void_p, c_size_t, c_void_p]),
    "om_linear_f32_backward": (c_int, [c_void_p, c_void_p, c_void_p, c_void_p, c_void_p, c_int, c_int, c_int, c_void_p]),
    "om_index_to_f16": (c_int, [c_void_p, c_int64, c_int, c_void_p, c_void_p, c_void_p]),
    "om_index_add_f16": (c_int, [c_int, c_void_p, c_int64, c_int, c_void_p, c_void_p, c_void_p, c_void_p]),
    "om_debug_rescore_rows": (c_int, [c_int, c_int, c_void_p, c_int64, c_int, c_void_p, c_int64, c_void_p, c_int, c_void_p, c_void_p, c_size_t,
                                      c_void_p]),
    "om_sim_topk_workspace_bytes": (c_size_t, [c_int64, c_int, c_int]),
    "om_sim_topk": (c_int, [c_int, c_void_p, c_int64, c_void_p, c_void_p, c_void_p, c_int64, c_int,
                            c_int, c_int64, c_void_p, c_void_p, c_void_p, c_size_t, c_void_p]),
    "om_sim_topk_async_workspace_bytes": (c_size_t, [c_int64, c_int, c_int]),
    "om_sim_topk_async": (c_int, [c_int, c_void_p, c_int64, c_void_p, c_void_p, c_void_p, c_int64, c_int,
                                  c_int, c_int64, c_void_p, c_void_p, c_void_p, c_void_p, c_size_t, c_void_p]),
    "om_debug_search_schedule": (c_int, [c_int, c_int64, c_int64, c_int, C.POINTER(c_int64), c_int, C.POINTER(c_int)]),
    "om_sim_topk_filtered_workspace_bytes": (c_size_t, [c_int64, c_int, c_int]),
    "om_sim_topk_filtered": (c_int, [c_int, c_void_p, c_int64, c_void_p, c_void_p, c_void_p, c_int64, c_int, c_int, c_int64, c_void_p, c_int64,
                                     c_void_p, c_void_p, c_void_p, c_void_p, c_size_t, c_void_p]),
    "om_debug_search_schedule_filtered": (c_int, [c_int, c_int64, c_int64, c_int, c_int64, C.POINTER(c_int64), c_int, C.POINTER(c_int),
                                                  C.POINTER(c_int64)]),
    "om_debug_search_filter_estimate": (c_int, [c_int, c_int64, c_int, c_int64, C.POINTER(c_int64), C.POINTER(c_int64)]),
    "om_sim_topk_info": (None, [C.POINTER(c_int64)]),
    "om_debug_scan_plan": (c_int, [c_int, c_int64, c_int, C.POINTER(c_int)]),
    "om_debug_scan_round": (c_int, [c_int, c_int64, c_int, c_int64, c_int, C.POINTER(c_int64)]),
    "om_debug_sim_stream": (c_int, [c_void_p, c_int64, C.c_uint32, c_void_p, c_int64, c_int, c_void_p, c_void_p, c_void_p, c_int, c_void_p]),
    "om_topk_merge": (c_int, [c_void_p, c_void_p, c_int, c_int64, c_int, c_int, c_void_p, c_void_p,
                              c_void_p]),
    "om_contrastive_fwd_bwd": (c_int, [c_void_p, c_void_p, c_int, c_int, c_int, c_int, c_float,
                                       c_int, c_int, c_int, c_int, c_void_p, c_void_p, c_void_p,
                                       c_void_p, c_void_p, c_void_p]),
    "om_encoder_train_set_layer_events": (c_int, [c_void_p, c_int]),
    "om_comm_unique_id": (c_int, [c_void_p]),
    "om_comm_init": (c_int, [c_void_p, c_int, c_int, C.POINTER(c_void_p)]),
    "om_comm_destroy": (c_int, [c_void_p]),
    "om_comm_count": (c_int, [c_void_p, C.POINTER(c_int)]),
    "om_allgather_rows": (c_int, [c_void_p, c_void_p, c_void_p, c_int64, c_int64, c_void_p]),
    "om_allreduce_grads": (c_int, [c_void_p, c_void_p, c_int64, c_int, c_void_p]),
    "om_exchange_topk": (c_int, [c_void_p, c_int, c_void_p, c_void_p, c_int64, c_int, c_void_p, c_void_p, c_void_p]),
    "om_grad_sqnorm": (c_int, [c_void_p, c_void_p, c_int, c_void_p, c_void_p, c_void_p]),
    "om_adamw_step": (c_int, [c_void_p, c_void_p, c_int, c_float, c_float, c_float, c_float, c_int64, c_void_p, c_float, c_float,
                              c_int, c_void_p, c_void_p]),
    "om_loss_scale_update": (c_int, [c_void_p, c_void_p, c_int, c_void_p]),
    "om_contrastive_fwd_bwd_ex": (c_int, [c_void_p, c_void_p, c_int, c_int, c_int, c_void_p, c_int, c_int, c_void_p,
                                          c_float, c_int, c_int, c_int, c_int, c_void_p, c_void_p, c_void_p,
                                          c_void_p, c_void_p, c_void_p]),
}

_lib = None


class NativeError(RuntimeError):
    pass


def lib():
    global _lib
    if _lib is None:
        if not os.path.exists(LIB_PATH):
            raise NativeError(
                f"{LIB_PATH} is missing: build the HIP library first "
                "(python -m openmatch_amd._build, or __graft_entry__.build()). "
                "openmatch_amd has no CPU / eager fallback.")
        handle = C.CDLL(LIB_PATH)
        for name, (res, args) in _SIGNATURES.items():
            try:
                fn = getattr(handle, name)
            except AttributeError as e:
                raise NativeError(f"{LIB_PATH} does not export {name}; rebuild it") from e
            fn.restype, fn.argtypes = res, args
        if handle.om_abi_version() != ABI_VERSION:
            raise NativeError("libopenmatch_hip.so ABI version mismatch; rebuild it")
        _lib = handle
    return _lib


def exported_symbols():
    return list(_SIGNATURES)


def check(rc):
    if rc != 0:
        raise NativeError(lib().om_last_error().decode("utf-8", "replace"))


def require_device(*tensors):
    for t in tensors:
        if t is None:
            continue
        if not t.is_cuda:
            raise NativeError(
                "openmatch_amd runs on MI355X only: got a CPU tensor. Move the model and the batch "
                "to the GPU (model.to('cuda')); there is no CPU / eager fallback.")
        if not t.is_contiguous():
            raise NativeError("non-contiguous tensor passed to the HIP boundary")


def ptr(t):
    return c_void_p(t.data_ptr()) if t is not None else c_void_p(0)


def stream_ptr(device=None):
    return c_void_p(torch.cuda.current_stream(device).cuda_stream)


class Workspace:
    _pool = {}

    @classmethod
    def get(cls, device, nbytes, tag="default"):
        key = (str(device), tag)
        buf = cls._pool.get(key)
        if buf is None or buf.numel() - ((-buf.data_ptr()) % 256) < nbytes:
            buf = torch.empty(int(nbytes) + 256, dtype=torch.uint8, device=device)
            cls._pool[key] = buf
        off = (-buf.data_ptr()) % 256
        return buf, buf.data_ptr() + off
```

Before: 75660 passages/s.

## Compute only the CLS query row in the last encoder layer's attention

```diff
diff --git a/include/openmatch_hip.h b/include/openmatch_hip.h
--- a/include/openmatch_hip.h
+++ b/include/openmatch_hip.h
@@ -101,7 +101,8 @@
 #define OM_OPT_ENCODER_SKIP_PAD 22
 #define OM_OPT_ENCODER_CLS_TAIL 23
 #define OM_OPT_ENCODER_LANES 24
-#define OM_OPT_COUNT 25
+#define OM_OPT_ENCODER_CLS_QUERY 25
+#define OM_OPT_COUNT 26
 int om_debug_option(int opt, int value);
 int om_debug_option_value(int opt);
 int om_debug_attention(const void* qkv, void* ctx, const int64_t* mask, int64_t B, int L, int H, int heads, void* stream);
@@ -172,6 +173,11 @@
 int om_debug_encoder_skip_pad(const struct OmEncoderConfig* cfg, int gated_ffn, int has_rel_bias, int64_t B, int64_t L, int want_hidden);
 int om_debug_encoder_cls_tail(const struct OmEncoderConfig* cfg, int gated_ffn, int has_rel_bias, int64_t B, int64_t L, int64_t packed_rows,
                               int want_hidden);
+int om_debug_encoder_cls_query(const struct OmEncoderConfig* cfg, int gated_ffn, int has_rel_bias, int64_t B, int64_t L, int64_t packed_rows,
+                               int want_hidden);
+int om_debug_encoder_cls_query_last(void);
+int om_debug_attention_cls(int dtype, const void* qkv, const void* q, void* ctx, const int64_t* mask, int64_t B, int L, int H, int heads,
+                           float scale, void* stream, int reverse, const int* kmax, const int* cu, int64_t Mc);
 int om_debug_encoder_lanes(const struct OmEncoderConfig* cfg, int gated_ffn, int has_rel_bias, int64_t B, int64_t L, int64_t packed_rows,
                            int want_hidden, int64_t* B0);
 #define OM_ENCODER_LANE_RANGES 15
diff --git a/openmatch_amd/csrc/abi.cpp b/openmatch_amd/csrc/abi.cpp
--- a/openmatch_amd/csrc/abi.cpp
+++ b/openmatch_amd/csrc/abi.cpp
@@ -118,6 +118,8 @@
   g_opt[OM_OPT_ENCODER_CLS_TAIL] = e ? atoi(e) : 1;
   e = getenv("OM_ENCODER_LANES");
   g_opt[OM_OPT_ENCODER_LANES] = e ? atoi(e) : 65536;
+  e = getenv("OM_ENCODER_CLS_QUERY");
+  g_opt[OM_OPT_ENCODER_CLS_QUERY] = e ? atoi(e) : 1;
   g_opt_init.store(true);
 }
 }
diff --git a/openmatch_amd/csrc/attention.hip b/openmatch_amd/csrc/attention.hip
--- a/openmatch_amd/csrc/attention.hip
+++ b/openmatch_amd/csrc/attention.hip
@@ -140,11 +140,12 @@
   }
 }
 
-template <typename T, int KT, bool BIAS, bool DROP, int DBG, int KTV>
+template <typename T, int KT, bool BIAS, bool DROP, int DBG, int KTV, bool CLS = false>
 __device__ __forceinline__ void attention_fwd16_body(
     const T* __restrict__ qkv, T* __restrict__ ctx, const int64_t* __restrict__ mask,
     const float* __restrict__ pos_bias, int L, int H, int heads, float scale, float drop_p, uint64_t seed, int rev,
-    int64_t row0, int Lm) {
+    int64_t row0, int Lm,
+    const T* __restrict__ qc = nullptr, int64_t Mc = 0) {
   typedef typename MmaOps<T>::frag_t frag_t;
   extern __shared__ __attribute__((aligned(16))) char smem[];
   char* const sK = smem;
@@ -173,13 +174,14 @@
     sM[k] = k < L ? (mask[b * Lm + k] != 0 ? 0.f : -1e30f) : -INFINITY;
 
   const int q0 = wave * 32;
-  const int qrow = (q0 + l31) < L ? (q0 + l31) : (L - 1);
+  const int qrow = CLS ? 0 : (q0 + l31) < L ? (q0 + l31) : (L - 1);
+  const char* const qbase = CLS ? (const char*)(qc + b * (int64_t)H + h * 64) : base;
   frag_t qf[4];
 #pragma unroll
-  for (int kk = 0; kk < 4; ++kk) qf[kk] = *(const frag_t*)(base + (int64_t)qrow * ld2 + (kk * 2 + half) * 16);
+  for (int kk = 0; kk < 4; ++kk) qf[kk] = *(const frag_t*)(qbase + (int64_t)qrow * ld2 + (kk * 2 + half) * 16);
   asm volatile("s_waitcnt vmcnt(0)" ::: "memory");
   __syncthreads();
-  if (q0 >= L) return;
+  if (CLS ? wave != 0 : q0 >= L) return;
 
   constexpr int KTC = (DBG & 2) ? 0 : KTV;
   const int key = (l31 >> 1) & 7;
@@ -286,6 +288,16 @@
       auto r1 = __builtin_amdgcn_permlane32_swap(a1, b1, false, false);
       *(uint4*)(so + l31 * 128 + (((4 * dt + 2 * gp + half) ^ (l31 & 7)) << 4)) = make_uint4(r0[0], r1[0], r0[1], r1[1]);
     }
+  if (CLS) {
+    if (lane < 8) {
+      const uint4 v = *(const uint4*)(so + (lane << 4));
+      const int64_t nb = gridDim.x / heads;
+      *(uint4*)((char*)(ctx + b * (int64_t)H + h * 64) + lane * 16) = v;
+      if (b == nb - 1)
+        for (int64_t r = nb; r < Mc; ++r) *(uint4*)((char*)(ctx + r * (int64_t)H + h * 64) + lane * 16) = v;
+    }
+    return;
+  }
   char* const out = (char*)(ctx + (row0 + q0) * (int64_t)H + h * 64);
 #pragma unroll
   for (int it = 0; it < 4; ++it) {
@@ -344,6 +356,38 @@
   }
   hipLaunchKernelGGL((attention_fwd16_kernel<T, KT, BIAS, DROP>), dim3((unsigned)(heads * B)), dim3(64 * KT), lds, s, (const T*)qkv,
                      (T*)ctx, mask, pos_bias, L, H, heads, scale, drop_p, seed, rev, kmax, cu);
+  OM_LAUNCH_CHECK();
+  return 0;
+}
+template <typename T, int KT>
+__global__ __launch_bounds__(64 * KT, KT <= 4 ? 4 : 2) void attention_cls16_kernel(
+    const T* __restrict__ qkv, const T* __restrict__ qc, T* __restrict__ ctxc, const int64_t* __restrict__ mask, int L, int H, int heads,
+    float scale, int rev, const int* __restrict__ kmax, const int* __restrict__ cu, int64_t Mc) {
+#define OM_ATTN_BODY(V) attention_fwd16_body<T, KT, false, false, 0, V, true>(qkv, ctxc, mask, nullptr, Lb, H, heads, scale, 0.f, 0, rev, row0, L, qc, Mc)
+  const int64_t b = rev ? (int64_t)(gridDim.x / heads) - 1 - blockIdx.x / heads : blockIdx.x / heads;
+  int64_t row0 = b * L;
+  int Lb = L;
+  if (cu) {
+    const int c0 = __builtin_amdgcn_readfirstlane(cu[b]), c1 = __builtin_amdgcn_readfirstlane(cu[b + 1]);
+    row0 = c0; Lb = c1 - c0;
+    if (Lb <= 0) return;
+  }
+  if (KT == 4 && (kmax || cu)) {
+    const int kt = ((cu ? Lb : __builtin_amdgcn_readfirstlane(kmax[b])) + 31) >> 5;
+    if (kt <= 1) { OM_ATTN_BODY(1); return; }
+    if (kt == 2) { OM_ATTN_BODY(2); return; }
+    if (kt == 3) { OM_ATTN_BODY(3); return; }
+  }
+  OM_ATTN_BODY(KT);
+#undef OM_ATTN_BODY
+}
+template <typename T, int KT>
+static int launch_attn_cls16(const void* qkv, const void* qc, void* ctxc, const int64_t* mask, int64_t B, int L, int H, int heads, float scale,
+                             hipStream_t s, int rev, const int* kmax, const int* cu, int64_t Mc) {
+  const int lds = 2 * KT * 32 * 128 + KT * 32 * 4;
+  if (attn_lds_once<attention_cls16_kernel<T, KT>>(lds)) return 1;
+  hipLaunchKernelGGL((attention_cls16_kernel<T, KT>), dim3((unsigned)(heads * B)), dim3(64 * KT), lds, s, (const T*)qkv, (const T*)qc, (T*)ctxc, mask,
+                     L, H, heads, scale, rev, kmax, cu, Mc);
   OM_LAUNCH_CHECK();
   return 0;
 }
@@ -512,6 +556,29 @@
   }
 }
 
+int omk_attention_cls(int dtype, const void* qkv, const void* q, void* ctx, const int64_t* mask, int64_t B, int L, int H, int heads, float scale,
+                      hipStream_t s, int reverse, const int* kmax, const int* cu, int64_t Mc) {
+  g_attn_last = 0;
+  const AttnPlan p = attn_plan_fwd(dtype, B, L, H, heads, false, 0.f, kmax != nullptr, cu != nullptr, 0, attn_switches(), true);
+  if (p.error) OM_FAIL(p.error);
+  if (p.family == 0) return 0;
+  if (p.family != OM_ATTN_FAMILY_FWD16 && p.family != OM_ATTN_FAMILY_FWD16_KMAX4) OM_FAIL("[CLS]-query attention: planned another kernel family");
+  if (Mc < B) OM_FAIL("[CLS]-query attention: the compact context has fewer rows than sequences");
+  if (((uintptr_t)q | (uintptr_t)ctx) & 15) OM_FAIL("[CLS]-query attention: 16-byte aligned compact buffers");
+  g_attn_last = p.family | (p.kt << 8) | (1 << 16);
+  return attn_with_type16(dtype, [&](auto t) {
+    return attn_with_kt<1, 2, 4, 6, 8>(p.kt, [&](auto kt) {
+      return launch_attn_cls16<decltype(t), kt()>(qkv, q, ctx, mask, B, L, H, heads, scale, s, reverse, kmax, cu, Mc);
+    });
+  });
+}
+extern "C" int om_debug_attention_cls(int dtype, const void* qkv, const void* q, void* ctx, const int64_t* mask, int64_t B, int L, int H, int heads,
+                                      float scale, void* stream, int reverse, const int* kmax, const int* cu, int64_t Mc) {
+  g_attn_last = 0;
+  if (!qkv || !q || !ctx || !mask) OM_FAIL("null argument");
+  return omk_attention_cls(dtype, qkv, q, ctx, mask, B, L, H, heads, scale, (hipStream_t)stream, reverse, kmax, cu, Mc);
+}
+
 extern "C" int om_debug_attention_plan(int dtype, int64_t B, int L, int H, int heads, int has_bias, float drop_p, int has_kmax, int has_cu, int w) {
   const AttnPlan p = attn_plan_fwd(dtype, B, L, H, heads, has_bias != 0, drop_p, has_kmax != 0, has_cu != 0, w, attn_switches());
   if (p.error) { om_set_error(std::string(__func__) + ": " + p.error); return -1; }
diff --git a/openmatch_amd/csrc/attn_plan.h b/openmatch_amd/csrc/attn_plan.h
--- a/openmatch_amd/csrc/attn_plan.h
+++ b/openmatch_amd/csrc/attn_plan.h
@@ -14,13 +14,15 @@
 struct AttnPlan { int family; int kt; bool bias, drop; const char* error; };
 
 static AttnPlan attn_plan_fwd(int dtype, int64_t B, int L, int H, int heads, bool has_bias, float drop_p, bool has_kmax, bool has_cu, int w,
-                              const AttnSwitches sw) {
+                              const AttnSwitches sw, bool cls = false) {
   AttnPlan p = {0, 0, has_bias, drop_p > 0.f, nullptr};
   auto run = [&](int family, int kt) { p.family = family; p.kt = kt; return p; };
   auto refuse = [&](const char* why) { p.error = why; return p; };
   const bool d32 = H == heads * 32;
   if (dtype != OM_F32 && !attn_is16(dtype)) return refuse("attention: dtype must be OM_F32, OM_BF16 or OM_F16");
   if (B <= 0) return p;
+  if (cls && (H != heads * 64 || L < 1 || L > 256 || has_bias || p.drop || w > 0 || (sw.fast & 2) || !(dtype == OM_F16 || (dtype == OM_BF16 && sw.fast))))
+    return refuse("[CLS]-query attention: the whole-row 16-bit kernel only (head_dim 64, up to 256 tokens, no bias, dropout or window)");
   const bool band = w > 0 && w < L - 1;
   if (band && H != heads * 64) return refuse("banded attention: head_dim must be 64");
   if (band && (has_bias || p.drop || has_cu)) return refuse("banded attention: no position bias, dropout, packed rows or reverse walk");
diff --git a/openmatch_amd/csrc/encoder.hip b/openmatch_amd/csrc/encoder.hip
--- a/openmatch_amd/csrc/encoder.hip
+++ b/openmatch_amd/csrc/encoder.hip
@@ -180,6 +180,17 @@
   return encoder_skip_pad(in, encoder_plan(in, sw), sw) ? 1 : 0;
 }
 
+extern "C" int om_debug_encoder_cls_query(const OmEncoderConfig* c, int gated_ffn, int has_rel_bias, int64_t B, int64_t L, int64_t packed_rows,
+                                          int want_hidden) {
+  if (!c) {
+    om_set_error("om_debug_encoder_cls_query: null argument");
+    return -1;
+  }
+  const EncPlanIn in = {c, B, L, packed_rows, want_hidden != 0, gated_ffn != 0, has_rel_bias != 0, c->type_vocab > 0};
+  const EncSwitches sw = encoder_switches();
+  return encoder_cls_query(in, encoder_plan(in, sw), sw) ? 1 : 0;
+}
+
 extern "C" int om_debug_encoder_cls_tail(const OmEncoderConfig* c, int gated_ffn, int has_rel_bias, int64_t B, int64_t L, int64_t packed_rows,
                                          int want_hidden) {
   if (!c) {
@@ -202,6 +213,10 @@
   if (large > nb - 1) large = nb - 1;
   return bucket + large;
 }
+
+static thread_local int g_cls_query_last = 0;
+extern "C" int om_debug_gemm_last(void);
+extern "C" int om_debug_encoder_cls_query_last(void) { return g_cls_query_last; }
 
 static int check_cfg(const OmEncoderConfig* c) {
   if (const char* why = encoder_cfg_error(c)) OM_FAIL(why);
@@ -222,6 +237,7 @@
   hipStream_t s;
   const int* rows_dev;
   int64_t cls_mc;
+  bool cls_query;
   std::vector<int>* families;
   int64_t whole_mg, whole_mc;
 };
@@ -281,6 +297,11 @@
   float* const cst1 = cst2p + 2 * Mc;
   if (Mc > 0 && ((char*)(cst1 + 2 * Mc) > ws.qkv + (size_t)Mg * 3 * H * 2 || Mc > Mg || c->n_layers < 2 || lo8))
     OM_FAIL("[CLS] tail: the compact buffers do not fit the qkv area");
+  const bool cq = k.cls_query;
+  char* const qbase = ws.ff;
+  float* const qst2p = (float*)(qbase + 4 * cplane);
+  if (cq && (Mc <= 0 || nomic || c->head_dim != 64 || L > 256 || k.posbias || (char*)(qst2p + 2 * Mc) > ws.ff + (size_t)Mg * F1 * 2))
+    OM_FAIL("[CLS] query: the compact buffers do not fit the feed-forward area");
 #define OM_WALK() (pingpong ? (walk ^= 1, walk ^ 1) : 0)
   for (int l = 0; l < c->n_layers; ++l) {
     const OmLayerWeights& lw = Ls[l];
@@ -296,6 +317,17 @@
     if (l == 0) {
       e.bias = lw.qkv_b; e.reverse = OM_WALK(); e.rows_dev = k.rows_dev;
       RUN(gemm(ws.x, H, lw.qkv_w, H, ws.qkv, 3 * H, Mg, 3 * H, H, e));
+    } else if (tail && cq) {
+      const OmLayerWeights& pw = Ls[l - 1];
+      const GatherPlane planes[3] = {{ws.x1, qbase + cplane}, {two ? ws.x1_lo : nullptr, qbase + 2 * cplane}, {nullptr, nullptr}};
+      LAUNCH(omk_gather_rows(planes, st2p, qst2p, k.cu ? ws.cls_rows : nullptr, B, L, Mc, H, s));
+      const void* wf; const float *cs, *bfp;
+      RUN(folded_weights(c, k.w, l, false, lw.qkv_w, pw.ln2_g, pw.ln2_b, lw.qkv_b, 3 * H, H, ws.wfold, ws.colsum, ws.bfold, s, &wf, &cs, &bfp));
+      e.bias = bfp + H; e.ln_stats = st2p; e.ln_colsum = cs + H; e.ln_inv_h = inv_h; e.ln_eps = c->ln_eps; e.reverse = OM_WALK(); e.rows_dev = k.rows_dev;
+      RUN(gemm(ws.x1, H, (const char*)wf + (size_t)H * H * 2, H, ws.qkv + (size_t)H * 2, 3 * H, Mg, 2 * H, H, e));
+      e.bias = bfp; e.ln_stats = qst2p; e.ln_colsum = cs; e.reverse = 0; e.rows_dev = nullptr;
+      RUN(gemm(qbase + cplane, H, wf, H, qbase + 3 * cplane, H, Mc, H, H, e));
+      if (!probe) g_cls_query_last = om_debug_gemm_last();
     } else {
       const OmLayerWeights& pw = Ls[l - 1];
       const void* wf; const float *cs, *bfp;
@@ -305,8 +337,14 @@
     }
     if (!probe) NOMIC_ROPE();
     const int attn_walk = OM_WALK();
-    LAUNCH(omk_attention(dt, ws.qkv, ws.ctx, k.mask, k.posbias, B, (int)L, H, nh, scale, 0.f, 0, s, attn_walk, ws.kmax, k.cu));
-    if (tail) {
+    if (tail && cq) {
+      LAUNCH(omk_attention_cls(dt, ws.qkv, qbase + 3 * cplane, qbase, k.mask, B, (int)L, H, nh, scale, s, attn_walk, ws.kmax, k.cu, Mc));
+      ctx = qbase; xin = qbase + cplane; xin_lo = qbase + 2 * cplane; st2p = qst2p;
+      y = cbase + 3 * cplane; y_lo = cbase + 4 * cplane; xout = cbase + 5 * cplane; xout_lo = cbase + 6 * cplane;
+    } else {
+      LAUNCH(omk_attention(dt, ws.qkv, ws.ctx, k.mask, k.posbias, B, (int)L, H, nh, scale, 0.f, 0, s, attn_walk, ws.kmax, k.cu));
+    }
+    if (tail && !cq) {
       const GatherPlane planes[3] = {{ws.ctx, cbase}, {ws.x1, cbase + cplane}, {two ? ws.x1_lo : nullptr, cbase + 2 * cplane}};
       LAUNCH(omk_gather_rows(planes, st2p, cst2p, k.cu ? ws.cls_rows : nullptr, B, L, Mc, H, s));
       ctx = cbase; xin = cbase + cplane; xin_lo = cbase + 2 * cplane; st2p = cst2p;
@@ -779,6 +817,7 @@
   if (c->arch == OM_ARCH_MODERNBERT && (!w->emb_ln_g || !w->final_ln_g)) OM_FAIL("ModernBERT needs emb_ln_g and final_ln_g");
   if (c->arch == OM_ARCH_NOMICBERT && (!w->type_emb || w->pos_emb || w->rel_bias)) OM_FAIL("NomicBERT needs type_emb and takes no pos_emb or rel_bias");
   if (!workspace || ((uintptr_t)workspace & 255)) OM_FAIL("workspace must be 256-byte aligned");
+  g_cls_query_last = 0;
   EncChain whole = {c, w, input_ids, attention_mask, token_type_ids, out_hidden, out_reps, plan_in, plan, sw,
                     carve(c, plan, B, L, packed_rows, (char*)workspace), (hipStream_t)stream, nullptr, 0, 0};
   if (whole.ws.total > workspace_bytes) OM_FAIL("workspace too small");
@@ -810,11 +849,12 @@
   const bool packed = pack_bound > 0;
   int64_t cls_mc = 0;
   if (!encoder_cls_tail(plan_in, plan, sw, &cls_mc)) cls_mc = 0;
+  const bool cls_query = !om_timing_on() && encoder_cls_query(plan_in, plan, sw);
   const int* const row_map = packed ? ws.row_map : nullptr;
   if (families) {
     if (plan.path != OM_ENC_PATH_BERT_FUSED) OM_FAIL("encoder lanes: the fused BERT path only");
     const EncCall k = {c, w, attention_mask, B, L, plan, ws, nullptr, packed ? ws.cu : nullptr, row_map, out_hidden, s, skip ? ws.cu + B : nullptr,
-                       cls_mc, families, q.whole_mg, q.whole_mc};
+                       cls_mc, cls_query, families, q.whole_mg, q.whole_mc};
     EncStream unused = {};
     RUN(bert_fused(k, &unused));
     if (c->head_in > 0 && w->head_w)
@@ -840,7 +880,7 @@
     RUN(omk_embed(dt, input_ids, nullptr, w->word_emb, nullptr, nullptr, nullptr, nullptr, ws.x, M, (int)L, H, c->vocab, 1, c->ln_eps, 0, s, row_map));
 
   const EncCall k = {c, w, attention_mask, B, L, plan, ws, plan.rel_bias ? ws.posbias : nullptr, packed ? ws.cu : nullptr, row_map, out_hidden, s,
-                     skip ? ws.cu + B : nullptr, cls_mc, nullptr, q.whole_mg, q.whole_mc};
+                     skip ? ws.cu + B : nullptr, cls_mc, cls_query, nullptr, q.whole_mg, q.whole_mc};
   EncStream stream_out = {};
   switch (plan.path) {
     case OM_ENC_PATH_BERT_FUSED: RUN(bert_fused(k, &stream_out)); break;
diff --git a/openmatch_amd/csrc/encoder_plan.h b/openmatch_amd/csrc/encoder_plan.h
--- a/openmatch_amd/csrc/encoder_plan.h
+++ b/openmatch_amd/csrc/encoder_plan.h
@@ -15,12 +15,14 @@
   int skip_pad;
   int cls_tail;
   int lanes;
+  int cls_query;
 };
 
 static EncSwitches encoder_switches() {
   return EncSwitches{om_option(OM_OPT_ENCODER_FUSED_LN), om_option(OM_OPT_ENCODER_TWO_PLANE), om_option(OM_OPT_ENCODER_PINGPONG),
                      om_option(OM_OPT_GEMM_SKINNY_M), om_option(OM_OPT_FEW_ROWS_LN_FUSE), om_option(OM_OPT_ATTENTION_FAST),
-                     om_option(OM_OPT_ENCODER_SKIP_PAD), om_option(OM_OPT_ENCODER_CLS_TAIL), om_option(OM_OPT_ENCODER_LANES)};
+                     om_option(OM_OPT_ENCODER_SKIP_PAD), om_option(OM_OPT_ENCODER_CLS_TAIL), om_option(OM_OPT_ENCODER_LANES),
+                     om_option(OM_OPT_ENCODER_CLS_QUERY)};
 }
 
 struct EncPlanIn {
@@ -184,6 +186,15 @@
   return true;
 }
 
+static bool encoder_cls_query(const EncPlanIn& in, const EncPlan& p, const EncSwitches sw) {
+  int64_t mc = 0;
+  if (!sw.cls_query || !encoder_cls_tail(in, p, sw, &mc)) return false;
+  const OmEncoderConfig* c = in.c;
+  if (c->arch != OM_ARCH_BERT || c->head_dim != 64 || in.L > 256 || p.rel_bias || in.has_rel_bias) return false;
+  if (!(c->dtype == OM_F16 || (c->dtype == OM_BF16 && sw.attention_fast)) || (sw.attention_fast & 2)) return false;
+  return mc * (4 * (int64_t)c->hidden * 2 + 8) <= p.Mp * (int64_t)enc_ffn1_cols(c) * 2;
+}
+
 static const int64_t ENC_LANE_ROWS_END = 131072;
 static bool encoder_lanes(const EncPlanIn& in, const EncPlan& p, const EncSwitches sw, int64_t* B0 = nullptr) {
   if (sw.lanes <= 0 || in.packed_rows != 0 || in.want_hidden || in.has_rel_bias || in.c->pooling == OM_POOL_NONE) return false;
@@ -193,13 +204,13 @@
   const int64_t b0 = in.B / 2 / step * step;
   if (b0 <= 0 || b0 * in.L < (int64_t)sw.lanes || (in.B - b0) * in.L < (int64_t)sw.lanes) return false;
   if ((in.B - b0) * in.L >= ENC_LANE_ROWS_END) return false;
-  const bool skip = encoder_skip_pad(in, p, sw), tail = encoder_cls_tail(in, p, sw);
+  const bool skip = encoder_skip_pad(in, p, sw), tail = encoder_cls_tail(in, p, sw), query = encoder_cls_query(in, p, sw);
   for (const int64_t bh : {b0, in.B - b0}) {
     EncPlanIn li = in;
     li.B = bh;
     const EncPlan lp = encoder_plan_checked(li, sw);
     if (lp.error || lp.path != p.path || lp.two != p.two || lp.lo8 != p.lo8 || lp.pingpong != p.pingpong) return false;
-    if (encoder_skip_pad(li, lp, sw) != skip || encoder_cls_tail(li, lp, sw) != tail) return false;
+    if (encoder_skip_pad(li, lp, sw) != skip || encoder_cls_tail(li, lp, sw) != tail || encoder_cls_query(li, lp, sw) != query) return false;
   }
   if (B0) *B0 = b0;
   return true;
diff --git a/openmatch_amd/csrc/kernels.h b/openmatch_amd/csrc/kernels.h
--- a/openmatch_amd/csrc/kernels.h
+++ b/openmatch_amd/csrc/kernels.h
@@ -33,6 +33,8 @@
                   const int* kmax = nullptr ,
                   const int* cu = nullptr ,
                   int w = 0 );
+int omk_attention_cls(int dtype, const void* qkv, const void* q, void* ctx, const int64_t* mask, int64_t B, int L, int H, int heads, float scale,
+                      hipStream_t s, int reverse, const int* kmax, const int* cu, int64_t Mc);
 struct AttnPlan;
 int omk_attention_d32(const AttnPlan& p, int dtype, const void* qkv, void* ctx, const int64_t* mask, const float* pos_bias, int64_t B, int L,
                       int H, int heads, float scale, float drop_p, uint64_t seed, hipStream_t s, int reverse, const int* kmax, const int* cu);
diff --git a/openmatch_amd/native.py b/openmatch_amd/native.py
--- a/openmatch_amd/native.py
+++ b/openmatch_amd/native.py
@@ -193,6 +193,10 @@
     "om_debug_encoder_plan": (c_int, [C.POINTER(OmEncoderConfig), c_int, c_int, c_int64, c_int64, c_int64, c_int]),
     "om_debug_encoder_skip_pad": (c_int, [C.POINTER(OmEncoderConfig), c_int, c_int, c_int64, c_int64, c_int]),
     "om_debug_encoder_cls_tail": (c_int, [C.POINTER(OmEncoderConfig), c_int, c_int, c_int64, c_int64, c_int64, c_int]),
+    "om_debug_encoder_cls_query": (c_int, [C.POINTER(OmEncoderConfig), c_int, c_int, c_int64, c_int64, c_int64, c_int]),
+    "om_debug_encoder_cls_query_last": (c_int, []),
+    "om_debug_attention_cls": (c_int, [c_int, c_void_p, c_void_p, c_void_p, c_void_p, c_int64, c_int, c_int, c_int, c_float, c_void_p, c_int, c_void_p,
+                                       c_void_p, c_int64]),
     "om_debug_encoder_lanes": (c_int, [C.POINTER(OmEncoderConfig), c_int, c_int, c_int64, c_int64, c_int64, c_int, C.POINTER(c_int64)]),
     "om_debug_encoder_lane_ranges": (c_int, [C.POINTER(OmEncoderConfig), c_int, c_int, c_int64, c_int64, c_int, C.POINTER(c_int64), c_int]),
     "om_debug_encoder_lane_forks": (c_int64, []),
```

Result: no change. 75970 passages/s, median of 6 (+0.4%).
